# PMatthaei/ma-league

Measured on AMD Instinct MI355X. Metric: env-steps/sec (rollout+learn), 5v5 QMIX, 4096 envs, at 1/2/4/8 MI355X, higher is better.
Workload: dtype f32

## Files before the change

### include/maleague.h

```cpp
#ifndef MALEAGUE_H
#define MALEAGUE_H

#include <stdint.h>

#ifdef __cplusplus
extern "C" {
#endif

#define MLG_MAXU 64

typedef struct {
    int32_t U;
    int32_t n_agents;
    int32_t n_actions;
    int32_t grid;
    int32_t episode_limit;
    int32_t stochastic;
    int32_t policy_team;
    int32_t n_policy_teams;
    int32_t team[MLG_MAXU];
    int32_t role[MLG_MAXU];
    int32_t melee[MLG_MAXU];
    int32_t agent_unit[MLG_MAXU];
    int32_t scripted[2];
    uint64_t seed;
} MlgEnvSpec;

typedef struct {
    int32_t *x, *y, *hp;
    int32_t *t;
    uint32_t *episode;
    int32_t B;
} MlgEnvState;

typedef struct {
    float *state;
    float *obs;
    int64_t *actions;
    int32_t *avail;
    float *reward;
    uint8_t *terminated;
    float *actions_onehot;
    int64_t *filled;
    int32_t B, T1;
    int32_t ring_slot0, ring_size, full_write;
    const int32_t *rows;
    int32_t *slot_extent;
} MlgBatch;

typedef struct {
    int32_t *ep_len;
    float *ret;
    int32_t *won;
    int32_t *draw;
    uint64_t *agent_rows;
    float *ret_away;
} MlgRunInfo;

typedef struct {
    const float *fc1_w, *fc1_b;
    const float *w_ih, *b_ih;
    const float *w_hh, *b_hh;
    const float *fc2_w, *fc2_b;
} MlgAgentParams;

typedef struct {
    int32_t d_obs, n_actions, n_agents, hidden, d_in;
    int32_t obs_last_action, obs_agent_id;
} MlgAgentDims;

int64_t mlg_packed_agent_size(const MlgAgentDims *d);
int mlg_pack_agent(const MlgAgentDims *d, const MlgAgentParams *p, float *packed, void *stream);

int mlg_env_reset(const MlgEnvSpec *spec, MlgEnvState *st, void *stream);
int mlg_env_step(const MlgEnvSpec *spec, MlgEnvState *st, const int64_t *actions ,
                 float *reward , int32_t *done , int32_t *won ,
                 int32_t *draw , void *stream);
int mlg_env_observe(const MlgEnvSpec *spec, const MlgEnvState *st, float *obs ,
                    float *state , int32_t *avail , void *stream);

int mlg_rollout(const MlgEnvSpec *spec, MlgEnvState *st, const MlgAgentDims *dims, const float *packed,
                MlgBatch *batch, MlgRunInfo *info, float epsilon, int32_t test_mode, void *stream);

int mlg_rollout_selfplay(const MlgEnvSpec *spec, MlgEnvState *st, const MlgAgentDims *dims, const float *home_packed,
                         const float *away_packed, MlgBatch *home, MlgBatch *away, MlgRunInfo *info,
                         float eps_home, float eps_away, int32_t test_mode, void *stream);

int mlg_rollout_describe(const MlgEnvSpec *spec, const MlgAgentDims *dims, int32_t selfplay, char *name,
                         int32_t name_cap, int64_t *lds_bytes);

int mlg_zero_slots_bytes(const MlgBatch *batch, const int64_t *slot_bytes, int32_t slot0, int32_t count,
                         int32_t ring_size, void *stream);

int mlg_agent_forward(const MlgAgentDims *d, const float *packed, const float *inputs, const float *h_in,
                      float *q, float *h_out, int32_t R, void *stream);

int mlg_mac_forward(const MlgAgentDims *d, const float *packed, const MlgBatch *batch, int32_t t,
                    const float *h_in, float *q , float *h_out, void *stream);

int mlg_select_actions(const float *q, const int32_t *avail, int32_t R, int32_t A, int32_t n_agents,
                       const uint64_t *keys, const uint32_t *episodes, int32_t t, float epsilon,
                       int64_t *actions, int64_t *is_greedy, void *stream);

typedef struct {
    const float *hw1_0w, *hw1_0b, *hw1_2w, *hw1_2b;
    const float *hwf_0w, *hwf_0b, *hwf_2w, *hwf_2b;
    const float *hb1_w, *hb1_b;
    const float *v0_w, *v0_b, *v2_w, *v2_b;
    int32_t n_agents, state_dim, embed_dim, hypernet_embed, hypernet_layers;
} MlgQMixParams;
int mlg_qmix_forward(const MlgQMixParams *p, const float *agent_qs , const float *states ,
                     float *q_tot , int32_t R, void *stream);

int64_t mlg_agent_backward_workspace_floats(const MlgAgentDims *d, int32_t R);
int mlg_agent_backward(const MlgAgentDims *d, const MlgAgentParams *p, const float *packed, const float *inputs,
                       const float *h_in, const float *gq, const float *gh_out, float *d_inputs, float *d_h_in,
                       float *dparams, float *workspace, int32_t R, void *stream);
int64_t mlg_qmix_backward_workspace_floats(const MlgQMixParams *p, int32_t R);
int mlg_qmix_backward(const MlgQMixParams *p, const float *agent_qs, const float *states, const float *g_qtot,
                      float *d_agent_qs, float *dparams, float *workspace, int32_t R, void *stream);

typedef struct {
    int32_t B, T, N, A, d_obs, H, S, E, HE, hypernet_layers;
    int32_t mixer;
    int32_t double_q, obs_last_action, obs_agent_id;
    float gamma, lr, optim_alpha, optim_eps, grad_norm_clip;
    int32_t agent;
    int32_t distinct;
} MlgLearnerCfg;

typedef struct {
    MlgBatch batch;
    float *params;
    float *grads;
    float *square_avg;
    const float *target_params;
    float *workspace;
    float *stats;
    float *target_sync;
    double *trained_steps;
    const int32_t *host_rows;
} MlgLearnerBufs;

int64_t mlg_qlearner_param_counts(const MlgLearnerCfg *c, int64_t *n_agent, int64_t *n_mixer);
int64_t mlg_qlearner_workspace_floats(const MlgLearnerCfg *c);
int mlg_qlearner_inline_rows(void);
int mlg_qlearner_train(const MlgLearnerCfg *c, const MlgLearnerBufs *b, void *stream);
int mlg_qlearner_describe(const MlgLearnerCfg *c, char *name, int32_t name_cap);


typedef struct {
    MlgEnvSpec base;
    int32_t min_agents, max_agents;
} MlgEntityEnvSpec;

typedef struct {
    float *entities;
    uint8_t *obs_mask;
    uint8_t *entity_mask;
    int64_t *actions;
    int32_t *avail;
    float *reward;
    uint8_t *terminated;
    float *actions_onehot;
    int64_t *filled;
    int32_t B, T1, ring_slot0, ring_size, full_write;
    const int32_t *rows;
    int32_t *slot_extent;
} MlgEntityBatch;

typedef struct {
    int32_t n_agents, n_entities, entity_shape, n_actions, entity_last_action;
    int32_t attn_embed_dim, attn_n_heads, rnn_hidden_dim;
} MlgRefilDims;

int64_t mlg_refil_packed_agent_size(const MlgRefilDims *d);
int mlg_refil_pack_agent(const MlgRefilDims *d, const float *flat, float *packed, void *stream);

int mlg_refil_agent_forward(const MlgRefilDims *d, const float *packed, const float *entities, const uint8_t *obs_mask,
                            const uint8_t *entity_mask, const float *h_in, float *q, float *h_out, int32_t R,
                            void *stream);

int mlg_refil_rollout(const MlgEntityEnvSpec *spec, MlgEnvState *st, const MlgRefilDims *d, const float *packed,
                      MlgEntityBatch *batch, MlgRunInfo *info, float epsilon, int32_t test_mode, void *stream);

int mlg_refil_rollout_describe(const MlgEntityEnvSpec *spec, const MlgRefilDims *d, char *name, int32_t name_cap,
                               int64_t *lds_bytes);

int mlg_refil_attention(const float *w_in, const float *w_out, const float *b_out, const float *x,
                        const uint8_t *pre_mask, const uint8_t *post_mask, int32_t bs, int32_t ne, int32_t nq,
                        int32_t n_heads, float *y, void *stream);

int64_t mlg_refil_packed_mixer_size(const MlgRefilDims *d);
int mlg_refil_pack_mixer(const MlgRefilDims *d, const float *flat, float *packed, void *stream);
int mlg_refil_mixer_forward(const MlgRefilDims *d, const float *packed, const float *agent_qs, const float *entities,
                            const uint8_t *entity_mask, const uint8_t *w_mask, const uint8_t *i_mask,
                            int32_t softmax_mixing_weights, float *q_tot, int32_t R, void *stream);

int64_t mlg_refil_attention_backward_workspace_floats(int32_t bs, int32_t ne, int32_t nq, int32_t n_heads);
int mlg_refil_attention_backward(const float *w_in, const float *w_out, const float *b_out, const float *x,
                                 const uint8_t *pre_mask, const uint8_t *post_mask, const float *gy, int32_t bs,
                                 int32_t ne, int32_t nq, int32_t n_heads, float *dx, float *dparams, float *workspace,
                                 void *stream);
int64_t mlg_refil_mixer_backward_workspace_floats(const MlgRefilDims *d, int32_t R, int32_t imagine);
int mlg_refil_mixer_backward(const MlgRefilDims *d, const float *packed, const float *agent_qs, const float *entities,
                             const uint8_t *entity_mask, const uint8_t *w_mask, const uint8_t *i_mask,
                             int32_t softmax_mixing_weights, const float *g_qtot, float *d_agent_qs, float *dparams,
                             float *workspace, int32_t R, void *stream);
int64_t mlg_refil_agent_backward_workspace_floats(const MlgRefilDims *d, int32_t R);
int mlg_refil_agent_backward(const MlgRefilDims *d, const float *packed, const float *entities,
                             const uint8_t *obs_mask, const uint8_t *entity_mask, const float *h_in, const float *gq,
                             const float *gh_out, float *d_h_in, float *dparams, float *workspace, int32_t R,
                             void *stream);

typedef struct {
    int32_t B, T, n_agents, n_entities, entity_shape, n_actions, entity_last_action;
    int32_t attn_embed_dim, attn_n_heads, rnn_hidden_dim, hypernet_embed, mixing_embed_dim;
    int32_t double_q, softmax_mixing_weights;
    int32_t imagine;
    int32_t mixer;
    float gamma, lmbda, lr, optim_alpha, optim_eps, grad_norm_clip;
} MlgRefilLearnerCfg;

typedef struct {
    MlgEntityBatch batch;
    const uint8_t *groupA;
    float *params;
    float *grads;
    float *square_avg;
    const float *target_params;
    float *workspace;
    float *stats;
    double *trained_steps;
    float *target_sync;
    const int32_t *host_rows;
} MlgRefilLearnerBufs;

int64_t mlg_refil_param_counts(const MlgRefilLearnerCfg *c, int64_t *n_agent, int64_t *n_mixer);
int64_t mlg_refil_workspace_floats(const MlgRefilLearnerCfg *c);
int mlg_refil_train(const MlgRefilLearnerCfg *c, const MlgRefilLearnerBufs *b, void *stream);
int mlg_refil_draw_groups(int32_t B, int32_t NE, uint64_t seed, uint32_t draw, uint8_t *groupA, void *stream);

int mlg_debug_set_stamps(void *ptr);
int mlg_debug_set_learner_stamps(void *ptr);
int mlg_refil_debug_set_stamps(void *ptr);

int mlg_league_record_runs(const int32_t *won, const int32_t *draw, int32_t B, float *entry, int32_t count_games,
                           void *stream);

typedef struct {
    int32_t home, away;
    int32_t spec;
} MlgCrossplayPair;

typedef struct {
    const float *packed_pool;
    int32_t n_pool;
    int32_t n_pairs;
    const MlgCrossplayPair *pairs;
    const MlgCrossplayPair *host_pairs;
    const MlgEnvSpec *specs;
    const MlgEnvSpec *host_specs;
    int32_t n_specs;
    int32_t E;
    uint32_t episode0;
    float *workspace;
    int64_t workspace_floats;
    int32_t *ep_len;
    float *ret, *ret_away;
    int32_t *won;
    int32_t *draw;
    float *summary;
} MlgCrossplay;

int64_t mlg_crossplay_workspace_floats(const MlgAgentDims *dims, int32_t n_pairs, int32_t E);
int mlg_crossplay_rollout(const MlgAgentDims *dims, const MlgCrossplay *c, void *stream);

int mlg_pack_agent_pool(const MlgAgentDims *dims, const float *flat, int64_t row_stride, int32_t P,
                        float *packed_pool, void *stream);

int mlg_policy_probs(const float *logits, const int32_t *avail, int32_t R, int32_t A, float epsilon,
                     int32_t mask_before_softmax, int32_t test_mode, float *probs, void *stream);
int mlg_policy_probs_backward(const float *logits, const int32_t *avail, const float *g_probs, int32_t R, int32_t A,
                              float epsilon, int32_t mask_before_softmax, int32_t test_mode, float *d_logits,
                              void *stream);

int mlg_select_multinomial(const float *probs, const int32_t *avail, int32_t R, int32_t A, int32_t n_agents,
                           const uint64_t *keys, const uint32_t *episodes, int32_t t, int32_t greedy,
                           int64_t *actions, void *stream);

int mlg_rollout_policy(const MlgEnvSpec *spec, MlgEnvState *st, const MlgAgentDims *dims, const float *packed,
                       MlgBatch *batch, MlgRunInfo *info, float epsilon, int32_t test_mode,
                       int32_t mask_before_softmax, int32_t test_greedy, void *stream);

// ... 70 lines not shown
```

### ma-league_amd/csrc/distinct.hip

```cpp
#include <cstdlib>
#include <cstring>

#include "agent_device.h"
#include "rollout_env_device.h"
#include "rollout_host.h"

int check_agent_dims(const MlgAgentDims* d);

namespace {

constexpr int DX_MAX_WAVES = 8, DX_MAX_TPW = 4;

__device__ __forceinline__ floatx4 dx_row_chunk(const float* obs, const float* onehot, int k0, int d_obs, int d_in) {
    floatx4 v = {0.f, 0.f, 0.f, 0.f};
    if (!obs) return v;
#pragma unroll
    for (int r = 0; r < 4; ++r) {
        const int k = k0 + r;
        v[r] = k < d_obs ? obs[k] : ((onehot && k < d_in) ? onehot[k - d_obs] : 0.f);
    }
    return v;
}

template <int H>
// ... 100 lines not shown
    SpecShared& SS = *reinterpret_cast<SpecShared*>(smem + lay.env.spec);
    const RoEnv R = env_view(smem, lay.env);
    const int U = spec.U, N = spec.n_agents, A = spec.n_actions, S = 6 * U, DO = 8 * U;
    const int tid = threadIdx.x, nthr = blockDim.x;
    const int lane = tid & 63, wave = __builtin_amdgcn_readfirstlane(tid >> 6), W = nthr >> 6;
    const int e0 = blockIdx.x * RE;
    const int T1 = sd.bt[0].T1;
    const bool any_full_write = sd.bt[0].full_write != 0;
    load_spec_tables(spec, SS);
    const EnvTables T = make_tables(spec, SS);
    const float inv_p = 1.0f / (float)pow2_at_least(spec.grid);
    ro_reset<RoNoStamps>(T, SS, spec, st, R, sd, e0, inv_p);
    __syncthreads();

    floatx4 h[TPW][HC];
#pragma unroll
    for (int ti = 0; ti < TPW; ++ti)
#pragma unroll
        for (int c = 0; c < HC; ++c) h[ti][c] = floatx4{0.f, 0.f, 0.f, 0.f};
    RoNoStamps sp;
    sp.init();
    const int e = lane & 15, g = lane >> 4;
    const int n_at = L.Ap / 16;
    int last_t = 0;
    for (int t = 0; t < T1; ++t) {
#pragma unroll
        for (int ti = 0; ti < TPW; ++ti) {
            const int a = wave + ti * W;
            if (a >= N) continue;
            const bool valid = R.status[e] < 2;
            if (!__any(valid)) continue;
            int zero = 0;
            asm volatile("" : "+s"(zero));
            const WView Wv = global_view(sd.P[0] + (int64_t)a * L.total + zero, L);
            const MlgBatch bt = sd.bt[0];
            const int64_t bt_off = valid ? ((int64_t)R.slot[e] * T1 + t) * N + a : 0;
            RowIn in;
            in.x = valid ? bt.obs + bt_off * DO : nullptr;
            in.onehot = nullptr;
            in.prev_action = (valid && t > 0) ? R.prev[e * N + a] : -1;
            in.agent = 0;
            agent_cell_hidden<H>(Wv, L, in, h[ti], lane);
            const int32_t* av = valid ? bt.avail + bt_off * A : nullptr;
            ArgmaxState as{-INFINITY, 1 << 30};
            for (int at = 0; at < n_at; ++at) {
                const floatx4 q = agent_q_tile<H>(Wv, h[ti], at, lane);
                argmax_accumulate(as, q, av, at, A, lane);
            }
            const int act = argmax_reduce(as);
            if (valid && g == 0) ro_record_action(spec, R, sd, act, av, e, a, e0 + e, t, test_mode);
        }
        __syncthreads();
        ro_env_step(T, SS, spec, R, sd, info, e0, t, inv_p, sp);
        if (any_full_write && t + 1 < T1) zero_slots(sd, R, e0, t + 1, t + 2, A, S, DO);
        if (tid == 0) ro_list_running(R);
        __syncthreads();
        last_t = t;
        if (!R.misc[0]) break;
    }
    for (int x = tid; x < RE; x += nthr) R.stepped[x] = 0;
    __syncthreads();
    if (any_full_write && last_t + 2 < T1) zero_slots(sd, R, e0, last_t + 2, T1, A, S, DO);
    ro_finish(st, R, sd, info, e0, sd.bt[0].B, U);
}

int check_distinct_dims(const MlgAgentDims* dims, const char* who) {
    if (check_agent_dims(dims)) return 1;
    MLG_REQUIRE(dims->obs_agent_id == 0,
                "%s: obs_agent_id must be 0 (distinct agent networks take no agent id: network i is agent i)", who);
    return 0;
}

struct DxPlan {
    AgentLayout L;
    int tpw, waves;
    RolloutLds lay;
    char name[24];
};

int plan_distinct(const MlgEnvSpec* spec, const MlgAgentDims* dims, DxPlan* p) {
    MLG_REQUIRE(dims->n_agents == spec->n_agents && dims->n_actions == spec->n_actions && dims->d_obs == 8 * spec->U,
                "rollout_distinct: agent dims do not match env spec (N=%d/%d A=%d/%d d_obs=%d/%d)", dims->n_agents,
                spec->n_agents, dims->n_actions, spec->n_actions, dims->d_obs, 8 * spec->U);
    p->L = make_agent_layout(*dims);
    const int tiles = spec->n_agents;
    MLG_REQUIRE(tiles <= DX_MAX_WAVES * DX_MAX_TPW,
                "rollout_distinct: %d agent tiles (one per agent) > %d: at most %d tiles per wave on %d waves", tiles,
                DX_MAX_WAVES * DX_MAX_TPW, DX_MAX_TPW, DX_MAX_WAVES);
    p->waves = tiles < DX_MAX_WAVES ? tiles : DX_MAX_WAVES;
    p->tpw = (tiles + p->waves - 1) / p->waves;
    p->lay = make_rollout_lds(p->L, spec->U, spec->n_agents, false);
    MLG_REQUIRE((int64_t)p->lay.total * 4 <= LDS_LIMIT_BYTES,
                "rollout_distinct: the env state of %d units does not fit in LDS", spec->U);
    snprintf(p->name, sizeof p->name, "dx-global/tpw%d", p->tpw);
    return 0;
}

template <int H, int TPW>
int launch_distinct(const DxPlan& p, int grid, hipStream_t s, const MlgEnvSpec& spec, const MlgEnvState& st,
                    const Sides& sd, const MlgRunInfo& info, int test_mode) {
    const size_t bytes = (size_t)p.lay.total * 4;
    auto kern = rollout_distinct_kernel<H, TPW>;
    if (int rc = allow_lds(kern, bytes, "rollout_distinct")) return rc;
    hipLaunchKernelGGL(kern, dim3(grid), dim3(p.waves * 64), bytes, s, spec, st, p.L, sd, info, test_mode, p.lay);
    return 0;
}

}

extern "C" int mlg_mac_forward_distinct(const MlgAgentDims* d, const float* packed_pool, const MlgBatch* batch,
                                        int32_t t, const float* h_in, float* q, float* h_out, void* stream) {
    if (check_distinct_dims(d, "mac_forward_distinct")) return 1;
    MLG_REQUIRE(packed_pool && batch && batch->obs && batch->actions_onehot && q && h_out,
                "mac_forward_distinct: bad arguments");
    MLG_REQUIRE(mlg::aligned16(packed_pool), "mac_forward_distinct: packed_pool must be 16-byte aligned");
    MLG_REQUIRE(batch->B >= 0, "mac_forward_distinct: batch B=%d", batch->B);
    MLG_REQUIRE(t >= 0 && t < batch->T1, "mac_forward_distinct: t=%d out of [0, %d)", t, batch->T1);
    if (batch->B == 0) return 0;
    const AgentLayout L = make_agent_layout(*d);
    const int tpa = (batch->B + 15) / 16, tiles = tpa * d->n_agents;
    const int grid = (tiles + 3) / 4;
    hipStream_t s = (hipStream_t)stream;
#define MLG_DX_FWD(HH)                                                                                             \
    hipLaunchKernelGGL(mac_forward_distinct_kernel<HH>, dim3(grid), dim3(256), 0, s, L, packed_pool, *batch, (int)t, \
                       h_in, q, h_out, tpa, tiles)
    if (d->hidden == 64) MLG_DX_FWD(64);
    else if (d->hidden == 32) MLG_DX_FWD(32);
    else MLG_DX_FWD(128);
#undef MLG_DX_FWD
    return mlg::check_launch("mac_forward_distinct_kernel");
}

extern "C" int mlg_rollout_distinct_describe(const MlgEnvSpec* spec, const MlgAgentDims* dims, char* name,
                                             int32_t name_cap, int64_t* lds_bytes) {
    if (check_spec(spec) || check_distinct_dims(dims, "rollout_distinct_describe")) return 1;
    MLG_REQUIRE(name && name_cap > 0 && lds_bytes, "rollout_distinct_describe: null output");
    DxPlan plan;
    if (int rc = plan_distinct(spec, dims, &plan)) return rc;
    MLG_REQUIRE((size_t)name_cap > strlen(plan.name), "rollout_distinct_describe: name buffer of %d bytes too small",
                name_cap);
    strcpy(name, plan.name);
    *lds_bytes = (int64_t)plan.lay.total * 4;
    return 0;
}

extern "C" int mlg_rollout_distinct(const MlgEnvSpec* spec, MlgEnvState* st, const MlgAgentDims* dims,
                                    const float* packed_pool, MlgBatch* batch, MlgRunInfo* info, float epsilon,
                                    int32_t test_mode, void* stream) {
    if (check_spec(spec) || check_state(st) || check_distinct_dims(dims, "rollout_distinct")) return 1;
    MLG_REQUIRE(packed_pool && batch && info, "rollout_distinct: null pointer");
    MLG_REQUIRE(mlg::aligned16(packed_pool), "rollout_distinct: packed_pool must be 16-byte aligned");
    if (check_rollout_batch(batch, spec, st, "rollout_distinct")) return 1;
    MLG_REQUIRE(info->ep_len && info->ret && info->won && info->draw, "rollout_distinct: run info has null tensors");
    DxPlan plan;
    if (int rc = plan_distinct(spec, dims, &plan)) return rc;
    hipStream_t s = (hipStream_t)stream;
    Sides sd;
    sd.bt[0] = sd.bt[1] = *batch;
    sd.P[0] = sd.P[1] = packed_pool;
    sd.eps[0] = sd.eps[1] = test_mode ? 0.f : epsilon;
    sd.ns = 1;
    sd.nh = spec->n_agents;
    const int grid = (st->B + RE - 1) / RE;
    int rc = 0;
#define MLG_RO(HH, TT) rc = launch_distinct<HH, TT>(plan, grid, s, *spec, *st, sd, *info, test_mode ? 1 : 0)
#define MLG_RO_H(HH)                       \
    if (plan.tpw == 1) MLG_RO(HH, 1);      \
    else if (plan.tpw == 2) MLG_RO(HH, 2); \
    else if (plan.tpw == 3) MLG_RO(HH, 3); \
    else MLG_RO(HH, 4)
    if (plan.L.H == 64) {
        MLG_RO_H(64);
    } else if (plan.L.H == 32) {
        MLG_RO_H(32);
    } else {
        MLG_RO_H(128);
    }
#undef MLG_RO_H
#undef MLG_RO
    if (rc) return rc;
    return mlg::check_launch("rollout_distinct_kernel");
}
```

### ma-league_amd/csrc/learner.hip

```cpp
#include <algorithm>
#include <cstdio>
#include <cstring>

#include "agent_device.h"
#include "agent_ff_device.h"
#include "batch_mask_device.h"
#include "gru4_device.h"
#include "mlg_host.h"
#include "wgrad_device.h"

namespace {

using WJobs = mlg::BJobsT<16>;
using mlg::block_sum_1024;

struct AgentOffs {
    int64_t fc1w, fc1b, wih, whh, bih, bhh, fc2w, fc2b, total;
};
__host__ __device__ inline AgentOffs agent_offs(int H, int d_in, int A) {
    AgentOffs o;
    int64_t p = 0;
    o.fc1w = p; p += (int64_t)H * d_in;
    o.fc1b = p; p += H;
    o.wih = p; p += (int64_t)3 * H * H;
// ... 2256 lines not shown
                           ws + p.w.gr, ws + p.w.gz, ws + p.w.gn, ws + p.w.ghn, sk);
        hipLaunchKernelGGL((agent_q_kernel<H, true>), dim3(ntiles, c.T, 2 * c.N), dim3(64 * dsp.q_tiles), 0, s, c, p.L,
                           ws + p.w.p_on, ws + p.w.p_tg, ws + p.w.hs, ws + p.w.hs_tg, ws + p.w.mac, ws + p.w.tmac, sk);
    } else if (c.ff)
        hipLaunchKernelGGL((ff_hidden_kernel<H>), dim3(ntiles, c.T, 2), dim3(threads), 0, s, c, bt, p.L, ws + p.w.p_on,
                           ws + p.w.p_tg, ws + p.w.in, ws + p.w.hs, ws + p.w.hs_tg, sk);
    else
        hipLaunchKernelGGL((agent_in_kernel<H>), dim3(ntiles, c.T, 2), dim3(threads), 0, s, c, bt, p.L, ws + p.w.p_on,
                           ws + p.w.p_tg, ws + p.w.in, ws + p.w.x, ws + p.w.gi_on, ws + p.w.gi_tg, sk);
    if (c.ff || c.dx) {
    } else if (split_mix) {
        const int nrec = 2 * ((c.R + 3) / 4), per = dsp.per;
        hipLaunchKernelGGL((rec4_mixpre_kernel<H>), dim3(nrec + (p.w.n_mix_tiles + per - 1) / per), dim3(threads), 0, s,
                           c, p.L, ws + p.w.p_on, ws + p.w.p_tg, ws + p.w.gi_on, ws + p.w.gi_tg, ws + p.w.hs,
                           ws + p.w.hs_tg, ws + p.w.gr, ws + p.w.gz, ws + p.w.gn, ws + p.w.ghn, sk, bt, Mon,
                           Mtg, p.mp, hy);
    } else
        hipLaunchKernelGGL((agent_rec4_kernel<H>), dim3(2 * ((c.R + 3) / 4)), dim3(threads), 0, s, c, p.L,
                           ws + p.w.p_on, ws + p.w.p_tg, ws + p.w.gi_on, ws + p.w.gi_tg, ws + p.w.hs, ws + p.w.hs_tg,
                           ws + p.w.gr, ws + p.w.gz, ws + p.w.gn, ws + p.w.ghn, sk);
    if (!c.dx)
        hipLaunchKernelGGL((agent_q_kernel<H>), dim3(ntiles, c.T, 2), dim3(64 * dsp.q_tiles), 0, s, c, p.L, ws + p.w.p_on,
                           ws + p.w.p_tg, ws + p.w.hs, ws + p.w.hs_tg, ws + p.w.mac, ws + p.w.tmac, sk);
    MixOut mo{ws + p.w.srow, ws + p.w.l1act, ws + p.w.d1, ws + p.w.da2, ws + p.w.df2, ws + p.w.dv2,
              ws + p.w.dq, ws + p.w.d2, ws + p.w.part};
#define MLG_MIX_LAUNCH(K)                                                                                       \
    hipLaunchKernelGGL((K), dim3(p.w.n_mix_tiles), dim3(128), 0, s, c, bt, Mon, Mtg, p.mp, ws + p.w.mac, ws + p.w.tmac, \
                       ws + p.w.msum, mo, sk)
    switch (dsp.mix) {
        case MIX_IQL:
            hipLaunchKernelGGL(iql_td_kernel, dim3(p.w.n_mix_tiles), dim3(64), 0, s, c, bt, ws + p.w.mac, ws + p.w.tmac,
                               ws + p.w.msum, mo, sk);
            break;
        case MIX_QMIX_SPLIT:
            hipLaunchKernelGGL((mix_td2_kernel<64, 32>), dim3(p.w.n_mix_tiles), dim3(128), 0, s, c, bt, Mon, ws + p.w.mac,
                               ws + p.w.tmac, ws + p.w.msum, hy, mo, sk);
            break;
        case MIX_VDN_FAST:
        case MIX_QMIX_FAST1: MLG_MIX_LAUNCH((mix_td_kernel<64, 32, true>)); break;
        case MIX_QMIX1:
            if (c.E == 16) MLG_MIX_LAUNCH(mix_td1_kernel<16>);
            else if (c.E == 32) MLG_MIX_LAUNCH(mix_td1_kernel<32>);
            else MLG_MIX_LAUNCH(mix_td1_kernel<64>);
            break;
        case MIX_VDN:
        case MIX_QMIX_DFLT: MLG_MIX_LAUNCH((mix_td_kernel<64, 32>)); break;
        case MIX_QMIX_WIDTHS:
            switch (c.HE * 1000 + c.E) {
                case 32016: MLG_MIX_LAUNCH((mix_td_kernel<32, 16>)); break;
                case 32032: MLG_MIX_LAUNCH((mix_td_kernel<32, 32>)); break;
                case 32064: MLG_MIX_LAUNCH((mix_td_kernel<32, 64>)); break;
                case 64016: MLG_MIX_LAUNCH((mix_td_kernel<64, 16>)); break;
                case 64064: MLG_MIX_LAUNCH((mix_td_kernel<64, 64>)); break;
                case 128016: MLG_MIX_LAUNCH((mix_td_kernel<128, 16>)); break;
                case 128032: MLG_MIX_LAUNCH((mix_td_kernel<128, 32>)); break;
                case 128064: MLG_MIX_LAUNCH((mix_td_kernel<128, 64>)); break;
                default: return mlg::fail("learner: no mixer kernel for hypernet_embed=%d mixing_embed_dim=%d", c.HE, c.E);
            }
            break;
    }
#undef MLG_MIX_LAUNCH
    int64_t slab_floats, n_red;
    int n_tasks;
    mlg::BRepeat rp{};
    WJobs J = make_jobs(p, ws, bufs->grads, &slab_floats, &n_tasks, &n_red, &rp);
    if (c.dx) {
        hipLaunchKernelGGL((agent_bwd4_kernel<H, true>), dim3((Ra + 3) / 4, c.N), dim3(threads), 0, s, c, bt, p.L,
                           ws + p.w.p_on, ws + p.w.hs, ws + p.w.gr, ws + p.w.gz, ws + p.w.gn, ws + p.w.ghn, ws + p.w.dq,
                           ws + p.w.dgi, ws + p.w.dgh, sk);
        hipLaunchKernelGGL((agent_dx_kernel<H, true>), dim3(ntiles, c.T, c.N), dim3(threads), 0, s, c, ws + p.w.wihT,
                           ws + p.w.x, ws + p.w.dgi, ws + p.w.da, sk);
        hipLaunchKernelGGL(mlg::wgrad_block_rep_kernel<16>, dim3((unsigned)((n_tasks + 3) / 4)), dim3(256), 0, s, J, rp,
                           ws + p.w.slab);
        return run_finish(p, cfg, bufs, s, J, n_red, pj.flag, sk, ntiles, &rp);
    }
    if (c.ff) {
        hipLaunchKernelGGL((ff_bwd_kernel<H>), dim3(ntiles, c.T), dim3(threads), 0, s, c, p.L, ws + p.w.p_on, ws + p.w.hs,
                           ws + p.w.d2, ws + p.w.da, sk);
        hipLaunchKernelGGL(mlg::wgrad_block_kernel<16>, dim3((unsigned)((n_tasks + 3) / 4)), dim3(256), 0, s, J,
                           ws + p.w.slab);
        return run_finish(p, cfg, bufs, s, J, n_red, pj.flag, sk, ntiles);
    }
    int ta, tb;
    int64_t ra, rb;
    const WJobs JA = mlg::bjob_view(J, 3, J.n, &ta, &ra), JB = mlg::bjob_view(J, 0, 3, &tb, &rb);
    constexpr bool fused = Dispatch::fused_for(H);
    if constexpr (fused) {
        const int nbwd = (c.R + 3) / 4;
        hipLaunchKernelGGL((bwd4_wgrad_kernel<H>), dim3((unsigned)(nbwd + (ta + 3) / 4)), dim3(256), 0, s, c, bt, p.L,
                           ws + p.w.p_on, ws + p.w.hs, ws + p.w.gr, ws + p.w.gz, ws + p.w.gn, ws + p.w.ghn, ws + p.w.dq,
                           ws + p.w.dgi, ws + p.w.dgh, sk, JA, ws + p.w.slab, nbwd);
    } else {
        hipLaunchKernelGGL((agent_bwd4_kernel<H>), dim3((c.R + 3) / 4), dim3(threads), 0, s, c, bt, p.L, ws + p.w.p_on,
                           ws + p.w.hs, ws + p.w.gr, ws + p.w.gz, ws + p.w.gn, ws + p.w.ghn, ws + p.w.dq, ws + p.w.dgi,
                           ws + p.w.dgh, sk);
    }
    hipLaunchKernelGGL((agent_dx_kernel<H>), dim3(ntiles, c.T), dim3(threads), 0, s, c, ws + p.w.wihT, ws + p.w.x,
                       ws + p.w.dgi, ws + p.w.da, sk);
    if (fused)
        hipLaunchKernelGGL(mlg::wgrad_block_kernel<16>, dim3((unsigned)((tb + 3) / 4)), dim3(256), 0, s, JB,
                           ws + p.w.slab);
    else
        hipLaunchKernelGGL(mlg::wgrad_block_kernel<16>, dim3((unsigned)((n_tasks + 3) / 4)), dim3(256), 0, s, J,
                           ws + p.w.slab);
    return run_finish(p, cfg, bufs, s, J, n_red, pj.flag, sk, ntiles);
}

}

extern "C" int mlg_debug_set_learner_stamps(void* ptr) {
#ifdef MLG_STAMPS
    hipError_t e = hipMemcpyToSymbol(HIP_SYMBOL(g_mlg_lstamps), &ptr, sizeof(ptr));
    if (e != hipSuccess) return mlg::fail("set learner stamps: %s", hipGetErrorString(e));
    return 0;
#else
    (void)ptr;
    return mlg::fail("not a stamps build (-DMLG_STAMPS)");
#endif
}

extern "C" int64_t mlg_qlearner_param_counts(const MlgLearnerCfg* c, int64_t* n_agent, int64_t* n_mixer) {
    if (check_cfg(c)) return -1;
    Plan p = make_plan(c, c->T);
    if (n_agent) *n_agent = p.n_agent;
    if (n_mixer) *n_mixer = p.n_mixer;
    return p.n_agent + p.n_mixer;
}

extern "C" int mlg_qlearner_inline_rows(void) { return MLG_INLINE_ROWS; }

extern "C" int64_t mlg_qlearner_workspace_floats(const MlgLearnerCfg* c) {
    if (check_cfg(c)) return -1;
    Plan p = make_plan(c, c->T);
    int64_t slab, n_red;
    int tasks;
    mlg::BRepeat rp{};
    make_jobs(p, nullptr, nullptr, &slab, &tasks, &n_red, &rp);
    return p.w.total + slab;
}

extern "C" int mlg_qlearner_describe(const MlgLearnerCfg* c, char* name, int32_t name_cap) {
    if (check_cfg(c)) return 1;
    MLG_REQUIRE(name && name_cap > 0, "qlearner_describe: null output");
    Plan p = make_plan(c, c->T);
    Dispatch d;
    if (make_dispatch(p, &d)) return 1;
    char full[64];
    dispatch_name(p.c, d, full, sizeof full);
    MLG_REQUIRE((size_t)name_cap > strlen(full), "qlearner_describe: name buffer of %d bytes too small", name_cap);
    strcpy(name, full);
    return 0;
}

extern "C" int mlg_qlearner_train(const MlgLearnerCfg* c, const MlgLearnerBufs* b, void* stream) {
    if (check_cfg(c)) return 1;
    MLG_REQUIRE(b && b->params && b->grads && b->square_avg && b->target_params && b->workspace && b->stats,
                "qlearner_train: null buffer");
    const MlgBatch& bt = b->batch;
    MLG_REQUIRE(bt.state && bt.obs && bt.actions && bt.avail && bt.reward && bt.terminated && bt.actions_onehot && bt.filled,
                "qlearner_train: batch has null tensors");
    MLG_REQUIRE(bt.B == c->B && bt.T1 >= c->T, "qlearner_train: batch B=%d T1=%d vs cfg B=%d T=%d", bt.B, bt.T1, c->B, c->T);
    MLG_REQUIRE(!b->host_rows || c->B <= MLG_INLINE_ROWS, "qlearner_train: host_rows needs B <= %d (got %d)",
                MLG_INLINE_ROWS, c->B);
    Plan p = make_plan(c, bt.T1);
    hipStream_t s = (hipStream_t)stream;
    if (c->H == 64) return run_train<64>(p, c, b, s);
    if (c->H == 32) return run_train<32>(p, c, b, s);
    return run_train<128>(p, c, b, s);
}
```

### ma-league_amd/csrc/mlg_host.h

```cpp
#pragma once
#include <hip/hip_runtime.h>

#include <cstdarg>
#include <cstdio>
#include <mutex>
#include <string>

constexpr int MLG_INLINE_ROWS = 64;

namespace mlg {

inline std::string& last_error() {
    static thread_local std::string err;
    return err;
}

inline int fail(const char* fmt, ...) {
    char buf[1024];
    va_list ap;
    va_start(ap, fmt);
    vsnprintf(buf, sizeof(buf), fmt, ap);
    va_end(ap);
    last_error() = buf;
    return 1;
}

inline int check_launch(const char* what) {
    hipError_t e = hipGetLastError();
    if (e != hipSuccess) return fail("%s: %s", what, hipGetErrorString(e));
    return 0;
}

inline bool aligned16(const void* p) { return (reinterpret_cast<uintptr_t>(p) & 15u) == 0; }

struct SideStream {
    hipStream_t s = nullptr;
    hipEvent_t ev[4] = {nullptr, nullptr, nullptr, nullptr};
};
inline SideStream* side_stream(hipStream_t caller) {
    static SideStream side[64];
    static std::mutex mu;
    int dev = 0;
    hipDevice_t sdev = 0;
    if (hipGetDevice(&dev) != hipSuccess || dev < 0 || dev >= 64) return nullptr;
    if (hipStreamGetDevice(caller, &sdev) != hipSuccess || (int)sdev != dev) return nullptr;
    std::lock_guard<std::mutex> lk(mu);
    SideStream& ss = side[dev];
    if (!ss.s) {
        int least = 0, greatest = 0;
        if (hipDeviceGetStreamPriorityRange(&least, &greatest) != hipSuccess) return nullptr;
        SideStream fresh;
        for (auto& e : fresh.ev)
            if (hipEventCreateWithFlags(&e, hipEventDisableTiming) != hipSuccess) {
                for (auto& x : fresh.ev)
                    if (x) (void)hipEventDestroy(x);
                return nullptr;
            }
        if (hipStreamCreateWithPriority(&fresh.s, hipStreamNonBlocking, least) != hipSuccess) {
            for (auto& x : fresh.ev) (void)hipEventDestroy(x);
            return nullptr;
        }
        ss = fresh;
    }
    return &ss;
}
inline bool fork_join(SideStream* ss, int k, hipStream_t from, hipStream_t to) {
    return hipEventRecord(ss->ev[k], from) == hipSuccess && hipStreamWaitEvent(to, ss->ev[k], 0) == hipSuccess;
}

}

#define MLG_REQUIRE(cond, ...)                  \
    do {                                        \
        if (!(cond)) return mlg::fail(__VA_ARGS__); \
    } while (0)
```

### ma-league_amd/csrc/refil.hip

```cpp
#include <cstdlib>
#include <cstring>

#include "mlg_host.h"
#include "refil_device.h"
#include "refil_host.h"

using namespace refil;

#define RO_PHASE __device__ inline

#ifdef MLG_STAMPS
__device__ unsigned long long* g_refil_stamps = nullptr;
struct RStamps {
    unsigned long long acc[30], last, begin;
    __device__ void init() {
        for (int k = 0; k < 30; ++k) acc[k] = 0;
        last = begin = __builtin_amdgcn_s_memtime();
    }
    __device__ void mark(int k) {
        const unsigned long long now = __builtin_amdgcn_s_memtime();
        acc[k] += now - last;
        last = now;
    }
    unsigned long long s0;
// ... 724 lines not shown
    const int lane = threadIdx.x;
    const int i0 = blockIdx.x * 2;
    zero_tile(o, lane);
    if (lane < 32) {
        const int e = lane >> 4, q = lane & 15;
        const int64_t it = i0 + e;
        mrow[e][q] = (it < R && q < NEa) ? mask_row_bits(om + (it * NEa + q) * NEa, NEa) : 0xFFFFFFFFu;
        if (q == 0) emb[e] = it < R ? mask_row_bits(em + it * NEa, NEa) : 0xFFFFFFFFu;
    }
    wave_sync();
    for (int e = 0; e < 2; ++e) {
        const int64_t it = i0 + e;
        load_entity_rows(it < R ? ent + it * NEa * D0 : nullptr, NEa, D0, L.K1, ein, lane, 64);
        wave_sync();
        entity_block(P, L, ein, x1, qkv, mrow[e], NA, NEa, o + e * NAS * LDX, nullptr, lane);
    }
    const int col = lane & 15, g = lane >> 4;
    const int e = col >> 3, n = col & 7, it = i0 + e;
    const bool valid = it < R && n < NA;
    const uint32_t dead = dead_rows(emb[0], NA, NAS) | dead_rows(emb[1], NA, NAS) << 8;
    floatx4 h[4];
#pragma unroll
    for (int mt = 0; mt < 4; ++mt)
        h[mt] = valid ? ld4(h_in + ((int64_t)it * NA + n) * EMB + mt * 16 + 4 * g) : floatx4{0.f, 0.f, 0.f, 0.f};
    agent_tile_post(P, L, o, dead, h, lane);
    if (valid) {
#pragma unroll
        for (int mt = 0; mt < 4; ++mt) *reinterpret_cast<floatx4*>(h_out + ((int64_t)it * NA + n) * EMB + mt * 16 + 4 * g) = h[mt];
    }
    for (int at = 0; at < L.Ap / 16; ++at) {
        const floatx4 q = agent_q(P, L, h, at, dead, lane);
        if (valid) {
#pragma unroll
            for (int r = 0; r < 4; ++r) {
                const int ac = at * 16 + 4 * g + r;
                if (ac < A) q_out[((int64_t)it * NA + n) * A + ac] = q[r];
            }
        }
    }
}

#include "refil_ro4.inc"

}

extern "C" int mlg_refil_debug_set_stamps(void* ptr) {
#ifdef MLG_STAMPS
    unsigned long long* p = (unsigned long long*)ptr;
    if (hipMemcpyToSymbol(HIP_SYMBOL(g_refil_stamps), &p, sizeof(p)) != hipSuccess) return mlg::fail("set stamps");
    return 0;
#else
    (void)ptr;
    return mlg::fail("mlg_refil_debug_set_stamps: build with -DMLG_STAMPS (make stamps)");
#endif
}

extern "C" int64_t mlg_refil_packed_agent_size(const MlgRefilDims* d) {
    if (check_refil_dims(d)) return -1;
    return agent_layout(d).total;
}

extern "C" int mlg_refil_pack_agent(const MlgRefilDims* d, const float* flat, float* packed, void* stream) {
    if (check_refil_dims(d)) return 1;
    MLG_REQUIRE(flat && packed, "refil_pack_agent: null pointer");
    const RAgent L = agent_layout(d);
    if (launch_copy(agent_pack_jobs(L), flat, packed, (hipStream_t)stream)) return 1;
    hipLaunchKernelGGL(refil_pack_gsp_kernel, dim3((unsigned)((REFIL_GSP + REFIL_WSP + 255) / 256)), dim3(256), 0,
                       (hipStream_t)stream,
                       L, flat, packed);
    return mlg::check_launch("refil_pack_gsp_kernel");
}

extern "C" int mlg_refil_agent_forward(const MlgRefilDims* d, const float* packed, const float* entities,
                                       const uint8_t* obs_mask, const uint8_t* entity_mask, const float* h_in, float* q,
                                       float* h_out, int32_t R, void* stream) {
    if (check_refil_dims(d)) return 1;
    MLG_REQUIRE(packed && entities && obs_mask && entity_mask && h_in && q && h_out, "refil_agent_forward: null pointer");
    MLG_REQUIRE(R >= 0, "refil_agent_forward: R=%d", R);
    if (R == 0) return 0;
    const RAgent L = agent_layout(d);
    hipLaunchKernelGGL(refil_agent_step_kernel, dim3((unsigned)((R + 1) / 2)), dim3(64), 0, (hipStream_t)stream, L, packed,
                       R, d->n_agents, d->n_entities, L.D0, d->n_actions, entities, obs_mask, entity_mask, h_in, q, h_out);
    return mlg::check_launch("refil_agent_forward");
}

namespace {

struct RefilRolloutPlan {
    const char* name;
    bool four;
    bool st16;
    int kc;
    size_t lds_bytes;
};

int plan_refil_rollout(const MlgEntityEnvSpec* spec, const MlgRefilDims* d, RefilRolloutPlan* plan) {
    if (check_refil_dims(d)) return 1;
    MLG_REQUIRE(spec != nullptr, "refil_rollout: null argument");
    const MlgEnvSpec& sp = spec->base;
    const int S = sp.U / 2;
    MLG_REQUIRE(sp.U >= 2 && sp.U % 2 == 0 && sp.U <= NE && S <= NAS, "refil_rollout: U=%d unsupported (even, <= 16)",
                sp.U);
    MLG_REQUIRE(sp.n_agents == S && d->n_agents == S && d->n_entities == sp.U && d->entity_shape == 8 &&
                    d->n_actions == MLG_ACT_BASE + sp.U && d->entity_last_action,
                "refil_rollout: dims (n_agents=%d n_entities=%d entity_shape=%d n_actions=%d) do not match the env "
                "(S=%d, U=%d)", d->n_agents, d->n_entities, d->entity_shape, d->n_actions, S, sp.U);
    MLG_REQUIRE(spec->min_agents >= 1 && spec->min_agents <= spec->max_agents && spec->max_agents <= S,
                "refil_rollout: min_agents=%d max_agents=%d (slots %d)", spec->min_agents, spec->max_agents, S);
    MLG_REQUIRE(sp.policy_team == 0 && sp.scripted[0] == 0 && sp.scripted[1] == 1,
                "refil_rollout: the entity env has policy team 0 and scripted team 1");
    const RAgent L = agent_layout(d);
    const char* var = getenv("MLG_REFIL_ROLLOUT");
    const bool v1 = (var && strcmp(var, "v1") == 0) || L.K1 != 32;
    if (!v1) {
        const bool generic = getenv("MLG_REFIL_GENERIC") != nullptr;
        const bool st16 = sp.U == 16 && !generic;
        *plan = RefilRolloutPlan{st16 ? "ro4-static" : "ro4", true, st16, 2, sizeof(R4Shared)};
        return 0;
    }
    const int kc = L.K1 <= 16 ? 1 : (L.K1 <= 32 ? 2 : 3);
    static const char* const names[3] = {"ro2/kc1", "ro2/kc2", "ro2/kc3"};
    *plan = RefilRolloutPlan{names[kc - 1], false, false, kc, sizeof(RoShared)};
    return 0;
}

}

extern "C" int mlg_refil_rollout_describe(const MlgEntityEnvSpec* spec, const MlgRefilDims* d, char* name,
                                          int32_t name_cap, int64_t* lds_bytes) {
    MLG_REQUIRE(name && name_cap > 0 && lds_bytes, "refil_rollout_describe: null output");
    RefilRolloutPlan plan;
    if (int rc = plan_refil_rollout(spec, d, &plan)) return rc;
    MLG_REQUIRE((size_t)name_cap > strlen(plan.name), "refil_rollout_describe: name buffer of %d bytes too small",
                name_cap);
    strcpy(name, plan.name);
    *lds_bytes = (int64_t)plan.lds_bytes;
    return 0;
}

extern "C" int mlg_refil_rollout(const MlgEntityEnvSpec* spec, MlgEnvState* st, const MlgRefilDims* d,
                                 const float* packed, MlgEntityBatch* batch, MlgRunInfo* info, float epsilon,
                                 int32_t test_mode, void* stream) {
    MLG_REQUIRE(spec && st && packed && batch && info, "refil_rollout: null argument");
    RefilRolloutPlan plan;
    if (int rc = plan_refil_rollout(spec, d, &plan)) return rc;
    const MlgEnvSpec& sp = spec->base;
    const int S = sp.U / 2;
    const MlgEntityBatch& bt = *batch;
    MLG_REQUIRE(bt.entities && bt.obs_mask && bt.entity_mask && bt.actions && bt.avail && bt.reward && bt.terminated &&
                    bt.actions_onehot && bt.filled, "refil_rollout: batch has null tensors");
    MLG_REQUIRE(st->B == bt.B && bt.T1 >= sp.episode_limit + 1, "refil_rollout: B=%d/%d T1=%d (episode_limit %d)", st->B,
                bt.B, bt.T1, sp.episode_limit);
    MLG_REQUIRE(info->ep_len && info->ret && info->won && info->draw, "refil_rollout: run info has null buffers");
    if (bt.B == 0) return 0;
    int p = 1;
    while (p < sp.grid) p <<= 1;
    RoArgs a{sp.U, S, d->n_actions, d->entity_shape, S, spec->min_agents, spec->max_agents, bt.B, 1.0f / (float)p};
    const RAgent L = agent_layout(d);
    if (plan.four) {
        const size_t lds4 = plan.lds_bytes;
        const bool st16 = plan.st16;
        auto kern4 = st16 ? refil_rollout4_kernel<2, 16> : refil_rollout4_kernel<2, 0>;
        static bool attr4[2] = {false, false};
        if (!attr4[st16]) {
            hipError_t e = hipFuncSetAttribute(reinterpret_cast<const void*>(kern4),
                                               hipFuncAttributeMaxDynamicSharedMemorySize, (int)lds4);
            if (e != hipSuccess) return mlg::fail("refil_rollout: LDS %zu B: %s", lds4, hipGetErrorString(e));
            attr4[st16] = true;
        }
        const int per_block4 = R4_ENVS * R4_WAVES;
        hipLaunchKernelGGL(kern4, dim3((unsigned)((bt.B + per_block4 - 1) / per_block4)), dim3(64 * R4_WAVES), lds4,
                           (hipStream_t)stream, *spec, *st, L, packed, bt, *info, a, test_mode ? 0.f : epsilon,
                           test_mode);
        return mlg::check_launch("refil_rollout4");
    }
    auto kern = plan.kc == 1 ? refil_rollout_kernel<1>
                             : (plan.kc == 2 ? refil_rollout_kernel<2> : refil_rollout_kernel<3>);
    const size_t lds = plan.lds_bytes;
    static bool attr_set[3] = {false, false, false};
    const int ki = plan.kc - 1;
    if (!attr_set[ki]) {
        hipError_t e = hipFuncSetAttribute(reinterpret_cast<const void*>(kern), hipFuncAttributeMaxDynamicSharedMemorySize,
                                           (int)lds);
        if (e != hipSuccess) return mlg::fail("refil_rollout: LDS %zu B: %s", lds, hipGetErrorString(e));
        attr_set[ki] = true;
    }
    const int per_block = 2 * RO_WAVES;
    hipLaunchKernelGGL(kern, dim3((unsigned)((bt.B + per_block - 1) / per_block)), dim3(64 * RO_WAVES), lds,
                       (hipStream_t)stream, *spec, *st, L, packed, bt, *info, a, test_mode ? 0.f : epsilon, test_mode);
    return mlg::check_launch("refil_rollout");
}
```

### ma-league_amd/csrc/rollout.hip

```cpp
#include <cstring>

#include "agent_device.h"
#include "rollout_env_device.h"
#include "rollout_host.h"

#ifdef MLG_STAMPS
__device__ unsigned long long* g_mlg_stamps = nullptr;
struct Stamps {
    unsigned long long acc[30], last, begin, tstep;
    __device__ void init() {
        for (int k = 0; k < 30; ++k) acc[k] = 0;
        last = begin = tstep = __builtin_amdgcn_s_memtime();
    }
    __device__ void step(int t, int nrun) {
        const unsigned long long now = __builtin_amdgcn_s_memtime();
        if (g_mlg_stamps && threadIdx.x == 0 && t < 128)
            g_mlg_stamps[(int64_t)gridDim.x * 8 * 32 + (int64_t)blockIdx.x * 128 + t] = ((now - tstep) << 8) | (unsigned)nrun;
        tstep = now;
#ifdef MLG_STAMPS_LOWRUN
        on = nrun <= MLG_STAMPS_LOWRUN;
#endif
#ifdef MLG_STAMPS_MINRUN
        on = nrun >= MLG_STAMPS_MINRUN;
#endif
#ifdef MLG_STAMPS_TIMELINE
        on = nrun == 1 && !seen;
        seen = seen || on;
#endif
    }
    bool on = true;
    bool seen = false;
    __device__ void mark(int k) {
        const unsigned long long now = __builtin_amdgcn_s_memtime();
#ifdef MLG_STAMPS_TIMELINE
        if (on) acc[k] = now - tstep;
#else
        if (on) acc[k] += now - last;
#endif
        last = now;
    }
    __device__ void flush() {
        if ((threadIdx.x & 63) || !g_mlg_stamps) return;
        unsigned long long* o = g_mlg_stamps + ((int64_t)blockIdx.x * 8 + (threadIdx.x >> 6)) * 32;
        for (int k = 0; k < 30; ++k) o[k] = acc[k];
        o[30] = __builtin_amdgcn_s_memtime() - begin;
        o[31] = 1;
    }
};
#else
using Stamps = RoNoStamps;
#endif

namespace {

template <int H, int TPW, bool WLDS>
__global__ void __launch_bounds__(512) rollout_kernel(MlgEnvSpec spec, MlgEnvState st, AgentLayout L, Sides sd,
                                                     MlgRunInfo info, int test_mode, RolloutLds lay) {
    constexpr int HC = H / 16;
    extern __shared__ __attribute__((aligned(16))) int smem[];
    SpecShared& SS = *reinterpret_cast<SpecShared*>(smem + lay.env.spec);
    const RoEnv R = env_view(smem, lay.env);
    const int U = spec.U, N = spec.n_agents, A = spec.n_actions, S = 6 * U, DO = 8 * U, nh = sd.nh;
    const int tid = threadIdx.x, nthr = blockDim.x;
    const int lane = tid & 63, wave = tid >> 6, W = nthr >> 6;
    const int e0 = blockIdx.x * RE;
    const int T1 = sd.bt[0].T1;
    const bool any_full_write = sd.bt[0].full_write || (sd.ns > 1 && sd.bt[1].full_write);
    load_spec_tables(spec, SS);
    if (WLDS) load_weights_to_lds(sd.P[0], L, lay.lw, reinterpret_cast<float*>(smem + lay.wts));
    const EnvTables T = make_tables(spec, SS);
    const float inv_p = 1.0f / (float)pow2_at_least(spec.grid);
    ro_reset<Stamps>(T, SS, spec, st, R, sd, e0, inv_p);
    __syncthreads();

    floatx4 h[TPW][HC];
#pragma unroll
    for (int ti = 0; ti < TPW; ++ti)
#pragma unroll
        for (int c = 0; c < HC; ++c) h[ti][c] = floatx4{0.f, 0.f, 0.f, 0.f};
    Stamps sp;
    sp.init();
    const int tps = (RE * nh + 15) / 16, n_tiles = sd.ns * tps;
    const int col = lane & 15, g = lane >> 4;
    const int n_at = L.Ap / 16;
    int last_t = 0;
    for (int t = 0; t < T1; ++t) {
#pragma unroll
        for (int ti = 0; ti < TPW; ++ti) {
            const int tile = wave + ti * W;
            if (tile >= n_tiles) continue;
            const int side = tile >= tps;
            const int r = (tile - side * tps) * 16 + col;
            const bool in_range = r < RE * nh;
            const int e = in_range ? r / nh : 0, ln = r % nh, a = side * nh + ln;
            const bool valid = in_range && R.status[e] < 2;
            if (!__any(valid)) continue;
            int zero = 0;
            asm volatile("" : "+s"(zero));
            const WView Wv = WLDS ? lds_view(reinterpret_cast<const float*>(smem + lay.wts) + zero, lay.lw, L)
                                  : global_view((side ? sd.P[1] : sd.P[0]) + zero, L);
            const MlgBatch bt = side_batch(sd, side);
            const int64_t bt_off = valid ? ((int64_t)side_slot(R, side, e) * T1 + t) * nh + ln : 0;
            RowIn in;
            in.x = valid ? bt.obs + bt_off * DO : nullptr;
            in.onehot = nullptr;
            in.prev_action = (valid && t > 0) ? R.prev[e * N + a] : -1;
            in.agent = valid ? ln : 0;
            agent_cell_hidden<H>(Wv, L, in, h[ti], lane);
            const int32_t* av = valid ? bt.avail + bt_off * A : nullptr;
            ArgmaxState as{-INFINITY, 1 << 30};
            for (int at = 0; at < n_at; ++at) {
                const floatx4 q = agent_q_tile<H>(Wv, h[ti], at, lane);
                argmax_accumulate(as, q, av, at, A, lane);
            }
            const int act = argmax_reduce(as);
            if (valid && g == 0) ro_record_action(spec, R, sd, act, av, e, a, e0 + e, t, test_mode);
        }
        sp.mark(0);
        __syncthreads();
        sp.mark(1);
        ro_env_step(T, SS, spec, R, sd, info, e0, t, inv_p, sp);
        if (any_full_write && t + 1 < T1) zero_slots(sd, R, e0, t + 1, t + 2, A, S, DO);
        if (tid == 0) ro_list_running(R);
        __syncthreads();
        sp.mark(10);
        last_t = t;
        if (!R.misc[0]) break;
    }
    sp.flush();
    for (int e = tid; e < RE; e += nthr) R.stepped[e] = 0;
    __syncthreads();
    if (any_full_write && last_t + 2 < T1) zero_slots(sd, R, e0, last_t + 2, T1, A, S, DO);
    ro_finish(st, R, sd, info, e0, sd.bt[0].B, U);
}

__device__ inline int tail_init(const MlgBatch& bt, int slot) {
    int zend = bt.T1;
    if (bt.full_write && bt.slot_extent) {
        const int x = bt.slot_extent[slot];
        zend = x < 0 ? 0 : (x < bt.T1 ? x : bt.T1);
    }
    return bt.T1 | (zend << 16);
}
__device__ inline int tail_start(int zc, int row) { return (zc & ~0xFFFF) | row; }

__device__ inline void zero_slot_steps(const MlgBatch& bt, int slot, int z0, int z1, int N, int A, int S, int DO,
                                       int lane, int nl) {
    if (z0 >= z1) return;
    const int64_t r0 = (int64_t)slot * bt.T1 + z0;
    const int n = z1 - z0;
    auto z16 = [&](float* p, int per) {
        float* b = p + r0 * per;
        if (per % 4 == 0) {
            uint4* q = reinterpret_cast<uint4*>(b);
            for (int x = lane; x < n * per / 4; x += nl) gst(q + x, make_uint4(0u, 0u, 0u, 0u));
        } else {
            for (int x = lane; x < n * per; x += nl) gst(b + x, 0.f);
        }
    };
    z16(bt.obs, N * DO);
    z16(bt.state, S);
    int* av = bt.avail + r0 * N * A;
    float* oh = bt.actions_onehot + r0 * N * A;
    for (int x = lane; x < n * N * A; x += nl) {
        gst(av + x, 0);
        gst(oh + x, 0.f);
    }
    int64_t* ac = bt.actions + r0 * N;
    for (int x = lane; x < n * N; x += nl) gst(ac + x, (int64_t)0);
    for (int x = lane; x < n; x += nl) {
        gst(bt.reward + r0 + x, 0.f);
        gst(bt.terminated + r0 + x, (uint8_t)0);
        gst(bt.filled + r0 + x, (int64_t)0);
    }
}

struct UnitMasks {
    uint32_t team1, healer, tank, melee;
};

__device__ inline UnitMasks make_unit_masks(const SpecShared& SS, int U) {
    UnitMasks m{0u, 0u, 0u, 0u};
    for (int u = 0; u < U; ++u) {
        m.team1 |= (uint32_t)(SS.team[u] == 1) << u;
        m.healer |= (uint32_t)(SS.role[u] == 1) << u;
        m.tank |= (uint32_t)(SS.role[u] == 0) << u;
        m.melee |= (uint32_t)(SS.melee[u] == 1) << u;
    }
    return m;
}

__device__ __forceinline__ int pk_unit(int x, int y, int hp) { return x | (y << 12) | (hp << 24); }
__device__ __forceinline__ int pk_x(int q) { return q & 0xFFF; }
__device__ __forceinline__ int pk_y(int q) { return (q >> 12) & 0xFFF; }
__device__ __forceinline__ int pk_hp(int q) { return q >> 24; }
__device__ __forceinline__ int mask_role(const UnitMasks& M, int j) {
    return ((M.tank >> j) & 1) ? 0 : (((M.healer >> j) & 1) ? 1 : 2);
}
__device__ __forceinline__ int move_toward_d(int dx, int dy) {
    const int adx = dx < 0 ? -dx : dx, ady = dy < 0 ? -dy : dy;
    if (adx >= ady && dx != 0) return dx > 0 ? 3 : 4;
    if (dy != 0) return dy > 0 ? 1 : 2;
    return 0;
}

struct UnitLane {
    int x, y, hp;
    uint32_t tgt, sight;
    int ai;
};

__device__ __forceinline__ void v2_pair_pass(const UnitMasks& M, int U, int u, UnitLane& L, int* spk) {
    const uint32_t all = U >= 32 ? 0xFFFFFFFFu : ((1u << U) - 1u);
    const int hbase = (threadIdx.x & 63) & 32;
    const uint32_t alive_m = (uint32_t)(__ballot(u < U && L.hp > 0) >> hbase) & all;
    const int pk_own = pk_unit(L.x, L.y, L.hp);
    spk[u] = pk_own;
    const bool split = U <= 16, odd = split && (threadIdx.x & 16) != 0;
    int pkm = pk_own, uu = u;
    if (split) {
        const auto sw = __builtin_amdgcn_permlane16_swap((unsigned)pk_own, (unsigned)pk_own, false, false);
        pkm = odd ? (int)sw[0] : pk_own;
        uu = u & 15;
    }
    const int X = pk_x(pkm), Y = pk_y(pkm), HP = pk_hp(pkm);
    const int my_team = (M.team1 >> uu) & 1;
    const bool healer = (M.healer >> uu) & 1;
    const int r2 = ((M.melee >> uu) & 1) ? 2 : 9;
    const bool alive = HP > 0;
    const uint32_t mates = (my_team ? M.team1 : ~M.team1) & all;
    const uint32_t cand_a = alive ? (mates & alive_m & ~(1u << uu)) : 0u;
    const uint32_t cand_e = alive ? (~mates & alive_m & all) : 0u;
    const uint32_t seen = alive ? alive_m : 0u;
    constexpr uint32_t NONE = 0xFFFFFFFFu;
    uint32_t kbest = NONE, kally = NONE, kenemy = NONE, tgt = 0, sight = 0;
    auto visit = [&](int j, int q) {
        const int hj = pk_hp(q);
        const int dx = pk_x(q) - X, dy = pk_y(q) - Y;
        const uint32_t d2 = (uint32_t)(__mul24(dx, dx) + __mul24(dy, dy));
        const uint32_t bit = 1u << j;
        const bool vis = (seen & bit) && d2 <= MLG_SIGHT2;
        const bool inr = d2 <= (uint32_t)r2;
        const int mxj = (M.tank & bit) ? 64 : 32;
        const bool tg = inr && (healer ? ((cand_a & bit) && hj < mxj) : (cand_e & bit) != 0);
        sight |= vis ? bit : 0u;
        tgt |= tg ? bit : 0u;
        kbest = min(kbest, tg ? ((uint32_t)hj << 5 | j) : NONE);
        kally = min(kally, (cand_a & bit) ? (d2 << 5 | j) : NONE);
        kenemy = min(kenemy, (cand_e & bit) ? (d2 << 5 | j) : NONE);
    };
    if (split) {
        const int JH = (U + 1) >> 1, base = odd ? JH : 0;
        int q[8];
#pragma unroll
        for (int k = 0; k < 8; ++k) q[k] = k < JH ? spk[(base + k) & 31] : 0;
#pragma unroll
        for (int k = 0; k < 8; ++k)
            if (k < JH) visit((base + k) & 31, q[k]);
        auto other = [&](uint32_t v) {
            const auto s2 = __builtin_amdgcn_permlane16_swap(v, v, false, false);
            return (threadIdx.x & 16) ? s2[0] : s2[1];
        };
        kbest = min(kbest, other(kbest));
        kally = min(kally, other(kally));
        kenemy = min(kenemy, other(kenemy));
        tgt |= other(tgt);
        sight |= other(sight);
    } else {
        for (int j0 = 0; j0 < U; j0 += 4) {
            const int4 q4 = *reinterpret_cast<const int4*>(spk + j0);
            visit(j0, q4.x);
            if (j0 + 1 < U) visit(j0 + 1, q4.y);
            if (j0 + 2 < U) visit(j0 + 2, q4.z);
            if (j0 + 3 < U) visit(j0 + 3, q4.w);
        }
    }
    int ai = 0;
    if (alive) {
        uint32_t k = NONE;
        if (kbest != NONE) ai = MLG_ACT_BASE + (int)(kbest & 31);
        else if (healer && kally != NONE) k = (kally >> 5) > 2 ? kally : NONE;
        else k = kenemy;
        if (ai == 0 && k != NONE) {
            const int q = spk[k & 31];
            ai = move_toward_d(pk_x(q) - X, pk_y(q) - Y);
        }
    }
    L.tgt = tgt;
    L.sight = sight;
    L.ai = ai;
}

__device__ __forceinline__ void resolve_hits(const UnitMasks& M, int U, int hl, const int* spk, const int* sact, int& dmg,
                                             int& heal) {
    if (U <= 16) {
        const bool odd = (hl & 16) != 0;
        const int me = MLG_ACT_BASE + (hl & 15), JH = (U + 1) >> 1, base = odd ? JH : 0;
        int qs[8], as[8];
#pragma unroll
        for (int k = 0; k < 8; ++k) {
            qs[k] = k < JH ? spk[(base + k) & 31] : 0;
            as[k] = k < JH ? sact[(base + k) & 31] : 0;
        }
#pragma unroll
        for (int k = 0; k < 8; ++k) {
            if (k >= JH) break;
            const int i = base + k;
            const bool hit = i < U && pk_hp(qs[k]) > 0 && as[k] == me;
            const bool hl_i = (M.healer >> i) & 1;
            heal += (hit && hl_i) ? role_power(1) : 0;
            dmg += (hit && !hl_i) ? role_power(mask_role(M, i)) : 0;
        }
        const auto sd = __builtin_amdgcn_permlane16_swap((unsigned)dmg, (unsigned)dmg, false, false);
        const auto sh = __builtin_amdgcn_permlane16_swap((unsigned)heal, (unsigned)heal, false, false);
        dmg += (int)(odd ? sd[0] : sd[1]);
        heal += (int)(odd ? sh[0] : sh[1]);
        return;
    }
    const int me = MLG_ACT_BASE + hl;
    for (int i0 = 0; i0 < U; i0 += 4) {
        const int4 q4 = *reinterpret_cast<const int4*>(spk + i0);
        const int4 a4 = *reinterpret_cast<const int4*>(sact + i0);
// ... 770 lines not shown
    v2_observe(C.M, spec, *C.SS, C.pairtab, C.avtab, C.bt, slot, t, e, hbase, hl, L, C.lobs, C.ldo, C.lavm, C.inv_p, sp,
               C.obf, C.U, C.N, C.A, C.sd);
}

__device__ inline void env_lane_reset(const EnvCtx& C, const MlgEnvState& st, EnvLane& E, int e, int e0, int hl) {
    const MlgEnvSpec& spec = *C.spec;
    const int hbase = (threadIdx.x & 63) & 32;
    E.e = e;
    E.b = e0 + e;
    E.u = UnitLane{0, 0, 0, 0u, 0u, 0};
    E.st = 2;
    E.slot = 0;
    E.len = 0;
    E.zcur = C.bt.T1;
    E.h0 = 0;
    E.act = 0;
    E.ep = 0;
    E.ret = 0.f;
    E.stepped = false;
    if (E.b < C.B) {
        E.ep = st.episode[E.b];
        E.st = 0;
        E.slot = C.bt.ring_size > 0 ? (C.bt.ring_slot0 + E.b) % C.bt.ring_size : E.b;
        E.zcur = tail_init(C.bt, E.slot);
        if (hl < C.U) {
            const int tm = C.SS->team[hl];
            env_spawn_xyh(make_tables(spec, *C.SS), mlg_env_key(spec.seed, E.b), E.ep, hl, C.SS->team_first[tm],
                          C.SS->team_size[tm], E.u.x, E.u.y, E.u.hp);
        }
        if (hl == 0) {
            st.episode[E.b] = E.ep + 1;
            gst(C.bt.filled + (int64_t)E.slot * C.bt.T1, (int64_t)1);
        }
    }
    if (hl == 0) {
        C.R.status[e] = E.st;
        C.R.slot[e] = E.slot;
        C.R.episode[e] = E.ep;
        C.amask[e] = E.b < C.B ? (C.N >= 32 ? 0xFFFFFFFFu : (1u << C.N) - 1u) : 0u;
    }
    if (E.b < C.B) {
        Stamps none;
        v2_pair_pass(C.M, C.U, hl, E.u, C.pk + e * 32);
        env_observe(C, spec, E.slot, 0, e, hbase, hl, E.u, none);
    }
}

__device__ inline void env_lane_step1(const EnvCtx& C, EnvLane& E, int t, int hl) {
    E.stepped = false;
    if (E.st == 2) return;
    const MlgEnvSpec& spec = *C.spec;
    const int N = C.N, A = C.A, U = C.U, T1 = C.bt.T1;
    int* pact = C.R.pact + E.e * N;
    if (hl < N && !((C.amask[E.e] >> hl) & 1u)) {
        pact[hl] = 0;
        const int64_t off = ((int64_t)E.slot * T1 + t) * N + hl;
        gst(C.bt.actions + off, (int64_t)0);
        if (!C.bt.full_write) gst(C.bt.actions_onehot + off * A, 1.0f);
    }
    if (hl < N) C.R.prev[E.e * N + hl] = pact[hl];
    if (C.bt.full_write) {
        const int64_t oh = ((int64_t)E.slot * T1 + t) * N * A;
#pragma unroll 1
        for (int k = hl; k < N * A; k += 32) {
            const int pt = C.sd ? ((k / A) << 8) | (k % A) : C.avtab[k];
            gst(C.bt.actions_onehot + oh + k, (pt & 255) == pact[pt >> 8] ? 1.0f : 0.0f);
        }
    }
    if (E.st == 1) {
        E.st = 2;
        E.zcur = tail_start(E.zcur, t + 1);
        if (hl == 0) C.amask[E.e] = 0u;
        if (C.bt.full_write && hl == 0) {
            gst(C.bt.reward + (int64_t)E.slot * T1 + t, 0.f);
            gst(C.bt.terminated + (int64_t)E.slot * T1 + t, (uint8_t)0);
        }
        if (hl == 0) C.R.status[E.e] = E.st;
        return;
    }
    const bool uvalid = hl < U;
    int act = 0;
    if (uvalid) {
        const int ag = C.SS->agent[hl];
        if (ag) {
            const int a = pact[ag - 1];
            act = (a >= 0 && a < MLG_ACT_BASE + U && v2_avail(C.M, spec.grid, E.u.x, E.u.y, E.u.hp, E.u.tgt, a)) ? a : 0;
        } else {
            act = E.u.ai;
        }
    }
    int* sact = C.act + E.e * 32;
    const int* spk = C.pk + E.e * 32;
    sact[hl] = act;
    int dmg = 0, heal = 0;
    resolve_hits(C.M, U, hl, spk, sact, dmg, heal);
    E.h0 = E.u.hp;
    if (uvalid && E.h0 > 0) {
        const int v = E.h0 - dmg + heal, mx = role_maxhp(mask_role(C.M, hl));
        E.u.hp = v < 0 ? 0 : (v > mx ? mx : v);
        E.u.x += (act == 3) - (act == 4);
        E.u.y += (act == 1) - (act == 2);
    }
    E.act = act;
    E.stepped = true;
}

__device__ inline void env_lane_step2(const EnvCtx& C, EnvLane& E, int t, int hl, Stamps& sp) {
    if (!E.stepped) return;
    const MlgEnvSpec& spec = *C.spec;
    const int U = C.U, T1 = C.bt.T1;
    const int hbase = (threadIdx.x & 63) & 32;
    const bool uvalid = hl < U;
    const int h0 = E.h0, h1 = E.u.hp;
    const uint32_t alive_m = (uint32_t)(__ballot(uvalid && h1 > 0) >> hbase);
    const uint32_t kill_m = (uint32_t)(__ballot(uvalid && h0 > 0 && h1 == 0) >> hbase);
    int lost0, lost1;
    team_losses(C.M, uvalid && h0 > h1 ? h0 - h1 : 0, hbase, lost0, lost1);
    const int alive0 = __builtin_popcount(alive_m & ~C.M.team1), alive1 = __builtin_popcount(alive_m & C.M.team1);
    const int kills0 = __builtin_popcount(kill_m & C.M.team1), kills1 = __builtin_popcount(kill_m & ~C.M.team1);
    const int done = alive0 == 0 || alive1 == 0 || t + 1 >= spec.episode_limit;
    const int won0 = alive1 == 0 && alive0 > 0, won1 = alive0 == 0 && alive1 > 0;
    const int pt = spec.policy_team;
    const int wpt = pt ? won1 : won0, wop = pt ? won0 : won1;
    const int r_int = (pt ? lost0 : lost1) + 10 * (pt ? kills1 : kills0) + 200 * wpt;
    const float r = (float)r_int * 0.0625f;
    E.ret += r;
    if (hl == 0) {
        const int64_t sl = (int64_t)E.slot * T1 + t;
        gst(C.bt.reward + sl, r);
        gst(C.bt.terminated + sl, (uint8_t)done);
        gst(C.bt.filled + sl + 1, (int64_t)1);
        if (done) {
            gst(C.info.won + 2 * E.b, (int32_t)wpt);
            gst(C.info.won + 2 * E.b + 1, (int32_t)wop);
            gst(C.info.draw + E.b, (int32_t)(!won0 && !won1));
        }
    }
    if (done) {
        E.st = 1;
        E.len = t + 1;
    }
    if (hl == 0) C.R.status[E.e] = E.st;
    {
        const int N = C.N;
        const uint32_t am = (uint32_t)(__ballot(hl < N && ((alive_m >> C.SS->aunit[hl < N ? hl : 0]) & 1u)) >> hbase);
        if (hl == 0) C.amask[E.e] = am;
    }
    sp.mark(6);
    v2_pair_pass(C.M, U, hl, E.u, C.pk + E.e * 32);
    sp.mark(7);
    env_observe(C, spec, E.slot, t + 1, E.e, hbase, hl, E.u, sp);
}

__device__ inline void env_lane_tail(const EnvCtx& C, EnvLane& E, int steps, int hl) {
    const int z0 = E.zcur & 0xFFFF, zend = E.zcur >> 16;
    if (!C.bt.full_write || E.st != 2 || z0 >= zend || E.b >= C.B) return;
    const int z1 = z0 + steps < zend ? z0 + steps : zend;
    zero_slot_steps(C.bt, E.slot, z0, z1, C.N, C.A, 6 * C.U, 8 * C.U, hl, 32);
    E.zcur = (E.zcur & ~0xFFFF) | z1;
}

__device__ inline void env_lane_finish(const EnvCtx& C, const MlgEnvState& st, EnvLane& E, int hl) {
    if (E.b >= C.B) return;
    const int U = C.U;
    if (C.bt.full_write) env_lane_tail(C, E, C.bt.T1, hl);
    if (hl == 0) {
        if (C.bt.full_write && C.bt.slot_extent) C.bt.slot_extent[E.slot] = E.len + 1;
        C.info.ep_len[E.b] = E.len;
        C.info.ret[E.b] = E.ret;
        st.t[E.b] = E.len;
    }
    if (hl < U) {
        st.x[(int64_t)E.b * U + hl] = E.u.x;
        st.y[(int64_t)E.b * U + hl] = E.u.y;
        st.hp[(int64_t)E.b * U + hl] = E.u.hp;
    }
}

__device__ inline EnvCtx make_env_ctx(const MlgEnvSpec& spec, const RolloutLds2& lay, int* smem, const MlgBatch& bt,
                                      const MlgRunInfo& info, int U, int N, int A, bool sd) {
    EnvCtx C;
    C.U = U;
    C.N = N;
    C.A = A;
    C.sd = sd;
    float* fm = reinterpret_cast<float*>(smem);
    C.spec = &spec;
    C.SS = reinterpret_cast<const SpecShared*>(smem + lay.env.spec);
    C.M = make_unit_masks(*C.SS, U);
    C.R = env_view(smem, lay.env);
    C.bt = bt;
    C.info = info;
    C.pairtab = smem + lay.pairtab;
    C.avtab = smem + lay.avtab;
    C.pk = smem + lay.pk;
    C.act = smem + lay.act;
    C.amask = reinterpret_cast<uint32_t*>(smem + lay.am);
    C.lobs = fm + lay.obs;
    C.lavm = reinterpret_cast<uint64_t*>(smem + lay.avail);
    C.ldo = lay.ldo;
    C.obf = lay.xpl != 0;
    C.B = bt.B;
    C.inv_p = 1.0f / (float)pow2_at_least(spec.grid);
    return C;
}

__device__ __forceinline__ EnvCtx env_ctx_step(const EnvCtx& C) {
    EnvCtx c = C;
    asm volatile("" : "+v"(c.M.team1), "+v"(c.M.healer), "+v"(c.M.tank), "+v"(c.M.melee));
    asm volatile("" : "+v"(c.bt.obs), "+v"(c.bt.state), "+v"(c.bt.avail), "+v"(c.bt.actions));
    asm volatile("" : "+v"(c.bt.actions_onehot), "+v"(c.bt.reward), "+v"(c.bt.terminated), "+v"(c.bt.filled));
    return c;
}

template <int H, bool G8, int SN, int SU>
struct StaticShape {
    static constexpr bool on = SN > 0;
    static constexpr MlgAgentDims dims{8 * SU, 5 + SU, SN, H, 8 * SU + 5 + SU + SN, 1, 1};
    static constexpr AgentLayout L = on ? make_agent_layout(dims) : AgentLayout{};
    static constexpr RolloutLds2 lay = on ? make_rollout_lds2(L, SU, SN, 16, 2, G8 ? 1 : 0) : RolloutLds2{};
};

__device__ __forceinline__ MlgBatch split_batch_sgprs(MlgBatch b) {
    asm volatile("" : "+s"(b.obs), "+s"(b.state), "+s"(b.avail), "+s"(b.actions));
    asm volatile("" : "+s"(b.actions_onehot), "+s"(b.reward), "+s"(b.terminated), "+s"(b.filled));
    return b;
}

template <int H, bool G8, int SN = 0, int SU = 0>
__device__ __forceinline__ void rollout_v2_body(const MlgEnvSpec& spec, const MlgEnvState& st, const AgentLayout& L,
                                                const float* __restrict__ P, const MlgBatch& bt_arg, const MlgRunInfo& info,
                                                float eps, int test_mode, const RolloutLds2& lay, int DU, int DN,
                                                int DA, bool SD) {
    const MlgBatch bt = split_batch_sgprs(bt_arg);
    constexpr int HC = H / 16, NW = 8, REW = 16, G = NW / HC;
    extern __shared__ __attribute__((aligned(16))) int smem[];
    float* fm = reinterpret_cast<float*>(smem);
    const int N = spec.n_agents, lane = threadIdx.x & 63, wave = __builtin_amdgcn_readfirstlane(threadIdx.x >> 6), hl = lane & 31;
    const int e0 = blockIdx.x * REW, T1 = bt.T1;
    v2_prologue(spec, L, P, lay, smem, REW * N);
    const EnvCtx C = make_env_ctx(spec, lay, smem, bt, info, DU, DN, DA, SD);
    EnvLane E;
    env_lane_reset(C, st, E, wave * 2 + (lane >> 5), e0, hl);
    const int j = wave % HC, gi = wave / HC;
    GruChunk<G8 ? 16 : H> W;
    GruG8 W8;
    if constexpr (G8)
        load_gru_g8(W8, P, L, lay, wave, lane);
    else
        load_gru_chunk<H>(W, P, L, fm, lay, j, lane);
    __syncthreads();
    Stamps sp;
    sp.init();
    uint64_t rows_issued = 0;
    uint32_t m_prev = 0u;
    int x_prev = 0;
    for (int t = 0; t < T1; ++t) {
        const uint32_t run = (uint32_t)__ballot(lane < REW && C.R.status[lane & (REW - 1)] < 2);
        sp.step(t, __popc(run));
        if (run == 0) break;
        const float* hc = fm + lay.hb + (t & 1) * (lay.nhb - 1) * lay.hsz;
        float* hn = fm + lay.hb + ((t & 1) ^ 1) * (lay.nhb - 1) * lay.hsz;
        StepRows SR;
        int tiles;
        int* wmap = smem + lay.rmap + wave * lay.rms;
        if constexpr (G8) {
            tiles = make_rmap(C.amask[lane & 15], wmap, lane, m_prev, x_prev);
            sp.mark(14);
            if constexpr (SN > 0) {
                const int nu = tiles > gi ? (tiles - gi + G - 1) / G : 0;
                fc1_g8_static<H, (8 * SU + 31) / 32, (SN + G - 1) / G>(L, lay, fm, wmap, C.R.prev, nu, j, gi, G, t, lane);
            } else
                ph_fc1_g8<H>(L, lay, fm, wmap, C.R.prev, tiles, j, gi, G, t, lane);
        } else {
            SR = make_rows(C.amask, 0, 16, lane);
            tiles = SR.tiles;
            ph_fc1<H>(L, lay, fm, C.R.prev, SR, j, gi, G, t, lane);
        }
        rows_issued += tiles * 16;
        sp.mark(0);
        lds_barrier();
        if constexpr (G8) sp.mark(5);
        int pre = -1;
        if constexpr (G8)
            if (wave < tiles) pre = eps_coin(spec, C.R, wmap, wave, e0, t, eps, test_mode, lane);
        if constexpr (G8)
            ph_gru_g8<H>(W8, lay, fm, wmap, hn, tiles, N, wave, lane);
        else
            ph_gru<H>(W, lay, fm, hc, hn, SR, N, j, gi, G, lane);
        sp.mark(1);
        lds_barrier();
        if constexpr (G8) sp.mark(13);
        if constexpr (G8)
            ph_fc2_g8<H>(spec, L, lay, fm, wmap, C.R, bt, hn, tiles, wave, NW, e0, t, eps, test_mode, lane, pre);
        else
            ph_fc2<H>(spec, L, lay, fm, C.R, bt, hn, SR, wave, NW, e0, t, eps, test_mode, lane);
        if constexpr (G8) {
            const bool idle = tiles < NW;
            const int step = idle ? NW - tiles : NW;
            for (int ti = idle ? wave - tiles : wave; ti >= 0 && ti < tiles; ti += step)
                hpl_split_tile<H>(lay, fm, wmap, hn, ti, N, lane);
        }
        sp.mark(2);
        lds_barrier();
        sp.mark(3);
        const EnvCtx Ce = env_ctx_step(C);
        env_lane_step1(Ce, E, t, hl);
        sp.mark(4);
        env_lane_step2(Ce, E, t, hl, sp);
#if defined(MLG_V7_TAIL_MIXED)
        if (!E.stepped && (t & 1)) env_lane_tail(Ce, E, 8, hl);
#else
        if (__ballot(E.stepped) == 0 && (t & 1)) env_lane_tail(Ce, E, 8, hl);
#endif
        sp.mark(8);
        lds_barrier();
        sp.mark(10);
    }
    sp.flush();
    if (threadIdx.x == 0 && info.agent_rows) atomicAdd(info.agent_rows, (unsigned long long)rows_issued);
    env_lane_finish(C, st, E, hl);
}

template <int H, bool G8 = false, int SN = 0, int SU = 0>
__global__ void __launch_bounds__(512, 2) rollout_v2_kernel(MlgEnvSpec spec, MlgEnvState st, AgentLayout L,
                                                           const float* __restrict__ P, MlgBatch bt, MlgRunInfo info,
                                                           float eps, int test_mode, RolloutLds2 lay) {
    using S = StaticShape<H, G8, SN, SU>;
    if constexpr (S::on)
        rollout_v2_body<H, G8, SN, SU>(spec, st, S::L, P, bt, info, eps, test_mode, S::lay, SU, SN, 5 + SU, true);
    else
        rollout_v2_body<H, G8>(spec, st, L, P, bt, info, eps, test_mode, lay, spec.U, spec.n_agents, spec.n_actions,
                               G8);
}

#include "rollout_sp.inc"
#include "rollout_sp8.inc"

__global__ void env_reset_kernel(MlgEnvSpec spec, MlgEnvState st) {
    __shared__ SpecShared SS;
    load_spec_tables(spec, SS);
    const EnvTables T = make_tables(spec, SS);
    const int b = blockIdx.x * blockDim.x + threadIdx.x;
    if (b >= st.B) return;
    const uint32_t ep = st.episode[b];
    st.episode[b] = ep + 1;
    st.t[b] = 0;
    const int U = spec.U;
    for (int u = 0; u < U; ++u) {
        const int tm = SS.team[u];
        env_spawn_unit(T, mlg_env_key(spec.seed, b), ep, u, SS.team_first[tm], SS.team_size[tm], st.x + (int64_t)b * U,
                       st.y + (int64_t)b * U, st.hp + (int64_t)b * U);
    }
}

__global__ void env_step_kernel(MlgEnvSpec spec, MlgEnvState st, const int64_t* __restrict__ actions, float* reward,
                                int32_t* done_out, int32_t* won_out, int32_t* draw_out) {
    __shared__ SpecShared SS;
    __shared__ int s_act[64][MLG_MAXU], s_nhp[64][MLG_MAXU];
    load_spec_tables(spec, SS);
    const EnvTables T = make_tables(spec, SS);
    const int b = blockIdx.x * blockDim.x + threadIdx.x;
    if (b >= st.B) return;
    const int U = spec.U, N = spec.n_agents;
    int* x = st.x + (int64_t)b * U;
    int* y = st.y + (int64_t)b * U;
    int* hp = st.hp + (int64_t)b * U;
    int* act = s_act[threadIdx.x];
    int* nhp = s_nhp[threadIdx.x];
    for (int u = 0; u < U; ++u) {
        const int ag = SS.agent[u];
        act[u] = env_exec_action(T, x, y, hp, u, ag ? actions[(int64_t)b * N + ag - 1] : 0);
    }
    for (int j = 0; j < U; ++j) nhp[j] = env_resolve_hp(T, act, hp, j);
    for (int j = 0; j < U; ++j)
        if (hp[j] > 0) env_apply_move(act[j], &x[j], &y[j]);
    int alive[2] = {0, 0}, lost[2] = {0, 0}, kills[2] = {0, 0};
    for (int j = 0; j < U; ++j) {
        const int tm = SS.team[j];
        if (hp[j] > 0) {
            lost[tm] += hp[j] - nhp[j] > 0 ? hp[j] - nhp[j] : 0;
            if (nhp[j] == 0) kills[1 - tm] += 1;
        }
        if (nhp[j] > 0) alive[tm] += 1;
        hp[j] = nhp[j];
    }
    const int t = st.t[b];
    const int done = alive[0] == 0 || alive[1] == 0 || t + 1 >= spec.episode_limit;
    st.t[b] = t + 1;
    int won[2];
    won[0] = alive[1] == 0 && alive[0] > 0;
    won[1] = alive[0] == 0 && alive[1] > 0;
    int k = 0;
    for (int tm = 0; tm < 2; ++tm) {
        if (spec.scripted[tm]) continue;
        const int r_int = lost[1 - tm] + 10 * kills[tm] + 200 * won[tm];
        reward[(int64_t)b * spec.n_policy_teams + k] = (float)r_int * 0.0625f;
        ++k;
    }
    done_out[b] = done;
    won_out[2 * b] = won[spec.policy_team];
    won_out[2 * b + 1] = won[1 - spec.policy_team];
    draw_out[b] = done && !won[0] && !won[1];
}

__global__ void env_observe_kernel(MlgEnvSpec spec, MlgEnvState st, float* obs, float* state, int32_t* avail) {
    __shared__ SpecShared SS;
    load_spec_tables(spec, SS);
    const EnvTables T = make_tables(spec, SS);
    const int b = blockIdx.x * blockDim.x + threadIdx.x;
    if (b >= st.B) return;
    const int U = spec.U, N = spec.n_agents, A = spec.n_actions;
    const int* x = st.x + (int64_t)b * U;
    const int* y = st.y + (int64_t)b * U;
    const int* hp = st.hp + (int64_t)b * U;
    const float inv_p = 1.0f / (float)pow2_at_least(spec.grid);
    for (int a = 0; a < N; ++a)
        for (int j = 0; j < U; ++j) env_obs_feat(T, x, y, hp, spec.agent_unit[a], j, inv_p, obs + (((int64_t)b * N + a) * U + j) * 8);
    for (int j = 0; j < U; ++j) env_state_feat(T, x, y, hp, j, inv_p, state + ((int64_t)b * U + j) * 6);
    for (int a = 0; a < N; ++a)
        for (int k = 0; k < A; ++k) avail[((int64_t)b * N + a) * A + k] = env_avail_one(T, x, y, hp, spec.agent_unit[a], k);
}

template <int SN, int SU>
bool static_shape_matches(const AgentLayout& L, const RolloutLds2& lay) {
    using S = StaticShape<64, true, SN, SU>;
    return memcmp(&L, &S::L, sizeof(AgentLayout)) == 0 && memcmp(&lay, &S::lay, sizeof(RolloutLds2)) == 0;
}

enum class Arm { V1, V2, V7, SP2, SP7, SP8 };

struct RolloutPlan {
    Arm arm;
    int sn;
    int tpw, waves;
    bool wlds;
    RolloutLds lay1;
    RolloutLds2 lay2;
    RolloutLdsSP laysp;
    size_t lds_bytes;
    char name[24];
};

int plan_rollout_v1(const AgentLayout& L, const MlgEnvSpec& spec, bool selfplay, RolloutPlan* p) {
    const int ns = selfplay ? 2 : 1, nh = spec.n_agents / ns;
    const int tiles = ns * ((RE * nh + 15) / 16);
    p->arm = Arm::V1;
    p->sn = 0;
    p->waves = tiles < 8 ? tiles : 8;
    p->tpw = (tiles + p->waves - 1) / p->waves;
    MLG_REQUIRE(p->tpw <= 4, "rollout: %d agent tiles per wave > 4 (too many agents per env)", p->tpw);
    MLG_REQUIRE(L.H == 32 || L.H == 64 || L.H == 128, "rollout: rnn_hidden_dim=%d unsupported (32, 64, 128)", L.H);
    p->lay1 = make_rollout_lds(L, spec.U, spec.n_agents, true);
    p->wlds = !selfplay && p->lay1.total * 4 <= LDS_LIMIT_BYTES && !getenv("MLG_ROLLOUT_GLOBAL_WEIGHTS");
    if (!p->wlds) p->lay1 = make_rollout_lds(L, spec.U, spec.n_agents, false);
    p->lds_bytes = (size_t)p->lay1.total * 4;
    snprintf(p->name, sizeof p->name, "v1-%s/tpw%d", p->wlds ? "lds" : "global", p->tpw);
    return 0;
}

int plan_rollout_single(const AgentLayout& L, const MlgEnvSpec& spec, RolloutPlan* p) {
    const char* k = getenv("MLG_ROLLOUT_KERNEL");
    const int want = (k && k[0] == 'v') ? k[1] - '0' : (L.H == 64 ? 7 : 2);
    if (want == 1 || (L.H != 64 && L.H != 32) || spec.U > 32) return plan_rollout_v1(L, spec, false, p);
    p->lay2 = make_rollout_lds2(L, spec.U, spec.n_agents, 16);
    if (p->lay2.total * 4 > LDS_LIMIT_BYTES) return plan_rollout_v1(L, spec, false, p);
    p->arm = Arm::V2;
    p->sn = 0;
    if (want == 7 && L.H == 64) {
        const RolloutLds2 l7 = make_rollout_lds2(L, spec.U, spec.n_agents, 16, 2, 1);
        if (l7.total * 4 <= LDS_LIMIT_BYTES) {
            p->arm = Arm::V7;
            p->lay2 = l7;
            if (!getenv("MLG_ROLLOUT_GENERIC")) {
                if (static_shape_matches<5, 10>(L, l7)) p->sn = 5;
                else if (static_shape_matches<3, 6>(L, l7)) p->sn = 3;
            }
        }
    }
    p->lds_bytes = (size_t)p->lay2.total * 4;
    snprintf(p->name, sizeof p->name, "%s", p->arm == Arm::V2 ? "v2" : p->sn ? "v7-static" : "v7");
    return 0;
}

int plan_rollout_selfplay(const AgentLayout& L, const MlgEnvSpec& spec, RolloutPlan* p) {
    const char* k = getenv("MLG_ROLLOUT_KERNEL");
    const bool force_v1 = k && k[0] == 'v' && k[1] == '1', force_sp2 = k && !strcmp(k, "sp2");
    const bool force_sp7 = k && !strcmp(k, "sp7");
    const bool generic = getenv("MLG_ROLLOUT_GENERIC") != nullptr;
    if (!force_v1 && !force_sp2 && !force_sp7 && L.H == 64 && !generic) {
        p->sn = static_shape_matches_sp8<10, 10>(L, spec.n_agents) ? 10
                : static_shape_matches_sp8<6, 6>(L, spec.n_agents) ? 6 : 0;
        if (p->sn) {
            p->arm = Arm::SP8;
            p->lds_bytes = (size_t)(p->sn == 10 ? StaticShapeSP8<10, 10>::lay.total : StaticShapeSP8<6, 6>::lay.total) * 4;
            snprintf(p->name, sizeof p->name, "sp8");
            return 0;
        }
    }
    const RolloutLdsSP l7 = make_rollout_lds_sp(L, spec.U, spec.n_agents, true);
    if (!force_v1 && !force_sp2 && L.H == 64 && L.Dob <= 32 * SP7_MAXKK && l7.total * 4 <= LDS_LIMIT_BYTES) {
        p->arm = Arm::SP7;
        p->laysp = l7;
        p->sn = 0;
        if (!generic) {
            if (static_shape_matches_sp<10, 10>(L, l7)) p->sn = 10;
            else if (static_shape_matches_sp<6, 6>(L, l7)) p->sn = 6;
        }
        p->lds_bytes = (size_t)l7.total * 4;
        snprintf(p->name, sizeof p->name, "%s", p->sn ? "sp7-static" : "sp7");
        return 0;
    }
    const RolloutLdsSP lsp = make_rollout_lds_sp(L, spec.U, spec.n_agents);
    if (!force_v1 && (L.H == 64 || L.H == 32) && spec.U <= 32 && lsp.total * 4 <= LDS_LIMIT_BYTES) {
        p->arm = Arm::SP2;
        p->laysp = lsp;
        p->sn = 0;
        p->lds_bytes = (size_t)lsp.total * 4;
        snprintf(p->name, sizeof p->name, "sp2");
        return 0;
    }
    return plan_rollout_v1(L, spec, true, p);
}

int plan_rollout(const AgentLayout& L, const MlgEnvSpec& spec, bool selfplay, RolloutPlan* p) {
    return selfplay ? plan_rollout_selfplay(L, spec, p) : plan_rollout_single(L, spec, p);
}

template <int H, int TPW, bool WLDS>
int launch_rollout_t(hipStream_t s, const MlgEnvSpec& spec, const MlgEnvState& st, const AgentLayout& L,
                     const Sides& sd, const MlgRunInfo& info, int tm, const RolloutPlan& p) {
    auto kern = rollout_kernel<H, TPW, WLDS>;
    if (int rc = allow_lds(kern, p.lds_bytes, "rollout")) return rc;
    hipLaunchKernelGGL(kern, dim3((st.B + RE - 1) / RE), dim3(p.waves * 64), p.lds_bytes, s, spec, st, L, sd, info, tm,
                       p.lay1);
    return 0;
}

template <int H>
int launch_rollout_h(hipStream_t s, const MlgEnvSpec& spec, const MlgEnvState& st, const AgentLayout& L,
                     const Sides& sd, const MlgRunInfo& info, int tm, const RolloutPlan& p) {
#define MLG_RO(TT)                                                                 \
    return p.wlds ? launch_rollout_t<H, TT, true>(s, spec, st, L, sd, info, tm, p) \
                  : launch_rollout_t<H, TT, false>(s, spec, st, L, sd, info, tm, p)
    if (p.tpw == 1) MLG_RO(1);
    if (p.tpw == 2) MLG_RO(2);
    if (p.tpw == 3) MLG_RO(3);
    MLG_RO(4);
#undef MLG_RO
}

int launch_rollout_v1(hipStream_t s, const MlgEnvSpec& spec, const MlgEnvState& st, const AgentLayout& L,
                      const Sides& sd, const MlgRunInfo& info, int tm, const RolloutPlan& p) {
    int rc = L.H == 64   ? launch_rollout_h<64>(s, spec, st, L, sd, info, tm, p)
             : L.H == 32 ? launch_rollout_h<32>(s, spec, st, L, sd, info, tm, p)
                         : launch_rollout_h<128>(s, spec, st, L, sd, info, tm, p);
    if (rc) return rc;
    return mlg::check_launch("rollout_kernel");
}

int launch_rollout_v2(hipStream_t s, const MlgEnvSpec& spec, const MlgEnvState& st, const AgentLayout& L,
                      const float* P, const MlgBatch& bt, const MlgRunInfo& info, float eps, int tm,
                      const RolloutPlan& p) {
    auto kern = L.H == 64 ? rollout_v2_kernel<64> : rollout_v2_kernel<32>;
    if (p.arm == Arm::V7)
        kern = p.sn == 5   ? rollout_v2_kernel<64, true, 5, 10>
               : p.sn == 3 ? rollout_v2_kernel<64, true, 3, 6>
                           : rollout_v2_kernel<64, true>;
    const int threads = 512, rew = 16;
    if (int rc = allow_lds(kern, p.lds_bytes, "rollout v2")) return rc;
    hipLaunchKernelGGL(kern, dim3((bt.B + rew - 1) / rew), dim3(threads), p.lds_bytes, s, spec, st, L, P, bt, info, eps,
                       tm, p.lay2);
    return mlg::check_launch("rollout_v2_kernel");
}


}

int check_agent_dims(const MlgAgentDims* d);

struct ZeroJobs {
    unsigned char* base[16];
    int64_t begin[16], end[16];
    int64_t words0[17];
    int n;
};

__global__ void zero_ranges_kernel(ZeroJobs J) {
    const int64_t total = J.words0[J.n];
    for (int64_t i = (int64_t)blockIdx.x * blockDim.x + threadIdx.x; i < total; i += (int64_t)gridDim.x * blockDim.x) {
        int j = 0;
        while (j + 1 < J.n && J.words0[j + 1] <= i) ++j;
        const int64_t a0 = (J.begin[j] + 15) & ~int64_t(15);
        *reinterpret_cast<uint4*>(J.base[j] + a0 + (i - J.words0[j]) * 16) = make_uint4(0, 0, 0, 0);
    }
    if (blockIdx.x == 0 && threadIdx.x < J.n) {
        const int j = threadIdx.x;
        const int64_t a0 = (J.begin[j] + 15) & ~int64_t(15), a1 = J.end[j] & ~int64_t(15);
        if (a0 >= a1) {
            for (int64_t b = J.begin[j]; b < J.end[j]; ++b) J.base[j][b] = 0;
        } else {
            for (int64_t b = J.begin[j]; b < a0; ++b) J.base[j][b] = 0;
            for (int64_t b = a1; b < J.end[j]; ++b) J.base[j][b] = 0;
        }
    }
}

extern "C" int mlg_zero_slots_bytes(const MlgBatch* bt, const int64_t* slot_bytes , int32_t slot0, int32_t count,
                                    int32_t ring_size, void* stream) {
    MLG_REQUIRE(bt && slot_bytes, "zero_slots: null argument");
    MLG_REQUIRE(ring_size >= 1 && count >= 0 && count <= ring_size && slot0 >= 0 && slot0 < ring_size,
                "zero_slots: bad range (slot0=%d count=%d ring=%d)", slot0, count, ring_size);
    void* ptrs[8] = {bt->state, bt->obs, bt->actions, bt->avail, bt->reward, bt->terminated, bt->actions_onehot,
                     bt->filled};
    ZeroJobs J;
    J.n = 0;
    J.words0[0] = 0;
    const int first = (slot0 + count <= ring_size) ? count : ring_size - slot0;
    const int second = count - first;
    for (int k = 0; k < 8; ++k) {
        MLG_REQUIRE(ptrs[k] != nullptr && slot_bytes[k] > 0, "zero_slots: key %d missing", k);
        for (int part = 0; part < 2; ++part) {
            const int s0 = part == 0 ? slot0 : 0, n = part == 0 ? first : second;
            if (n <= 0) continue;
            J.base[J.n] = reinterpret_cast<unsigned char*>(ptrs[k]);
            J.begin[J.n] = (int64_t)s0 * slot_bytes[k];
            J.end[J.n] = (int64_t)(s0 + n) * slot_bytes[k];
            const int64_t a0 = (J.begin[J.n] + 15) & ~int64_t(15), a1 = J.end[J.n] & ~int64_t(15);
            J.words0[J.n + 1] = J.words0[J.n] + (a1 > a0 ? (a1 - a0) / 16 : 0);
            ++J.n;
        }
    }
    if (J.n == 0) return 0;
    hipLaunchKernelGGL(zero_ranges_kernel, dim3(2048), dim3(256), 0, (hipStream_t)stream, J);
    return mlg::check_launch("zero_ranges_kernel");
}

extern "C" int mlg_debug_set_stamps(void* ptr) {
#ifdef MLG_STAMPS
    hipError_t e = hipMemcpyToSymbol(HIP_SYMBOL(g_mlg_stamps), &ptr, sizeof(ptr));
    if (e != hipSuccess) return mlg::fail("set stamps: %s", hipGetErrorString(e));
    return 0;
#else
    (void)ptr;
    return mlg::fail("not a stamps build (-DMLG_STAMPS)");
#endif
}

extern "C" int mlg_env_reset(const MlgEnvSpec* spec, MlgEnvState* st, void* stream) {
    if (check_spec(spec) || check_state(st)) return 1;
    hipLaunchKernelGGL(env_reset_kernel, dim3((st->B + 63) / 64), dim3(64), 0, (hipStream_t)stream, *spec, *st);
    return mlg::check_launch("env_reset_kernel");
}

extern "C" int mlg_env_step(const MlgEnvSpec* spec, MlgEnvState* st, const int64_t* actions, float* reward,
                            int32_t* done, int32_t* won, int32_t* draw, void* stream) {
    if (check_spec(spec) || check_state(st)) return 1;
    MLG_REQUIRE(actions && reward && done && won && draw, "env_step: null output pointer");
    hipLaunchKernelGGL(env_step_kernel, dim3((st->B + 63) / 64), dim3(64), 0, (hipStream_t)stream, *spec, *st, actions,
                       reward, done, won, draw);
    return mlg::check_launch("env_step_kernel");
}

extern "C" int mlg_env_observe(const MlgEnvSpec* spec, const MlgEnvState* st, float* obs, float* state, int32_t* avail,
                               void* stream) {
    if (check_spec(spec) || check_state(st)) return 1;
    MLG_REQUIRE(obs && state && avail, "env_observe: null output pointer");
    hipLaunchKernelGGL(env_observe_kernel, dim3((st->B + 63) / 64), dim3(64), 0, (hipStream_t)stream, *spec, *st, obs,
                       state, avail);
    return mlg::check_launch("env_observe_kernel");
}

namespace {

int check_rollout_dims(const MlgEnvSpec* spec, const MlgAgentDims* dims) {
    MLG_REQUIRE(dims->n_agents == spec->n_agents && dims->n_actions == spec->n_actions && dims->d_obs == 8 * spec->U,
                "rollout: agent dims do not match env spec (N=%d/%d A=%d/%d d_obs=%d/%d)", dims->n_agents,
                spec->n_agents, dims->n_actions, spec->n_actions, dims->d_obs, 8 * spec->U);
    return 0;
}

int check_selfplay_dims(const MlgEnvSpec* spec, const MlgAgentDims* dims) {
    MLG_REQUIRE(spec->n_policy_teams == 2 && spec->n_agents % 2 == 0,
                "rollout_selfplay: %d agents in %d policy teams do not fit the symmetric two-team scenario "
                "(stepper_utils.py:9)", spec->n_agents, spec->n_policy_teams);
    const int nh = spec->n_agents / 2;
    MLG_REQUIRE(dims->n_agents == nh && dims->n_actions == spec->n_actions && dims->d_obs == 8 * spec->U,
                "rollout_selfplay: agent dims do not match one side of the env (N=%d/%d A=%d/%d d_obs=%d/%d)",
                dims->n_agents, nh, dims->n_actions, spec->n_actions, dims->d_obs, 8 * spec->U);
    for (int a = 0; a < nh; ++a)
        MLG_REQUIRE(spec->team[spec->agent_unit[a]] == spec->policy_team &&
                        spec->team[spec->agent_unit[nh + a]] == 1 - spec->policy_team,
                    "rollout_selfplay: agents 0..%d must be the home team, %d..%d the away team", nh - 1, nh,
                    2 * nh - 1);
    return 0;
}

}

extern "C" int mlg_rollout_describe(const MlgEnvSpec* spec, const MlgAgentDims* dims, int32_t selfplay, char* name,
                                    int32_t name_cap, int64_t* lds_bytes) {
    if (check_spec(spec) || check_agent_dims(dims)) return 1;
    MLG_REQUIRE(name && name_cap > 0 && lds_bytes, "rollout_describe: null output");
    if (selfplay ? check_selfplay_dims(spec, dims) : check_rollout_dims(spec, dims)) return 1;
    RolloutPlan plan;
    if (int rc = plan_rollout(make_agent_layout(*dims), *spec, selfplay != 0, &plan)) return rc;
    MLG_REQUIRE((size_t)name_cap > strlen(plan.name), "rollout_describe: name buffer of %d bytes too small", name_cap);
    strcpy(name, plan.name);
    *lds_bytes = (int64_t)plan.lds_bytes;
    return 0;
}

extern "C" int mlg_rollout(const MlgEnvSpec* spec, MlgEnvState* st, const MlgAgentDims* dims, const float* packed,
                           MlgBatch* batch, MlgRunInfo* info, float epsilon, int32_t test_mode, void* stream) {
    if (check_spec(spec) || check_state(st) || check_agent_dims(dims)) return 1;
    MLG_REQUIRE(packed && batch && info, "rollout: null pointer");
    if (check_rollout_batch(batch, spec, st, "rollout")) return 1;
    MLG_REQUIRE(info->ep_len && info->ret && info->won && info->draw, "rollout: run info has null tensors");
    if (check_rollout_dims(spec, dims)) return 1;
    const AgentLayout L = make_agent_layout(*dims);
    hipStream_t s = (hipStream_t)stream;
    const float eps = test_mode ? 0.f : epsilon;
    RolloutPlan plan;
    if (int rc = plan_rollout(L, *spec, false, &plan)) return rc;
    if (plan.arm != Arm::V1) return launch_rollout_v2(s, *spec, *st, L, packed, *batch, *info, eps, test_mode, plan);
    Sides sd;
    sd.bt[0] = sd.bt[1] = *batch;
    sd.P[0] = sd.P[1] = packed;
    sd.eps[0] = sd.eps[1] = eps;
    sd.ns = 1;
    sd.nh = spec->n_agents;
    return launch_rollout_v1(s, *spec, *st, L, sd, *info, test_mode, plan);
}

extern "C" int mlg_rollout_selfplay(const MlgEnvSpec* spec, MlgEnvState* st, const MlgAgentDims* dims,
                                    const float* home_packed, const float* away_packed, MlgBatch* home, MlgBatch* away,
                                    MlgRunInfo* info, float eps_home, float eps_away, int32_t test_mode, void* stream) {
    if (check_spec(spec) || check_state(st) || check_agent_dims(dims)) return 1;
    MLG_REQUIRE(home_packed && away_packed && info, "rollout_selfplay: null pointer");
    if (check_rollout_batch(home, spec, st, "rollout_selfplay (home)") ||
        check_rollout_batch(away, spec, st, "rollout_selfplay (away)"))
        return 1;
    MLG_REQUIRE(info->ep_len && info->ret && info->won && info->draw, "rollout_selfplay: run info has null tensors");
    if (check_selfplay_dims(spec, dims)) return 1;
    const AgentLayout L = make_agent_layout(*dims);
    hipStream_t s = (hipStream_t)stream;
    Sides sd;
    sd.bt[0] = *home;
    sd.bt[1] = *away;
    sd.P[0] = home_packed;
    sd.P[1] = away_packed;
    sd.eps[0] = test_mode ? 0.f : eps_home;
    sd.eps[1] = test_mode ? 0.f : eps_away;
    sd.ns = 2;
    sd.nh = spec->n_agents / 2;
    RolloutPlan plan;
    if (int rc = plan_rollout(L, *spec, true, &plan)) return rc;
    const size_t bytes = plan.lds_bytes;
    if (plan.arm == Arm::SP8) {
        auto kern = plan.sn == 10 ? rollout_sp8_kernel<10, 10> : rollout_sp8_kernel<6, 6>;
        if (int rc = allow_lds(kern, bytes, "rollout_selfplay")) return rc;
        hipLaunchKernelGGL(kern, dim3((st->B + RS8 - 1) / RS8), dim3(512), bytes, s, *spec, *st, home_packed,
                           away_packed, *home, *away, *info, sd.eps[0], sd.eps[1], test_mode);
        return mlg::check_launch("rollout_sp8_kernel");
    }
    if (plan.arm == Arm::SP7) {
        auto kern = plan.sn == 10 ? rollout_sp7_kernel<10, 10>
                    : plan.sn == 6 ? rollout_sp7_kernel<6, 6>
                                   : rollout_sp7_kernel<0, 0>;
        if (int rc = allow_lds(kern, bytes, "rollout_selfplay")) return rc;
        hipLaunchKernelGGL(kern, dim3((st->B + RS - 1) / RS), dim3(512), bytes, s, *spec, *st, L, home_packed,
                           away_packed, *home, *away, *info, sd.eps[0], sd.eps[1], test_mode, plan.laysp);
        return mlg::check_launch("rollout_sp7_kernel");
    }
    if (plan.arm == Arm::SP2) {
        auto kern = L.H == 64 ? rollout_sp_kernel<64> : rollout_sp_kernel<32>;
        if (int rc = allow_lds(kern, bytes, "rollout_selfplay")) return rc;
        hipLaunchKernelGGL(kern, dim3((st->B + RS - 1) / RS), dim3(512), bytes, s, *spec, *st, L, home_packed,
                           away_packed, *home, *away, *info, sd.eps[0], sd.eps[1], test_mode, plan.laysp);
        return mlg::check_launch("rollout_sp_kernel");
    }
    return launch_rollout_v1(s, *spec, *st, L, sd, *info, test_mode, plan);
}
```

### ma-league_amd/csrc/rollout_ff.hip

```cpp
#include <cstdlib>
#include <cstring>

#include "agent_ff_device.h"
#include "rollout_env_device.h"
#include "rollout_host.h"

int check_agent_dims(const MlgAgentDims* d);

namespace {

struct FFRolloutLds {
    int32_t wts, total;
    RoEnvLds env;
    LdsWeights lw;
};

__host__ __device__ inline FFRolloutLds make_ff_rollout_lds(const AgentLayout& L, int U, int n_agents,
                                                            bool weights_in_lds) {
    FFRolloutLds r;
    r.lw = make_ff_lds_weights(L);
    int64_t o = 0;
    r.wts = ro_take(o, weights_in_lds ? r.lw.total : 0);
    r.env = make_env_lds(o, U, n_agents);
    r.total = o;
    return r;
}

template <int H, int TPW, bool WLDS>
__global__ void __launch_bounds__(512) rollout_ff_kernel(MlgEnvSpec spec, MlgEnvState st, AgentLayout L, Sides sd,
                                                        MlgRunInfo info, int test_mode, FFRolloutLds lay) {
    constexpr int HC = H / 16;
    extern __shared__ __attribute__((aligned(16))) int smem[];
    SpecShared& SS = *reinterpret_cast<SpecShared*>(smem + lay.env.spec);
    const RoEnv R = env_view(smem, lay.env);
    const int U = spec.U, N = spec.n_agents, A = spec.n_actions, S = 6 * U, DO = 8 * U, nh = sd.nh;
    const int tid = threadIdx.x, nthr = blockDim.x;
    const int lane = tid & 63, wave = tid >> 6, W = nthr >> 6;
    const int e0 = blockIdx.x * RE;
    const int T1 = sd.bt[0].T1;
    const bool any_full_write = sd.bt[0].full_write != 0;
    load_spec_tables(spec, SS);
    if (WLDS) load_ff_weights_to_lds(sd.P[0], L, lay.lw, reinterpret_cast<float*>(smem + lay.wts));
    const EnvTables T = make_tables(spec, SS);
    const float inv_p = 1.0f / (float)pow2_at_least(spec.grid);
    ro_reset<RoNoStamps>(T, SS, spec, st, R, sd, e0, inv_p);
    __syncthreads();

    RoNoStamps sp;
    sp.init();
    const int n_tiles = (RE * nh + 15) / 16;
    const int col = lane & 15, g = lane >> 4;
    const int n_at = L.Ap / 16;
    int last_t = 0;
    for (int t = 0; t < T1; ++t) {
#pragma unroll
        for (int ti = 0; ti < TPW; ++ti) {
            const int tile = wave + ti * W;
            if (tile >= n_tiles) continue;
            const int r = tile * 16 + col;
            const bool in_range = r < RE * nh;
            const int e = in_range ? r / nh : 0, a = r % nh;
            const bool valid = in_range && R.status[e] < 2;
            if (!__any(valid)) continue;
            int zero = 0;
            asm volatile("" : "+s"(zero));
            const WView Wv = WLDS ? lds_view(reinterpret_cast<const float*>(smem + lay.wts) + zero, lay.lw, L)
                                  : global_view(sd.P[0] + zero, L);
            const MlgBatch bt = sd.bt[0];
            const int64_t bt_off = valid ? ((int64_t)R.slot[e] * T1 + t) * nh + a : 0;
            RowIn in;
            in.x = valid ? bt.obs + bt_off * DO : nullptr;
            in.onehot = nullptr;
            in.prev_action = (valid && t > 0) ? R.prev[e * N + a] : -1;
            in.agent = valid ? a : 0;
            floatx4 x[HC];
            ff_hidden<H, false>(Wv, L, in, x, lane);
            const int32_t* av = valid ? bt.avail + bt_off * A : nullptr;
            ArgmaxState as{-INFINITY, 1 << 30};
            for (int at = 0; at < n_at; ++at) {
                const floatx4 q = agent_q_tile<H>(Wv, x, at, lane);
                argmax_accumulate(as, q, av, at, A, lane);
            }
            const int act = argmax_reduce(as);
            if (valid && g == 0) ro_record_action(spec, R, sd, act, av, e, a, e0 + e, t, test_mode);
        }
        __syncthreads();
        ro_env_step(T, SS, spec, R, sd, info, e0, t, inv_p, sp);
        if (any_full_write && t + 1 < T1) zero_slots(sd, R, e0, t + 1, t + 2, A, S, DO);
        if (tid == 0) ro_list_running(R);
        __syncthreads();
        last_t = t;
        if (!R.misc[0]) break;
    }
    for (int e = tid; e < RE; e += nthr) R.stepped[e] = 0;
    __syncthreads();
    if (any_full_write && last_t + 2 < T1) zero_slots(sd, R, e0, last_t + 2, T1, A, S, DO);
    ro_finish(st, R, sd, info, e0, sd.bt[0].B, U);
}

template <int H, int TPW, bool WLDS>
int launch_ff_t(int grid, int threads, hipStream_t s, const MlgEnvSpec& spec, const MlgEnvState& st,
                const AgentLayout& L, const Sides& sd, const MlgRunInfo& info, int test_mode, const FFRolloutLds& lay) {
    const size_t bytes = (size_t)lay.total * 4;
    auto kern = rollout_ff_kernel<H, TPW, WLDS>;
    if (int rc = allow_lds(kern, bytes, "rollout_ff")) return rc;
    hipLaunchKernelGGL(kern, dim3(grid), dim3(threads), bytes, s, spec, st, L, sd, info, test_mode, lay);
    return 0;
}

struct FFPlan {
    AgentLayout L;
    int tpw, waves;
    bool wlds;
    FFRolloutLds lay;
    char name[24];
};

int plan_ff(const MlgEnvSpec* spec, const MlgAgentDims* dims, FFPlan* p) {
    MLG_REQUIRE(dims->n_agents == spec->n_agents && dims->n_actions == spec->n_actions && dims->d_obs == 8 * spec->U,
                "rollout_ff: agent dims do not match env spec (N=%d/%d A=%d/%d d_obs=%d/%d)", dims->n_agents,
                spec->n_agents, dims->n_actions, spec->n_actions, dims->d_obs, 8 * spec->U);
    p->L = make_ff_layout(*dims);
    const int tiles = (RE * spec->n_agents + 15) / 16;
    p->waves = tiles < 8 ? tiles : 8;
    p->tpw = (tiles + p->waves - 1) / p->waves;
    MLG_REQUIRE(p->tpw <= 4, "rollout_ff: %d agent tiles per wave > 4 (too many agents per env)", p->tpw);
    p->lay = make_ff_rollout_lds(p->L, spec->U, spec->n_agents, true);
    p->wlds = (int64_t)p->lay.total * 4 <= LDS_LIMIT_BYTES;
    if (!p->wlds) {
        p->lay = make_ff_rollout_lds(p->L, spec->U, spec->n_agents, false);
        MLG_REQUIRE((int64_t)p->lay.total * 4 <= LDS_LIMIT_BYTES,
                    "rollout_ff: the env state of %d units does not fit in LDS", spec->U);
    }
    snprintf(p->name, sizeof p->name, "ff-%s/tpw%d", p->wlds ? "lds" : "global", p->tpw);
    return 0;
}

template <int H, int TPW>
int launch_ff(const FFPlan& p, int grid, hipStream_t s, const MlgEnvSpec& spec, const MlgEnvState& st, const Sides& sd,
              const MlgRunInfo& info, int test_mode) {
    if (p.wlds) return launch_ff_t<H, TPW, true>(grid, p.waves * 64, s, spec, st, p.L, sd, info, test_mode, p.lay);
    return launch_ff_t<H, TPW, false>(grid, p.waves * 64, s, spec, st, p.L, sd, info, test_mode, p.lay);
}

}

extern "C" int mlg_rollout_ff_describe(const MlgEnvSpec* spec, const MlgAgentDims* dims, char* name, int32_t name_cap,
                                       int64_t* lds_bytes) {
    if (check_spec(spec) || check_agent_dims(dims)) return 1;
    MLG_REQUIRE(name && name_cap > 0 && lds_bytes, "rollout_ff_describe: null output");
    FFPlan plan;
    if (int rc = plan_ff(spec, dims, &plan)) return rc;
    MLG_REQUIRE((size_t)name_cap > strlen(plan.name), "rollout_ff_describe: name buffer of %d bytes too small",
                name_cap);
    strcpy(name, plan.name);
    *lds_bytes = (int64_t)plan.lay.total * 4;
    return 0;
}

extern "C" int mlg_rollout_ff(const MlgEnvSpec* spec, MlgEnvState* st, const MlgAgentDims* dims, const float* packed,
                              MlgBatch* batch, MlgRunInfo* info, float epsilon, int32_t test_mode, void* stream) {
    if (check_spec(spec) || check_state(st) || check_agent_dims(dims)) return 1;
    MLG_REQUIRE(packed && batch && info, "rollout_ff: null pointer");
    MLG_REQUIRE(mlg::aligned16(packed), "rollout_ff: packed must be 16-byte aligned");
    if (check_rollout_batch(batch, spec, st, "rollout_ff")) return 1;
    MLG_REQUIRE(info->ep_len && info->ret && info->won && info->draw, "rollout_ff: run info has null tensors");
    FFPlan plan;
    if (int rc = plan_ff(spec, dims, &plan)) return rc;
    hipStream_t s = (hipStream_t)stream;
    Sides sd;
    sd.bt[0] = sd.bt[1] = *batch;
    sd.P[0] = sd.P[1] = packed;
    sd.eps[0] = sd.eps[1] = test_mode ? 0.f : epsilon;
    sd.ns = 1;
    sd.nh = spec->n_agents;
    const int grid = (st->B + RE - 1) / RE;
    int rc = 0;
#define MLG_RO(HH, TT) rc = launch_ff<HH, TT>(plan, grid, s, *spec, *st, sd, *info, test_mode ? 1 : 0)
#define MLG_RO_H(HH)                       \
    if (plan.tpw == 1) MLG_RO(HH, 1);      \
    else if (plan.tpw == 2) MLG_RO(HH, 2); \
    else if (plan.tpw == 3) MLG_RO(HH, 3); \
    else MLG_RO(HH, 4)
    if (plan.L.H == 64) {
        MLG_RO_H(64);
    } else if (plan.L.H == 32) {
        MLG_RO_H(32);
    } else {
        MLG_RO_H(128);
    }
#undef MLG_RO_H
#undef MLG_RO
    if (rc) return rc;
    return mlg::check_launch("rollout_ff_kernel");
}
```

### ma-league_amd/csrc/rollout_policy.hip

```cpp
#include <cstdlib>
#include <cstring>

#include "agent_device.h"
#include "coma_device.h"
#include "rollout_env_device.h"
#include "rollout_host.h"

int check_agent_dims(const MlgAgentDims* d);

namespace {

constexpr int RO_MAXAT = 5;
__device__ __forceinline__ int ro_policy_select(floatx4 (&qt)[RO_MAXAT], int n_at, const int32_t* av, int A, int lane,
                                                float eps, bool mask, bool test_mode, bool greedy, float u) {
    const int g = lane >> 4;
    auto xor_f = [](float v, int m) { return __shfl_xor(v, m); };
    unsigned ok = 0u;
    float mx = -INFINITY;
#pragma unroll
    for (int at = 0; at < RO_MAXAT; ++at)
#pragma unroll
        for (int r = 0; r < 4; ++r) {
            const int a = at * 16 + 4 * g + r;
            const bool in = at < n_at && a < A;
// ... 82 lines not shown
    extern __shared__ __attribute__((aligned(16))) int smem[];
    SpecShared& SS = *reinterpret_cast<SpecShared*>(smem + lay.env.spec);
    const RoEnv R = env_view(smem, lay.env);
    const int U = spec.U, N = spec.n_agents, A = spec.n_actions, S = 6 * U, DO = 8 * U, nh = sd.nh;
    const int tid = threadIdx.x, nthr = blockDim.x;
    const int lane = tid & 63, wave = tid >> 6, W = nthr >> 6;
    const int e0 = blockIdx.x * RE;
    const int T1 = sd.bt[0].T1;
    const bool any_full_write = sd.bt[0].full_write || (sd.ns > 1 && sd.bt[1].full_write);
    load_spec_tables(spec, SS);
    if (WLDS) load_weights_to_lds(sd.P[0], L, lay.lw, reinterpret_cast<float*>(smem + lay.wts));
    const EnvTables T = make_tables(spec, SS);
    const float inv_p = 1.0f / (float)pow2_at_least(spec.grid);
    ro_reset<RoNoStamps>(T, SS, spec, st, R, sd, e0, inv_p);
    __syncthreads();

    floatx4 h[TPW][HC];
#pragma unroll
    for (int ti = 0; ti < TPW; ++ti)
#pragma unroll
        for (int c = 0; c < HC; ++c) h[ti][c] = floatx4{0.f, 0.f, 0.f, 0.f};
    RoNoStamps sp;
    sp.init();
    const int tps = (RE * nh + 15) / 16, n_tiles = sd.ns * tps;
    const int col = lane & 15, g = lane >> 4;
    const int n_at = L.Ap / 16;
    int last_t = 0;
    for (int t = 0; t < T1; ++t) {
#pragma unroll
        for (int ti = 0; ti < TPW; ++ti) {
            const int tile = wave + ti * W;
            if (tile >= n_tiles) continue;
            const int side = tile >= tps;
            const int r = (tile - side * tps) * 16 + col;
            const bool in_range = r < RE * nh;
            const int e = in_range ? r / nh : 0, ln = r % nh, a = side * nh + ln;
            const bool valid = in_range && R.status[e] < 2;
            if (!__any(valid)) continue;
            int zero = 0;
            asm volatile("" : "+s"(zero));
            const WView Wv = WLDS ? lds_view(reinterpret_cast<const float*>(smem + lay.wts) + zero, lay.lw, L)
                                  : global_view((side ? sd.P[1] : sd.P[0]) + zero, L);
            const MlgBatch bt = side_batch(sd, side);
            const int64_t bt_off = valid ? ((int64_t)side_slot(R, side, e) * T1 + t) * nh + ln : 0;
            RowIn in;
            in.x = valid ? bt.obs + bt_off * DO : nullptr;
            in.onehot = nullptr;
            in.prev_action = (valid && t > 0) ? R.prev[e * N + a] : -1;
            in.agent = valid ? ln : 0;
            agent_cell_hidden<H>(Wv, L, in, h[ti], lane);
            const int32_t* av = valid ? bt.avail + bt_off * A : nullptr;
            floatx4 qt[RO_MAXAT];
#pragma unroll
            for (int at = 0; at < RO_MAXAT; ++at)
                qt[at] = at < n_at ? agent_q_tile<H>(Wv, h[ti], at, lane) : floatx4{0.f, 0.f, 0.f, 0.f};
            const bool tm = (flags & 1) != 0, greedy = tm && (flags & 4) != 0;
            float u = 0.f;
            if (valid && !greedy)
                u = mlg_u01(mlg_rng(mlg_env_key(spec.seed, e0 + e),
                                    mlg_ctr(R.episode[e], (uint32_t)t, MLG_PURPOSE_POLICY, (uint32_t)a)));
            const int act = ro_policy_select(qt, n_at, av, A, lane, sd.eps[0], (flags & 2) != 0, tm, greedy, u);
            if (valid && g == 0) ro_record_action(spec, R, sd, act, av, e, a, e0 + e, t, 1);
        }
        sp.mark(0);
        __syncthreads();
        sp.mark(1);
        ro_env_step(T, SS, spec, R, sd, info, e0, t, inv_p, sp);
        if (any_full_write && t + 1 < T1) zero_slots(sd, R, e0, t + 1, t + 2, A, S, DO);
        if (tid == 0) ro_list_running(R);
        __syncthreads();
        sp.mark(10);
        last_t = t;
        if (!R.misc[0]) break;
    }
    sp.flush();
    for (int e = tid; e < RE; e += nthr) R.stepped[e] = 0;
    __syncthreads();
    if (any_full_write && last_t + 2 < T1) zero_slots(sd, R, e0, last_t + 2, T1, A, S, DO);
    ro_finish(st, R, sd, info, e0, sd.bt[0].B, U);
}


template <int H, int TPW, bool WLDS>
int launch_policy_t(int grid, int threads, hipStream_t s, const MlgEnvSpec& spec, const MlgEnvState& st,
                    const AgentLayout& L, const Sides& sd, const MlgRunInfo& info, int flags, const RolloutLds& lay) {
    const size_t bytes = (size_t)lay.total * 4;
    auto kern = rollout_policy_kernel<H, TPW, WLDS>;
    if (int rc = allow_lds(kern, bytes, "rollout_policy")) return rc;
    hipLaunchKernelGGL(kern, dim3(grid), dim3(threads), bytes, s, spec, st, L, sd, info, flags, lay);
    return 0;
}

struct PolicyPlan {
    AgentLayout L;
    int tpw, waves;
    bool wlds;
    RolloutLds lay;
    char name[24];
};

int plan_policy(const MlgEnvSpec* spec, const MlgAgentDims* dims, PolicyPlan* p) {
    MLG_REQUIRE(dims->n_agents == spec->n_agents && dims->n_actions == spec->n_actions && dims->d_obs == 8 * spec->U,
                "rollout_policy: agent dims do not match env spec (N=%d/%d A=%d/%d d_obs=%d/%d)", dims->n_agents,
                spec->n_agents, dims->n_actions, spec->n_actions, dims->d_obs, 8 * spec->U);
    p->L = make_agent_layout(*dims);
    MLG_REQUIRE(p->L.Ap <= 16 * RO_MAXAT, "rollout_policy: n_actions=%d does not fit %d action tiles", dims->n_actions,
                RO_MAXAT);
    const int tiles = (RE * spec->n_agents + 15) / 16;
    p->waves = tiles < 8 ? tiles : 8;
    p->tpw = (tiles + p->waves - 1) / p->waves;
    MLG_REQUIRE(p->tpw <= 4, "rollout_policy: %d agent tiles per wave > 4 (too many agents per env)", p->tpw);
    MLG_REQUIRE(p->L.H == 32 || p->L.H == 64 || p->L.H == 128,
                "rollout_policy: rnn_hidden_dim=%d unsupported (32, 64, 128)", p->L.H);
    p->lay = make_rollout_lds(p->L, spec->U, spec->n_agents, true);
    p->wlds = p->lay.total * 4 <= LDS_LIMIT_BYTES;
    if (!p->wlds) {
        p->lay = make_rollout_lds(p->L, spec->U, spec->n_agents, false);
        MLG_REQUIRE(p->lay.total * 4 <= LDS_LIMIT_BYTES, "rollout_policy: the env state of %d units does not fit in LDS",
                    spec->U);
    }
    snprintf(p->name, sizeof p->name, "policy-%s/tpw%d", p->wlds ? "lds" : "global", p->tpw);
    return 0;
}

template <int H, int TPW>
int launch_policy(const PolicyPlan& p, int grid, hipStream_t s, const MlgEnvSpec& spec, const MlgEnvState& st,
                  const Sides& sd, const MlgRunInfo& info, int flags) {
    if (p.wlds) return launch_policy_t<H, TPW, true>(grid, p.waves * 64, s, spec, st, p.L, sd, info, flags, p.lay);
    return launch_policy_t<H, TPW, false>(grid, p.waves * 64, s, spec, st, p.L, sd, info, flags, p.lay);
}

}

extern "C" int mlg_rollout_policy_describe(const MlgEnvSpec* spec, const MlgAgentDims* dims, char* name,
                                           int32_t name_cap, int64_t* lds_bytes) {
    if (check_spec(spec) || check_agent_dims(dims)) return 1;
    MLG_REQUIRE(name && name_cap > 0 && lds_bytes, "rollout_policy_describe: null output");
    PolicyPlan plan;
    if (int rc = plan_policy(spec, dims, &plan)) return rc;
    MLG_REQUIRE((size_t)name_cap > strlen(plan.name), "rollout_policy_describe: name buffer of %d bytes too small",
                name_cap);
    strcpy(name, plan.name);
    *lds_bytes = (int64_t)plan.lay.total * 4;
    return 0;
}

extern "C" int mlg_rollout_policy(const MlgEnvSpec* spec, MlgEnvState* st, const MlgAgentDims* dims,
                                  const float* packed, MlgBatch* batch, MlgRunInfo* info, float epsilon,
                                  int32_t test_mode, int32_t mask_before_softmax, int32_t test_greedy, void* stream) {
    if (check_spec(spec) || check_state(st) || check_agent_dims(dims)) return 1;
    MLG_REQUIRE(packed && batch && info, "rollout_policy: null pointer");
    if (check_rollout_batch(batch, spec, st, "rollout_policy")) return 1;
    MLG_REQUIRE(info->ep_len && info->ret && info->won && info->draw, "rollout_policy: run info has null tensors");
    PolicyPlan plan;
    if (int rc = plan_policy(spec, dims, &plan)) return rc;
    hipStream_t s = (hipStream_t)stream;
    Sides sd;
    sd.bt[0] = sd.bt[1] = *batch;
    sd.P[0] = sd.P[1] = packed;
    sd.eps[0] = sd.eps[1] = test_mode ? 0.f : epsilon;
    sd.ns = 1;
    sd.nh = spec->n_agents;
    const int flags = (test_mode ? 1 : 0) | (mask_before_softmax ? 2 : 0) | (test_greedy ? 4 : 0);
    const int grid = (st->B + RE - 1) / RE;
    int rc = 0;
#define MLG_RO(HH, TT) rc = launch_policy<HH, TT>(plan, grid, s, *spec, *st, sd, *info, flags)
#define MLG_RO_H(HH)               \
    if (plan.tpw == 1) MLG_RO(HH, 1);      \
    else if (plan.tpw == 2) MLG_RO(HH, 2); \
    else if (plan.tpw == 3) MLG_RO(HH, 3); \
    else MLG_RO(HH, 4)
    if (plan.L.H == 64) {
        MLG_RO_H(64);
    } else if (plan.L.H == 32) {
        MLG_RO_H(32);
    } else {
        MLG_RO_H(128);
    }
#undef MLG_RO_H
#undef MLG_RO
    if (rc) return rc;
    return mlg::check_launch("rollout_policy_kernel");
}
```

### ma-league_amd/maleague/_native.py

```python
from __future__ import annotations

import ctypes
import os

import torch

MAXU = 64
_LIB_PATH = os.environ.get("MLG_LIB") or os.path.join(os.path.dirname(os.path.abspath(__file__)), "_lib",
                                                      "libmaleague.so")


class NativeError(RuntimeError):
    """Raised when a libmaleague call fails (the C side's mlg_last_error())."""


class MlgEnvSpec(ctypes.Structure):
    _fields_ = [("U", ctypes.c_int32), ("n_agents", ctypes.c_int32), ("n_actions", ctypes.c_int32),
                ("grid", ctypes.c_int32), ("episode_limit", ctypes.c_int32), ("stochastic", ctypes.c_int32),
                ("policy_team", ctypes.c_int32), ("n_policy_teams", ctypes.c_int32),
                ("team", ctypes.c_int32 * MAXU), ("role", ctypes.c_int32 * MAXU), ("melee", ctypes.c_int32 * MAXU),
                ("agent_unit", ctypes.c_int32 * MAXU), ("scripted", ctypes.c_int32 * 2), ("seed", ctypes.c_uint64)]


class MlgEnvState(ctypes.Structure):
    _fields_ = [("x", ctypes.c_void_p), ("y", ctypes.c_void_p), ("hp", ctypes.c_void_p), ("t", ctypes.c_void_p),
                ("episode", ctypes.c_void_p), ("B", ctypes.c_int32)]


class MlgBatch(ctypes.Structure):
    _fields_ = [("state", ctypes.c_void_p), ("obs", ctypes.c_void_p), ("actions", ctypes.c_void_p),
                ("avail", ctypes.c_void_p), ("reward", ctypes.c_void_p), ("terminated", ctypes.c_void_p),
                ("actions_onehot", ctypes.c_void_p), ("filled", ctypes.c_void_p), ("B", ctypes.c_int32),
                ("T1", ctypes.c_int32), ("ring_slot0", ctypes.c_int32), ("ring_size", ctypes.c_int32),
                ("full_write", ctypes.c_int32), ("rows", ctypes.c_void_p), ("slot_extent", ctypes.c_void_p)]


class MlgRunInfo(ctypes.Structure):
    _fields_ = [("ep_len", ctypes.c_void_p), ("ret", ctypes.c_void_p), ("won", ctypes.c_void_p),
                ("draw", ctypes.c_void_p), ("agent_rows", ctypes.c_void_p), ("ret_away", ctypes.c_void_p)]


class MlgAgentParams(ctypes.Structure):
    _fields_ = [(n, ctypes.c_void_p) for n in ["fc1_w", "fc1_b", "w_ih", "b_ih", "w_hh", "b_hh", "fc2_w", "fc2_b"]]


class MlgAgentDims(ctypes.Structure):
    _fields_ = [(n, ctypes.c_int32) for n in ["d_obs", "n_actions", "n_agents", "hidden", "d_in", "obs_last_action",
                                              "obs_agent_id"]]


class MlgFFParams(ctypes.Structure):
    _fields_ = [(n, ctypes.c_void_p) for n in ["fc1_w", "fc1_b", "fc2_w", "fc2_b"]]


class MlgQMixParams(ctypes.Structure):
    _fields_ = [(n, ctypes.c_void_p) for n in ["hw1_0w", "hw1_0b", "hw1_2w", "hw1_2b", "hwf_0w", "hwf_0b", "hwf_2w",
                                              "hwf_2b", "hb1_w", "hb1_b", "v0_w", "v0_b", "v2_w", "v2_b"]] + \
               [(n, ctypes.c_int32) for n in ["n_agents", "state_dim", "embed_dim", "hypernet_embed",
                                              "hypernet_layers"]]


class MlgLearnerCfg(ctypes.Structure):
    _fields_ = [(n, ctypes.c_int32) for n in ["B", "T", "N", "A", "d_obs", "H", "S", "E", "HE", "hypernet_layers",
                                              "mixer", "double_q", "obs_last_action", "obs_agent_id"]] + \
               [(n, ctypes.c_float) for n in ["gamma", "lr", "optim_alpha", "optim_eps", "grad_norm_clip"]] + \
               [("agent", ctypes.c_int32),
                ("distinct", ctypes.c_int32)]


class MlgLearnerBufs(ctypes.Structure):
    _fields_ = [("batch", MlgBatch)] + [(n, ctypes.c_void_p) for n in ["params", "grads", "square_avg",
                                                                      "target_params", "workspace", "stats",
                                                                      "target_sync", "trained_steps", "host_rows"]]


class MlgEntityEnvSpec(ctypes.Structure):
    _fields_ = [("base", MlgEnvSpec), ("min_agents", ctypes.c_int32), ("max_agents", ctypes.c_int32)]


class MlgEntityBatch(ctypes.Structure):
    _fields_ = [(n, ctypes.c_void_p) for n in ["entities", "obs_mask", "entity_mask", "actions", "avail", "reward",
                                              "terminated", "actions_onehot", "filled"]] + \
               [(n, ctypes.c_int32) for n in ["B", "T1", "ring_slot0", "ring_size", "full_write"]] + \
               [("rows", ctypes.c_void_p), ("slot_extent", ctypes.c_void_p)]


class MlgRefilDims(ctypes.Structure):
    _fields_ = [(n, ctypes.c_int32) for n in ["n_agents", "n_entities", "entity_shape", "n_actions",
                                              "entity_last_action", "attn_embed_dim", "attn_n_heads",
                                              "rnn_hidden_dim"]]



class MlgRefilLearnerCfg(ctypes.Structure):
    _fields_ = [(n, ctypes.c_int32) for n in ["B", "T", "n_agents", "n_entities", "entity_shape", "n_actions",
                                              "entity_last_action", "attn_embed_dim", "attn_n_heads", "rnn_hidden_dim",
                                              "hypernet_embed", "mixing_embed_dim", "double_q",
                                              "softmax_mixing_weights", "imagine", "mixer"]] + \
               [(n, ctypes.c_float) for n in ["gamma", "lmbda", "lr", "optim_alpha", "optim_eps", "grad_norm_clip"]]


class MlgRefilLearnerBufs(ctypes.Structure):
    _fields_ = [("batch", MlgEntityBatch)] + [(n, ctypes.c_void_p) for n in ["groupA", "params", "grads", "square_avg",
                                                                           "target_params", "workspace", "stats",
                                                                           "trained_steps", "target_sync",
                                                                           "host_rows"]]


class MlgCrossplayPair(ctypes.Structure):
    _fields_ = [("home", ctypes.c_int32), ("away", ctypes.c_int32), ("spec", ctypes.c_int32)]


class MlgCrossplay(ctypes.Structure):
    _fields_ = [("packed_pool", ctypes.c_void_p), ("n_pool", ctypes.c_int32), ("n_pairs", ctypes.c_int32),
                ("pairs", ctypes.c_void_p), ("host_pairs", ctypes.c_void_p), ("specs", ctypes.c_void_p),
                ("host_specs", ctypes.c_void_p), ("n_specs", ctypes.c_int32), ("E", ctypes.c_int32),
                ("episode0", ctypes.c_uint32), ("workspace", ctypes.c_void_p), ("workspace_floats", ctypes.c_int64),
                ("ep_len", ctypes.c_void_p), ("ret", ctypes.c_void_p), ("ret_away", ctypes.c_void_p),
                ("won", ctypes.c_void_p), ("draw", ctypes.c_void_p), ("summary", ctypes.c_void_p)]


class MlgComaCfg(ctypes.Structure):
    _fields_ = [(n, ctypes.c_int32) for n in ["B", "T", "N", "A", "d_obs", "S", "hidden"]] + \
               [(n, ctypes.c_float) for n in ["lr", "optim_eps", "grad_norm_clip"]] + \
               [(n, ctypes.c_double) for n in ["gamma", "td_lambda", "optim_alpha"]]


class MlgComaBufs(ctypes.Structure):
    _fields_ = [("batch", MlgBatch)] + [(n, ctypes.c_void_p) for n in ["params", "grads", "square_avg",
                                                                      "target_params", "workspace", "q_vals",
                                                                      "targets", "stats", "counters"]]


_P = ctypes.c_void_p
_I = ctypes.c_int32
SIGNATURES = {
    "mlg_packed_agent_size": (ctypes.c_int64, [_P]),
    "mlg_pack_agent": (ctypes.c_int, [_P, _P, _P, _P]),
    "mlg_env_reset": (ctypes.c_int, [_P, _P, _P]),
    "mlg_env_step": (ctypes.c_int, [_P, _P, _P, _P, _P, _P, _P, _P]),
    "mlg_env_observe": (ctypes.c_int, [_P, _P, _P, _P, _P, _P]),
    "mlg_rollout": (ctypes.c_int, [_P, _P, _P, _P, _P, _P, ctypes.c_float, _I, _P]),
    "mlg_rollout_selfplay": (ctypes.c_int, [_P, _P, _P, _P, _P, _P, _P, _P, ctypes.c_float, ctypes.c_float, _I, _P]),
    "mlg_rollout_describe": (ctypes.c_int, [_P, _P, _I, _P, _I, _P]),
    "mlg_agent_forward": (ctypes.c_int, [_P, _P, _P, _P, _P, _P, _I, _P]),
    "mlg_mac_forward": (ctypes.c_int, [_P, _P, _P, _I, _P, _P, _P, _P]),
    "mlg_select_actions": (ctypes.c_int, [_P, _P, _I, _I, _I, _P, _P, _I, ctypes.c_float, _P, _P, _P]),
    "mlg_qmix_forward": (ctypes.c_int, [_P, _P, _P, _P, _I, _P]),
    "mlg_agent_backward_workspace_floats": (ctypes.c_int64, [_P, _I]),
    "mlg_agent_backward": (ctypes.c_int, [_P] * 11 + [_I, _P]),
    "mlg_qmix_backward_workspace_floats": (ctypes.c_int64, [_P, _I]),
    "mlg_qmix_backward": (ctypes.c_int, [_P] * 7 + [_I, _P]),
    "mlg_qlearner_param_counts": (ctypes.c_int64, [_P, _P, _P]),
    "mlg_qlearner_workspace_floats": (ctypes.c_int64, [_P]),
    "mlg_qlearner_inline_rows": (ctypes.c_int, []),
    "mlg_qlearner_train": (ctypes.c_int, [_P, _P, _P]),
    "mlg_qlearner_describe": (ctypes.c_int, [_P, _P, _I]),
    "mlg_zero_slots_bytes": (ctypes.c_int, [_P, _P, _I, _I, _I, _P]),
    "mlg_refil_packed_agent_size": (ctypes.c_int64, [_P]),
    "mlg_refil_pack_agent": (ctypes.c_int, [_P, _P, _P, _P]),
    "mlg_refil_agent_forward": (ctypes.c_int, [_P, _P, _P, _P, _P, _P, _P, _P, _I, _P]),
    "mlg_refil_rollout": (ctypes.c_int, [_P, _P, _P, _P, _P, _P, ctypes.c_float, _I, _P]),
    "mlg_refil_rollout_describe": (ctypes.c_int, [_P, _P, _P, _I, _P]),
    "mlg_refil_attention": (ctypes.c_int, [_P] * 6 + [_I] * 4 + [_P] * 2),
    "mlg_refil_packed_mixer_size": (ctypes.c_int64, [_P]),
    "mlg_refil_pack_mixer": (ctypes.c_int, [_P, _P, _P, _P]),
    "mlg_refil_mixer_forward": (ctypes.c_int, [_P] * 7 + [_I, _P, _I, _P]),
    "mlg_refil_attention_backward_workspace_floats": (ctypes.c_int64, [_I] * 4),
    "mlg_refil_attention_backward": (ctypes.c_int, [_P] * 7 + [_I] * 4 + [_P] * 4),
    "mlg_refil_mixer_backward_workspace_floats": (ctypes.c_int64, [_P, _I, _I]),
    "mlg_refil_mixer_backward": (ctypes.c_int, [_P] * 7 + [_I] + [_P] * 4 + [_I, _P]),
    "mlg_refil_agent_backward_workspace_floats":(ctypes.c_int64, [_P, _I]),
    "mlg_refil_agent_backward": (ctypes.c_int, [_P] * 11 + [_I, _P]),
    "mlg_refil_param_counts": (ctypes.c_int64, [_P, _P, _P]),
    "mlg_refil_workspace_floats": (ctypes.c_int64, [_P]),
    "mlg_refil_train": (ctypes.c_int, [_P, _P, _P]),
    "mlg_debug_set_stamps": (ctypes.c_int, [_P]),
    "mlg_debug_set_learner_stamps": (ctypes.c_int, [_P]),
    "mlg_refil_debug_set_stamps": (ctypes.c_int, [_P]),
    "mlg_league_record_runs": (ctypes.c_int, [_P, _P, _I, _P, _I, _P]),
    "mlg_refil_draw_groups": (ctypes.c_int, [_I, _I, ctypes.c_uint64, ctypes.c_uint32, _P, _P]),
    "mlg_crossplay_workspace_floats": (ctypes.c_int64, [_P, _I, _I]),
    "mlg_crossplay_rollout": (ctypes.c_int, [_P, _P, _P]),
    "mlg_pack_agent_pool": (ctypes.c_int, [_P, _P, ctypes.c_int64, _I, _P, _P]),
    "mlg_policy_probs": (ctypes.c_int, [_P, _P, _I, _I, ctypes.c_float, _I, _I, _P, _P]),
    "mlg_policy_probs_backward": (ctypes.c_int, [_P, _P, _P, _I, _I, ctypes.c_float, _I, _I, _P, _P]),
    "mlg_select_multinomial": (ctypes.c_int, [_P, _P, _I, _I, _I, _P, _P, _I, _I, _P, _P]),
    "mlg_rollout_policy": (ctypes.c_int, [_P, _P, _P, _P, _P, _P, ctypes.c_float, _I, _I, _I, _P]),
    "mlg_rollout_policy_describe": (ctypes.c_int, [_P, _P, _P, _I, _P]),
    "mlg_coma_policy_loss": (ctypes.c_int, [_P, _P, _P, _P, _P, _I, _I, _I, _P, _P, _P]),
    "mlg_coma_param_count": (ctypes.c_int64, [_P]),
    "mlg_coma_workspace_floats": (ctypes.c_int64, [_P]),
    "mlg_coma_critic_train": (ctypes.c_int, [_P, _P, _P]),
    "mlg_coma_target_update": (ctypes.c_int, [_P, _P, ctypes.c_int64, _P, _I, _P]),
    "mlg_ff_packed_size": (ctypes.c_int64, [_P]),
    "mlg_ff_pack": (ctypes.c_int, [_P, _P, _P, _P]),
    "mlg_ff_forward": (ctypes.c_int, [_P, _P, _P, _P, _I, _P]),
    "mlg_ff_mac_forward": (ctypes.c_int, [_P, _P, _P, _I, _P, _P]),
    "mlg_ff_backward_workspace_floats": (ctypes.c_int64, [_P, _I]),
    "mlg_ff_backward": (ctypes.c_int, [_P] * 8 + [_I, _P]),
    "mlg_rollout_ff": (ctypes.c_int, [_P, _P, _P, _P, _P, _P, ctypes.c_float, _I, _P]),
    "mlg_rollout_ff_describe": (ctypes.c_int, [_P, _P, _P, _I, _P]),
    "mlg_mac_forward_distinct": (ctypes.c_int, [_P, _P, _P, _I, _P, _P, _P, _P]),
    "mlg_rollout_distinct": (ctypes.c_int, [_P, _P, _P, _P, _P, _P, ctypes.c_float, _I, _P]),
    "mlg_rollout_distinct_describe": (ctypes.c_int, [_P, _P, _P, _I, _P]),
    "mlg_last_error": (ctypes.c_char_p, []),
    "mlg_version": (ctypes.c_char_p, []),
}

_lib = None


def lib_path() -> str:
    return _LIB_PATH


def load(require_gpu: bool = False):
    global _lib
    if _lib is None:
        if not os.path.exists(_LIB_PATH):
            raise NativeError(f"libmaleague.so not found at {_LIB_PATH}; build it with `make -C ma-league_amd` "
                              "(or __graft_entry__.build()). There is no CPU fallback.")
        lib = ctypes.CDLL(_LIB_PATH)
        for name, (res, args) in SIGNATURES.items():
            fn = getattr(lib, name)
            fn.restype = res
# ... 91 lines not shown
```

### ma-league_amd/maleague/components/replay_buffer.py

```python
from __future__ import annotations

import weakref
from types import SimpleNamespace

import numpy as np
import torch

from .episode_batch import EpisodeBatch


class ReplayBuffer(EpisodeBatch):
    def __init__(self, scheme, groups, buffer_size: int, max_seq_length: int, preprocess=None, device="cpu"):
        super().__init__(scheme, groups, buffer_size, max_seq_length, preprocess=preprocess, device=device)
        self.buffer_size = buffer_size
        self.buffer_index = 0
        self.episodes_in_buffer = 0
        self._outstanding = []
        self.slot_extent = (torch.full((buffer_size,), max_seq_length, dtype=torch.int32, device=device)
                            if torch.device(device).type == "cuda" else None)

    def update(self, data, bs=slice(None), ts=slice(None), mark_filled=True):
        super().update(data, bs, ts, mark_filled)
        self.invalidate_extents(bs)

    def extent_ptr(self):
        ext = getattr(self, "slot_extent", None)
        return None if ext is None else ext.data_ptr()

    def invalidate_extents(self, slots=None):
        if getattr(self, "slot_extent", None) is not None:
            if slots is None:
                self.slot_extent.fill_(self.max_seq_length)
            else:
                self.slot_extent[slots] = self.max_seq_length

    def has_outstanding(self) -> bool:
        self._outstanding = [r for r in getattr(self, "_outstanding", []) if r() is not None and r().attached]
        return bool(self._outstanding)

    def _register(self, ring_batch: "RingEpisodeBatch"):
        if not hasattr(self, "_outstanding"):
            self._outstanding = []
        self._outstanding.append(weakref.ref(ring_batch))

    def _detach_outstanding(self):
        for r in getattr(self, "_outstanding", []):
            rb = r()
            if rb is not None and rb.attached:
                rb.detach()
        self._outstanding = []

    def insert_episode_batch(self, ep_batch: EpisodeBatch):
        if isinstance(ep_batch, RingEpisodeBatch) and ep_batch.attached and ep_batch.ring is self:
            if ep_batch.slot0 != self.buffer_index:
                raise RuntimeError("ring episodes must be inserted in the order they were written")
            self._advance(ep_batch.batch_size)
            ep_batch.committed = True
            return
        self._detach_outstanding()
        room = self.buffer_size - self.buffer_index
        if ep_batch.batch_size > room:
            self.insert_episode_batch(ep_batch[0:room, :])
            self.insert_episode_batch(ep_batch[room:, :])
            return
        dst = slice(self.buffer_index, self.buffer_index + ep_batch.batch_size)
        self._copy_in(ep_batch, dst)
        self.invalidate_extents(dst)
        self.buffer_index += ep_batch.batch_size
        self.episodes_in_buffer = max(self.episodes_in_buffer, self.buffer_index)
        self.buffer_index %= self.buffer_size
        assert self.buffer_index < self.buffer_size

    def _advance(self, n: int):
        room = self.buffer_size - self.buffer_index
        if n > room:
            self._advance(room)
            self._advance(n - room)
            return
        self.buffer_index += n
        self.episodes_in_buffer = max(self.episodes_in_buffer, self.buffer_index)
        self.buffer_index %= self.buffer_size

    def _copy_in(self, ep_batch: EpisodeBatch, dst: slice):
        t = slice(0, ep_batch.max_seq_length)
        src = ep_batch.data.transition_data
        derived = {v[0] for v in self.preprocess.values()}
        for key, value in src.items():
            if key not in self.data.transition_data:
                raise KeyError(f"{key} not found in transition or episode data")
            if key in self.preprocess and self.preprocess[key][0] in src:
                self.data.transition_data[key][dst, t] = value.to(self.data.transition_data[key].dtype)
                continue
            if key in derived or key not in self.preprocess:
                self.data.transition_data[key][dst, t] = value.to(self.data.transition_data[key].dtype)
            else:
                self.update({key: value}, dst, t, mark_filled=False)
        if ep_batch.data.episode_data:
            self.update(ep_batch.data.episode_data, dst)

    def can_sample(self, batch_size: int) -> bool:
        return self.episodes_in_buffer >= batch_size

    def sample(self, batch_size: int, view: bool = False) -> EpisodeBatch:
        assert self.can_sample(batch_size)
        if self.episodes_in_buffer == batch_size:
            ep_ids = np.arange(batch_size)
            if not view:
                return self[:batch_size]
        else:
            ep_ids = np.random.choice(self.episodes_in_buffer, batch_size, replace=False)
        if view and torch.device(self.device).type == "cuda":
            return SampledEpisodeBatch(self, ep_ids)
        return self[ep_ids]

    def __repr__(self):
        return (f"ReplayBuffer. {self.episodes_in_buffer}/{self.buffer_size} episodes. "
                f"Keys:{self.scheme.keys()} Groups:{self.groups.keys()}")


class RingEpisodeBatch(EpisodeBatch):

    def __init__(self, ring: ReplayBuffer, slot0: int, batch_size: int):
        self.ring, self.slot0, self.committed = ring, slot0, False
        self.scheme, self.groups, self.preprocess = ring.scheme, ring.groups, ring.preprocess
        self.batch_size, self.max_seq_length, self.device = batch_size, ring.max_seq_length, ring.device
        self._data = None
        ring._register(self)

    @property
    def attached(self) -> bool:
        return self.ring is not None and not self.committed

    def detach(self):
        d = self.data
        self._data = SimpleNamespace(transition_data={k: v.clone() for k, v in d.transition_data.items()},
                                     episode_data={k: v.clone() for k, v in d.episode_data.items()})
        self.ring = None

    @property
    def data(self):
        if self._data is None:
            size, B = self.ring.buffer_size, self.batch_size
            if self.slot0 + B <= size:
                sel = lambda v: v[self.slot0:self.slot0 + B]
            else:
                idx = (torch.arange(B, device=self.device) + self.slot0) % size
                sel = lambda v: v.index_select(0, idx)
            self._data = SimpleNamespace(
                transition_data={k: sel(v) for k, v in self.ring.data.transition_data.items()},
                episode_data={k: sel(v) for k, v in self.ring.data.episode_data.items()})
        return self._data

    @data.setter
    def data(self, value):
        self._data = value


class SampledEpisodeBatch(EpisodeBatch):

    def __init__(self, ring: ReplayBuffer, ep_ids):
        self.ring = ring
        self.scheme, self.groups, self.preprocess = ring.scheme, ring.groups, ring.preprocess
        self.batch_size, self.max_seq_length, self.device = len(ep_ids), ring.max_seq_length, ring.device
        self.ep_ids = np.asarray(ep_ids, dtype=np.int64)
        self.host_rows = np.ascontiguousarray(self.ep_ids, dtype=np.int32)
        self._rows = None
        self._data = None

    @property
    def rows(self) -> torch.Tensor:
        if self._rows is None:
            host = torch.from_numpy(self.host_rows)
            if torch.device(self.device).type == "cuda":
                host = host.pin_memory()
            self._rows = host.to(self.device, non_blocking=True)
        return self._rows

    @property
    def data(self):
        if self._data is None:
            idx = self.rows.long()
            self._data = SimpleNamespace(
                transition_data={k: v.index_select(0, idx) for k, v in self.ring.data.transition_data.items()},
                episode_data={k: v.index_select(0, idx) for k, v in self.ring.data.episode_data.items()})
        return self._data

    @data.setter
    def data(self, value):
        self._data = value
```

### ma-league_amd/maleague/learners/q_learner.py

```python
from __future__ import annotations

import copy
import os

import torch

from .. import _native
from ..components.batch_view import mlg_batch
from ..controllers.distinct_controller import DistinctMAC
from ..modules.agents import DQNAgentNetwork
from ..modules.mixers import QMixer, VDNMixer
from ..utils.checkpoint import save_module, save_optimizer

AGENT_ORDER = ["fc1.weight", "fc1.bias", "gru.weight_ih", "gru.weight_hh", "gru.bias_ih", "gru.bias_hh",
               "fc2.weight", "fc2.bias"]
QMIX_ORDER = ["hyper_w_1.0.weight", "hyper_w_1.0.bias", "hyper_w_1.2.weight", "hyper_w_1.2.bias",
              "hyper_w_final.0.weight", "hyper_w_final.0.bias", "hyper_w_final.2.weight", "hyper_w_final.2.bias",
              "hyper_b_1.weight", "hyper_b_1.bias", "V.0.weight", "V.0.bias", "V.2.weight", "V.2.bias"]
QMIX1_ORDER = ["hyper_w_1.weight", "hyper_w_1.bias", "hyper_w_final.weight", "hyper_w_final.bias",
               "hyper_b_1.weight", "hyper_b_1.bias", "V.0.weight", "V.0.bias", "V.2.weight", "V.2.bias"]


class FlatParams:

# ... 2 lines not shown
        n = sum(p.numel() for p in params)
        self.flat = torch.empty(n, dtype=torch.float32, device=device)
        self.views = []
        off = 0
        for p in params:
            k = p.numel()
            self.flat[off:off + k].copy_(p.detach().reshape(-1))
            p.data = self.flat[off:off + k].view_as(p)
            self.views.append((p, off, k))
            off += k

    def attach_grads(self, gflat):
        for p, off, k in self.views:
            p.grad = gflat[off:off + k].view_as(p)


class Learner:
    def __init__(self, mac, scheme, logger, args, name=None):
        self.mac = mac
        self.scheme = scheme
        self.logger = logger
        self.args = args
        self.name = f'{"" if name is None else name}_{self.__class__.__name__.lower()}_'
        self.log_stats_t = -self.args.learner_log_interval - 1
        self.optimiser = None

    def parameters(self):
        raise NotImplementedError()

    def train(self, batch, t_env: int, episode_num: int):
        raise NotImplementedError()

    def update_targets(self):
        pass


class QLearner(Learner):
    def __init__(self, mac, scheme, logger, args, name=None):
        super().__init__(mac, scheme, logger, args, name)
        self.last_target_update_episode = 0
        self.mixer = None
        if args.mixer is not None:
            if args.mixer == "vdn":
                self.mixer = VDNMixer()
            elif args.mixer == "qmix":
                self.mixer = QMixer(args)
            else:
                raise ValueError(f"Mixer {args.mixer} not recognised.")
            self.target_mixer = copy.deepcopy(self.mixer)
        self.target_mac = copy.deepcopy(mac)
        self.device = torch.device(getattr(args, "device", "cuda"))
        self._ws = None
        self._stats = None
        self._last_stats = None
        self._stats_fresh = False
        self.train_calls = 0
        self._distinct = isinstance(mac, DistinctMAC)
        self._tcount = None
        self._tviews = None
        if self._distinct:
            mac.enable_autograd()
            if isinstance(self.mixer, QMixer):
                self.mixer.enable_autograd()

    def parameters(self):
        return list(self.mac.parameters()) + (list(self.mixer.parameters()) if self.mixer is not None else [])

    def _target_parameters(self):
        return list(self.target_mac.parameters()) + (list(self.target_mixer.parameters())
                                                     if self.mixer is not None else [])

    def _check_order(self):
        for agent in (self.mac.agents if self._distinct else [self.mac.agent]):
            names = [n for n, _ in agent.named_parameters()]
            order = list(getattr(agent, "PARAM_ORDER", AGENT_ORDER))
            if names != order:
                raise RuntimeError(f"agent parameter order {names} != kernel layout {order}")
        if isinstance(self.mixer, QMixer):
            names = [n for n, _ in self.mixer.named_parameters()]
            order = QMIX1_ORDER if self.mixer.hypernet_layers == 1 else QMIX_ORDER
            if names != order:
                raise RuntimeError(f"mixer parameter order {names} != kernel layout {order}")

    def build_optimizer(self):
        self._check_order()
        nets = [self.mac.agents, self.target_mac.agents] if self._distinct else [self.mac.agent, self.target_mac.agent]
        for m in nets + ([self.mixer, self.target_mixer] if self.mixer else []):
            m.to(self.device)
        params = self.parameters()
        self._flat = FlatParams(params, self.device)
        self._tflat = FlatParams(self._target_parameters(), self.device)
        self._grads = torch.zeros_like(self._flat.flat)
        self._sq = torch.zeros_like(self._flat.flat)
        self._flat.attach_grads(self._grads)
        a = self.args
        self.optimiser = torch.optim.RMSprop(params=params, lr=a.lr, alpha=a.optim_alpha, eps=a.optim_eps)
        self._step = torch.zeros((), dtype=torch.float32)
        for p, off, k in self._flat.views:
            self.optimiser.state[p] = {"step": self._step, "square_avg": self._sq[off:off + k].view_as(p)}
        self._stats = torch.zeros(8, dtype=torch.float32, device=self.device)
        self._online().mark_dirty()
        self._target().mark_dirty()

    def _online(self):
        return self.mac if self._distinct else self.mac.agent

    def _target(self):
        return self.target_mac if self._distinct else self.target_mac.agent

    def _trained_counters(self):
        agents = self.mac.agents
        if self._tcount is None or not all(a.trained_counter_is(v) for a, v in zip(agents, self._tviews)):
            self._tcount = torch.stack([a.trained_counter(self.device) for a in agents])
            self._tviews = [a.seat_trained_counter(self._tcount[i]) for i, a in enumerate(agents)]
        return self._tcount

    def _cfg(self, B, T):
        a = self.args
        d = self._online().dims()
        mixer = 2 if isinstance(self.mixer, QMixer) else (1 if isinstance(self.mixer, VDNMixer) else 0)
        return _native.MlgLearnerCfg(B=B, T=T, N=a.n_agents, A=a.n_actions, d_obs=d.d_obs, H=a.rnn_hidden_dim,
                             S=int(a.state_shape), E=int(getattr(a, "mixing_embed_dim", 32)),
                             HE=int(getattr(a, "hypernet_embed", 64)), hypernet_layers=int(getattr(a, "hypernet_layers", 1)),
                             mixer=mixer, double_q=int(bool(a.double_q)), obs_last_action=int(bool(a.obs_last_action)),
                             obs_agent_id=int(bool(a.obs_agent_id)), gamma=float(a.gamma), lr=float(a.lr),
                             optim_alpha=float(a.optim_alpha), optim_eps=float(a.optim_eps),
                             grad_norm_clip=float(a.grad_norm_clip),
                             agent=int(not self._distinct and isinstance(self.mac.agent, DQNAgentNetwork)),
                             distinct=int(self._distinct))

    def train(self, batch, t_env, episode_num: int):
        if self.optimiser is None:
            raise RuntimeError("call build_optimizer() before train()")
        if self._distinct:
            which = os.environ.get("MLG_DISTINCT_LEARNER", "fused")
            if which == "unrolled":
                return self._train_distinct(batch, t_env, episode_num)
            if which != "fused":
                raise ValueError(f"MLG_DISTINCT_LEARNER={which!r} not recognised (fused, unrolled)")
        lib = _native.load(require_gpu=True)
        cfg = self._cfg(batch.batch_size, batch.max_seq_length)
        need = lib.mlg_qlearner_workspace_floats(_native.byref(cfg))
        if need < 0:
            raise _native.NativeError(lib.mlg_last_error().decode())
        if self._ws is None or self._ws.numel() < need:
            self._ws = torch.zeros(int(need * 1.25) + 1024, dtype=torch.float32, device=self.device)
        host_rows = getattr(batch, "host_rows", None)
        if host_rows is not None and (batch.batch_size > lib.mlg_qlearner_inline_rows()
                                      or getattr(batch, "_data", None) is not None):
            host_rows = None
        mb, keep = mlg_batch(batch, device_rows=host_rows is None)
        sync = (episode_num - self.last_target_update_episode) / self.args.target_update_interval >= 1.0
        counter = self._trained_counters() if self._distinct else self.mac.agent.trained_counter(self.device)
        bufs = _native.MlgLearnerBufs(mb, self._flat.flat.data_ptr(), self._grads.data_ptr(), self._sq.data_ptr(),
                                      self._tflat.flat.data_ptr(), self._ws.data_ptr(), self._stats.data_ptr(),
                                      self._tflat.flat.data_ptr() if sync else None, counter.data_ptr(),
                                      None if host_rows is None else host_rows.ctypes.data)
        _native.call("mlg_qlearner_train", _native.byref(cfg), _native.byref(bufs), _native.stream_ptr(self.device))
        del keep
        self._step += 1
        self._online().mark_dirty()
        self.train_calls += 1
        if sync:
            self._target().mark_dirty()
            self.logger.info(f"Updated {self.name}target network.")
            self.last_target_update_episode = episode_num
        self._stats_fresh = True
        if callable(t_env):
            up = getattr(t_env, "upper", None)
            if up is not None and up() - self.log_stats_t < self.args.learner_log_interval:
                return
            t_env = t_env()
        if t_env - self.log_stats_t >= self.args.learner_log_interval:
            for k, v in self.last_stats.items():
                self.logger.log_stat(self.name + k, v, t_env)
            self.log_stats_t = t_env

    def _train_distinct(self, batch, t_env, episode_num):
        a = self.args
        rewards = batch["reward"][:, :-1]
        actions = batch["actions"][:, :-1]
        terminated = batch["terminated"][:, :-1].float()
        mask = batch["filled"][:, :-1].float()
        mask[:, 1:] = mask[:, 1:] * (1 - terminated[:, :-1])
        avail = batch["avail_actions"]
        T = batch.max_seq_length
        te = batch["filled"][:, :, 0].sum(dim=1).max().clamp(min=2)
        mask = mask * (torch.arange(T - 1, device=mask.device) < te - 1).view(1, T - 1, 1).float()
        self.mac.init_hidden(batch.batch_size)
        mac_out = torch.stack([self.mac.forward(batch, t=t) for t in range(T)], dim=1)
        chosen = torch.gather(mac_out[:, :-1], dim=3, index=actions).squeeze(3)
        stored = (batch["filled"][:, :, 0] != 0).unsqueeze(2)
        alive = ((avail[..., 1:] != 0).any(dim=3) & stored).flatten(0, 1).any(dim=0)
        chosen = torch.where(alive.view(1, 1, -1), chosen, chosen.detach())
        with torch.no_grad():
            self.target_mac.init_hidden(batch.batch_size)
            tmac = torch.stack([self.target_mac.forward(batch, t=t) for t in range(T)][1:], dim=1)
            tmac[avail[:, 1:] == 0] = -9999999
            if a.double_q:
                md = mac_out.detach().clone()
                md[avail == 0] = -9999999
                cur_max = md[:, 1:].max(dim=3, keepdim=True)[1]
                target_max = torch.gather(tmac, 3, cur_max).squeeze(3)
            else:
                target_max = tmac.max(dim=3)[0]
        if self.mixer is not None:
            chosen = self.mixer(chosen, batch["state"][:, :-1])
            with torch.no_grad():
                target_max = self.target_mixer(target_max, batch["state"][:, 1:])
        targets = rewards + a.gamma * (1 - terminated) * target_max
        td = chosen - targets.detach()
        mask = mask.expand_as(td)
        mtd = td * mask
        n = mask.sum()
        loss = (mtd ** 2).sum() / n
        self._grads.zero_()
        self._flat.attach_grads(self._grads)
        loss.backward()
        params = self.parameters()
        grad_norm = torch.nn.utils.clip_grad_norm_(params, a.grad_norm_clip)
        steps_done = float(self._step)
        self.optimiser.step()
        self._step.fill_(steps_done + 1)
        self.mac.mark_dirty()
        self.train_calls += 1
        if (episode_num - self.last_target_update_episode) / a.target_update_interval >= 1.0:
            self.update_targets()
            self.last_target_update_episode = episode_num
        with torch.no_grad():
            steps = torch.count_nonzero(mask)
            for ag in self.mac.agents:
                ag.add_trained_steps(steps)
            self._stats[:7] = torch.stack([loss.detach(), grad_norm.detach().reshape(()), mtd.abs().sum() / n,
                                           (chosen * mask).sum() / (n * a.n_agents),
                                           (targets * mask).sum() / (n * a.n_agents), n, steps.float()])
        self._stats_fresh = True
        if callable(t_env):
            up = getattr(t_env, "upper", None)
            if up is not None and up() - self.log_stats_t < a.learner_log_interval:
                return
            t_env = t_env()
        if t_env - self.log_stats_t >= a.learner_log_interval:
            for k, v in self.last_stats.items():
                self.logger.log_stat(self.name + k, v, t_env)
            self.log_stats_t = t_env

    @property
    def last_stats(self):
        if self._stats is None or not self._stats_fresh:
            return self._last_stats
        st = self._stats.cpu()
        self._last_stats = {"loss": float(st[0]), "grad_norm": float(st[1]), "td_error_abs": float(st[2]),
                            "q_taken_mean": float(st[3]), "target_mean": float(st[4])}
        self._stats_fresh = False
        return self._last_stats

    def update_targets(self):
        self._tflat.flat.copy_(self._flat.flat)
        (self.target_mac if self._distinct else self.target_mac.agent).mark_dirty()
        self.logger.info(f"Updated {self.name}target network.")

    def cuda(self):
        pass

    def save_models(self, path, name):
        self.mac.save_models(path, name=self.name)
        if self.mixer is not None:
            save_module(self.mixer, f"{path}/{self.name}mixer.th")
        save_optimizer(self.optimiser, f"{path}/{self.name}opt.th")

    def load_models(self, path):
        self.mac.load_models(path, self.name)
        self.target_mac.load_models(path, self.name)
        if self.mixer is not None:
            sd = torch.load(f"{path}/{self.name}mixer.th", map_location=lambda s, loc: s, weights_only=True)
            self.mixer.load_state_dict(sd)
        opt = torch.load(f"{path}/{self.name}opt.th", map_location=lambda s, loc: s, weights_only=True)
        self.optimiser.load_state_dict(opt)
        if self._distinct:
            self._tflat.flat.copy_(self._flat.flat)
        for p, off, k in self._flat.views:
            st = self.optimiser.state.get(p, {})
            if "square_avg" in st:
                self._sq[off:off + k].copy_(st["square_avg"].reshape(-1))
            if "step" in st:
                self._step.fill_(float(st["step"]))
            self.optimiser.state[p] = {"step": self._step, "square_avg": self._sq[off:off + k].view_as(p)}
        self._online().mark_dirty()
        self._target().mark_dirty()
```

### ma-league_amd/maleague/steppers/parallel_stepper.py

```python
from __future__ import annotations

from collections import deque
from collections.abc import Sequence
from functools import partial

import numpy as np
import torch

from .. import _native
from ..components.batch_view import mlg_batch
from ..components.episode_batch import EpisodeBatch
from ..components.replay_buffer import RingEpisodeBatch
from ..controllers.distinct_controller import DistinctMAC
from ..custom_logging import Collectibles, Originator
from ..envs.teams_env import TeamsEnvSpec, VecEnvState
from ..exceptions import MultiAgentControllerNotInitialized
from ..modules.agents import DQNAgentNetwork


def _same_device(a, b) -> bool:
    a, b = torch.device(a), torch.device(b)
    if a.type != b.type:
        return False
    if a.type == "cuda":
        cur = torch.cuda.current_device()
        return (cur if a.index is None else a.index) == (cur if b.index is None else b.index)
    return True


class EnvInfos(Sequence):

    def __init__(self, won, draw, ep_len):
        self._won, self._draw, self._len, self._order = won, draw, ep_len, None

    def _o(self):
        if self._order is None:
            self._order = np.lexsort((np.arange(len(self._len)), self._len))
        return self._order

    @property
    def won(self):
        return self._won[self._o()]

    @property
    def draw(self):
        return self._draw[self._o()]

    def __len__(self):
        return len(self._draw)

    def __getitem__(self, i):
        if isinstance(i, slice):
            return [self[k] for k in range(*i.indices(len(self)))]
        k = self._o()[i]
        return {"battle_won": [bool(self._won[k, 0]), bool(self._won[k, 1])], "draw": bool(self._draw[k])}


class LazyEnvInfos(Sequence):

    def __init__(self, stepper, run_id):
        self._stepper, self._run_id, self._infos = stepper, run_id, None

    def _get(self):
        if self._infos is None:
            self._infos = self._stepper._env_infos_of(self._run_id)
        return self._infos

    def __len__(self):
        return self._stepper.batch_size

    def __getitem__(self, i):
        return self._get()[i]


class EnvStepper:
    def __init__(self, args, logger, log_start_t=0):
        self.args = args
        self.logger = logger
        self.batch_size = None
        self.t_env = 0
        self.is_initalized = False
        self.log_start_t = log_start_t or 0

    @property
    def log_t(self):
        return self.log_start_t + self.t_env


class ParallelStepper(EnvStepper):
    def __init__(self, args, logger, log_start_t=0):
        super().__init__(args, logger, log_start_t)
        self.batch_size = args.batch_size_run
        self.device = torch.device(args.device)
        env_args = dict(args.env_args)
        env_args.setdefault("seed", getattr(args, "seed", 0))
        self.spec = self._build_spec(env_args, getattr(args, "config_dir", None))
        self.policy_team_id = self.spec.policy_team
        self.env_info = self.spec.env_info()
        self.episode_limit = self.env_info["episode_limit"]
        self._cspec = self.spec.to_c()
        self.envs = VecEnvState(self.spec, self.batch_size, self.device)
        B = self.batch_size
        self._info = torch.zeros(6 * B, dtype=torch.int32, device=self.device)
        self.agent_rows = torch.zeros(1, dtype=torch.int64, device=self.device)
        pin = self.device.type == "cuda"
        self._info_hosts = [torch.zeros(6 * B, dtype=torch.int32, pin_memory=pin) for _ in range(self._HOST_RING)]
        self._pendings = deque()
        self._last_end_ev = None
        self._host_slot = None
        self._post = []
        self._runs = {}
        self._run_id = 0
        self._t = 0
        self.env_steps_this_run = 0
        self.new_batch_fn = None
        self.home_mac = None
        self.home_batch = None
        self.away_mac = None
        self.timing = None
        self.timing_every = 1
        self.t_history = None
        self._launches = 0
        self._ring = None

    _batch_keys = ("state", "obs", "actions", "avail_actions", "reward", "terminated", "actions_onehot", "filled")
    _HOST_RING = 4
    _ZERO_COPY = True

    def _build_spec(self, env_args, config_dir):
        return TeamsEnvSpec.from_env_args(env_args, config_dir)

    def set_match_build_plan(self, plan):
        env_args = dict(self.args.env_args)
        env_args["match_build_plan"] = plan
        env_args.setdefault("seed", getattr(self.args, "seed", 0))
        spec = self._build_spec(env_args, getattr(self.args, "config_dir", None))
        old = self.spec
        if (spec.U, spec.n_agents, spec.n_actions, spec.policy_team, spec.n_policy_teams) != \
                (old.U, old.n_agents, old.n_actions, old.policy_team, old.n_policy_teams):
            raise ValueError(f"match_build_plan changes the env shape (U {old.U} -> {spec.U}, agents {old.n_agents} -> "
                             f"{spec.n_agents}, policy teams {old.n_policy_teams} -> {spec.n_policy_teams}): a "
                             "roster swap keeps the team sizes")
        self.args.env_args = env_args
        self.spec = spec
        self.envs.spec = spec
        self._cspec = spec.to_c()

    def _to_mlg(self, batch):
        return mlg_batch(batch)

    def _rollout(self, mb, run_info, epsilon, test_mode):
        if isinstance(self.home_mac, DistinctMAC):
            mac = self.home_mac
            _native.call("mlg_rollout_distinct", _native.byref(self._cspec), _native.byref(self.envs.to_c()),
                         _native.byref(mac.dims()), _native.ptr(mac.packed()), _native.byref(mb),
                         _native.byref(run_info), float(epsilon), int(bool(test_mode)), _native.stream_ptr(self.device))
            return
        agent = self.home_mac.agent
        if isinstance(agent, DQNAgentNetwork):
            self._refuse_dqn_policy()
        st = self.envs.to_c()
        if isinstance(agent, DQNAgentNetwork):
            _native.call("mlg_rollout_ff", _native.byref(self._cspec), _native.byref(st), _native.byref(agent.dims()),
                         _native.ptr(agent.packed()), _native.byref(mb), _native.byref(run_info), float(epsilon),
                         int(bool(test_mode)), _native.stream_ptr(self.device))
            return
        if getattr(self.home_mac, "agent_output_type", "q") == "pi_logits":
            sel = self.home_mac.action_selector
            _native.call("mlg_rollout_policy", _native.byref(self._cspec), _native.byref(st),
                         _native.byref(agent.dims()), _native.ptr(agent.packed()), _native.byref(mb),
                         _native.byref(run_info), float(epsilon), int(bool(test_mode)),
                         int(bool(getattr(self.home_mac.args, "mask_before_softmax", True))),
                         int(bool(getattr(sel, "test_greedy", True))), _native.stream_ptr(self.device))
            return
        _native.call("mlg_rollout", _native.byref(self._cspec), _native.byref(st), _native.byref(agent.dims()),
                     _native.ptr(agent.packed()), _native.byref(mb), _native.byref(run_info), float(epsilon),
                     int(bool(test_mode)), _native.stream_ptr(self.device))

    _SELFPLAY = False

    def _refuse_dqn_policy(self):
        if getattr(self.home_mac, "agent_output_type", "q") == "pi_logits":
            raise NotImplementedError("agent='dqn' with agent_output_type='pi_logits' is not supported: the policy "
                                      "rollout (mlg_rollout_policy) runs the recurrent agent (agent='rnn') only")

    def describe_rollout(self):
        if self.home_mac is None:
            raise MultiAgentControllerNotInitialized()
        if isinstance(self.home_mac, DistinctMAC):
            return _native.rollout_distinct_describe(self._cspec, self.home_mac.dims())
        if isinstance(self.home_mac.agent, DQNAgentNetwork):
            self._refuse_dqn_policy()
            return _native.rollout_ff_describe(self._cspec, self.home_mac.agent.dims())
        if getattr(self.home_mac, "agent_output_type", "q") == "pi_logits":
            return _native.rollout_policy_describe(self._cspec, self.home_mac.agent.dims())
        return _native.rollout_describe(self._cspec, self.home_mac.agent.dims(), self._SELFPLAY)

    def initialize(self, scheme, groups, preprocess, home_mac, away_mac=None):
        if away_mac is not None:
            raise NotImplementedError("ParallelStepper drives one policy; self-play (home + away MAC) is "
                                      "SelfPlayParallelStepper (steppers.SELF_REGISTRY['parallel'])")
        self.new_batch_fn = partial(EpisodeBatch, scheme, groups, self.batch_size, self.episode_limit + 1,
                                    preprocess=preprocess, device=self.device)
        self.home_mac = home_mac
        self.is_initalized = True

    def get_env_info(self):
        return self.env_info

    @property
    def t_env(self) -> int:
        self._resolve()
        return self._t_env

    @t_env.setter
    def t_env(self, value: int):
        if getattr(self, "_pendings", None):
            self._resolve()
        self._t_env = int(value)

    @property
    def t(self) -> int:
        self._resolve()
        return self._t

    @t.setter
    def t(self, value: int):
        self._t = int(value)

    @property
    def last_run(self):
        self._resolve()
        self._finish_post()
        return self._runs[self._run_id][0] if self._run_id in self._runs else None

    def t_env_bounds(self):
        lo = self._t_env
        pend = sum(1 for p in self._pendings if not p[2])
        return lo, lo + pend * self.batch_size * self.episode_limit

    def _epsilon(self, mac, test_mode):
        sel = mac.action_selector
        lo, hi = self.t_env_bounds()
        e = sel.schedule.eval(lo)
        if hi != lo and sel.schedule.eval(hi) != e:
            e = sel.schedule.eval(self.t_env)
        sel.epsilon = e
        if test_mode:
            sel.epsilon = 0.0
            return 0.0
        return float(e)

    def _zero_copy(self) -> bool:
        return self._ZERO_COPY and self.device.type == "cuda"

    def _reserve_host(self):
        while len(self._pendings) >= self._HOST_RING:
            self._resolve_one()
        return self._info_hosts[(self._run_id + 1) % self._HOST_RING]

    def _queue_summary(self, test_mode):
        ev = None
        if self._zero_copy():
            host = self._host_slot
            ev = self._last_end_ev
        else:
            host = self._reserve_host()
            host.copy_(self._info, non_blocking=True)
        self._last_end_ev = None
        if ev is None:
            ev = torch.cuda.Event()
            ev.record()
        self._run_id += 1
        self._pendings.append((self._run_id, ev, test_mode, host))

    def _resolve(self):
        while getattr(self, "_pendings", None):
            self._resolve_one()

    def _resolve_one(self):
        run_id, ev, test_mode, buf = self._pendings.popleft()
        ev.synchronize()
        B = self.batch_size
        host = buf.numpy().copy()
        ep_len = host[0:B]
        self._t = int(ep_len.max())
        if self.t_history is not None:
            self.t_history.append((run_id, self._t))
        if not test_mode:
            self.env_steps_this_run = int(ep_len.sum())
            self._t_env += self.env_steps_this_run
        self._post.append((run_id, host, self._t, self._t_env, test_mode))

    def _finish_post(self):
        B = self.batch_size
        mode_now = self.logger.test_mode
        for run_id, host, t_max, t_env, test_mode in self._post:
            self.logger.test_mode = test_mode
            ep_len = host[0:B]
            won = host[B:3 * B].reshape(B, 2) != 0
            draw = host[3 * B:4 * B] != 0
            ret = host[4 * B:5 * B].view(np.float32)
            ret_away = host[5 * B:6 * B].view(np.float32)
            infos = EnvInfos(won, draw, ep_len)
            last = {"ep_len": torch.from_numpy(ep_len), "returns": torch.from_numpy(ret)}
            if self.away_mac is not None:
                last["away_returns"] = torch.from_numpy(ret_away)
            self._runs[run_id] = (last, infos)
            self._runs.pop(run_id - 2, None)
            self.logger.collect(Collectibles.RETURN, ret, origin=Originator.HOME, parallel=True)
            if self.away_mac is not None:
                self.logger.collect(Collectibles.RETURN, ret_away, origin=Originator.AWAY, parallel=True)
            self.logger.collect(Collectibles.WON, won[:, 0], origin=Originator.HOME, parallel=True)
            self.logger.collect(Collectibles.WON, won[:, 1], origin=Originator.AWAY, parallel=True)
            self.logger.collect(Collectibles.DRAW, draw, parallel=True)
            self.logger.collect(Collectibles.STEPS, t_max, parallel=True)
            self.logger.log(t_env)
        self.logger.test_mode = mode_now
        self._post = []

    def _env_infos_of(self, run_id):
        self._resolve()
        self._finish_post()
        if run_id not in self._runs:
            raise RuntimeError("env_infos of an old run are no longer available")
        return self._runs[run_id][1]

    def flush(self):
        self._resolve()
        self._finish_post()

    def attach_replay(self, buffer) -> bool:
        ok = (_same_device(buffer.device, self.device) and buffer.max_seq_length == self.episode_limit + 1
              and buffer.buffer_size >= self.batch_size
              and all(k in buffer.data.transition_data for k in self._batch_keys))
        self._ring = buffer if ok else None
        return ok

    def save_replay(self):
        pass

    def close_env(self):
        pass

    def reset(self):
        pass

    def _launch(self, batch: EpisodeBatch, epsilon: float, test_mode: bool):
        mb, keep = self._to_mlg(batch)
        self._launch_mb(mb, epsilon, test_mode)
        del keep

    def last_run_info(self) -> torch.Tensor:
        return self._host_slot if self._zero_copy() and self._host_slot is not None else self._info

    def _run_info(self):
        B = self.batch_size
        if self._zero_copy():
            self._host_slot = self._reserve_host()
            info = self._host_slot
        else:
            info = self._info
        return _native.MlgRunInfo(info[0:B].data_ptr(), info[4 * B:5 * B].data_ptr(), info[B:3 * B].data_ptr(),
                                  info[3 * B:4 * B].data_ptr(), self.agent_rows.data_ptr(),
                                  info[5 * B:6 * B].data_ptr())

    def _timed_launch(self) -> bool:
        self._launches += 1
        return self.timing is not None and self.timing_every > 0 and self._launches % self.timing_every == 0

    def _launch_mb(self, mb, epsilon: float, test_mode: bool):
        run_info = self._run_info()
        (self.home_mac if isinstance(self.home_mac, DistinctMAC) else self.home_mac.agent).packed()
        ev = None
        if self._timed_launch():
            ev = (torch.cuda.Event(enable_timing=True), torch.cuda.Event(enable_timing=True))
            ev[0].record()
        self._rollout(mb, run_info, epsilon, test_mode)
        if ev is not None:
            ev[1].record()
            self.timing.append(ev)
            self._last_end_ev = ev[1]

    def run(self, test_mode=False):
        if self.home_mac is None:
            raise MultiAgentControllerNotInitialized()
        self.reset()
        self.logger.test_mode = test_mode
        self.home_mac.init_hidden(batch_size=self.batch_size)
        eps = self._epsilon(self.home_mac, test_mode)
        ring = self._ring if not test_mode else None
        if ring is not None and ring.has_outstanding():
            ring = None
        if ring is not None:
            slot0 = ring.buffer_index
            mb, keep = self._to_mlg(ring)
            mb.B, mb.ring_slot0, mb.ring_size, mb.full_write = self.batch_size, slot0, ring.buffer_size, 1
            mb.slot_extent = ring.extent_ptr()
            self._launch_mb(mb, eps, test_mode)
            del keep
            self.home_batch = RingEpisodeBatch(ring, slot0, self.batch_size)
        else:
            self.home_batch = self.new_batch_fn()
            self._launch(self.home_batch, eps, test_mode)
        self._queue_summary(test_mode)
        self._finish_post()
        return self.home_batch, LazyEnvInfos(self, self._run_id)


class EpisodeStepper(ParallelStepper):

    def __init__(self, args, logger, log_start_t=0):
        assert args.batch_size_run == 1
        super().__init__(args, logger, log_start_t)

    @property
    def epsilon(self):
        return getattr(self.home_mac.action_selector, "epsilon", None)

    def run(self, test_mode=False):
        batch, infos = super().run(test_mode)
        self.logger.log_stat("home_epsilon", self.epsilon, self.log_t)
        return batch, infos[-1]
```

Measured before the change: 204.0 million.

## Overlap learner with rollout via per-slot ready flags and side-stream gating

The rollout kernel now publishes a per-replay-slot ready tag with release semantics once each env's episode finishes. The learner forks onto a side stream and runs a spin-wait kernel that polls only the sampled rows belonging to the current run, so training can start before the whole rollout kernel completes. This is meant to hide learner time behind the rollout tail. In exchange it adds extra zeroing work, s_waitcnt and release fences inside the rollout loop, a spinning wavefront that occupies a CU, and a timeout path that flags errors.

```diff
diff --git a/include/maleague.h b/include/maleague.h
--- a/include/maleague.h
+++ b/include/maleague.h
@@ -55,6 +55,8 @@
     int32_t *draw;
     uint64_t *agent_rows;
     float *ret_away;
+    int32_t *slot_ready;
+    int32_t run_tag;
 } MlgRunInfo;
 
 typedef struct {
@@ -140,6 +142,11 @@
     float *target_sync;
     double *trained_steps;
     const int32_t *host_rows;
+    const int32_t *slot_ready;
+    int32_t run_tag;
+    int32_t n_wait_rows;
+    const int32_t *wait_rows;
+    int32_t *gate_error;
 } MlgLearnerBufs;
 
 int64_t mlg_qlearner_param_counts(const MlgLearnerCfg *c, int64_t *n_agent, int64_t *n_mixer);
diff --git a/ma-league_amd/csrc/distinct.hip b/ma-league_amd/csrc/distinct.hip
--- a/ma-league_amd/csrc/distinct.hip
+++ b/ma-league_amd/csrc/distinct.hip
@@ -276,6 +276,7 @@
     MLG_REQUIRE(mlg::aligned16(packed_pool), "rollout_distinct: packed_pool must be 16-byte aligned");
     if (check_rollout_batch(batch, spec, st, "rollout_distinct")) return 1;
     MLG_REQUIRE(info->ep_len && info->ret && info->won && info->draw, "rollout_distinct: run info has null tensors");
+    MLG_REQUIRE(!info->slot_ready, "rollout_distinct: slot_ready is not supported (mlg_rollout's v7 / v2 kernels only)");
     DxPlan plan;
     if (int rc = plan_distinct(spec, dims, &plan)) return rc;
     hipStream_t s = (hipStream_t)stream;
diff --git a/ma-league_amd/csrc/learner.hip b/ma-league_amd/csrc/learner.hip
--- a/ma-league_amd/csrc/learner.hip
+++ b/ma-league_amd/csrc/learner.hip
@@ -2432,6 +2432,39 @@
     return 0;
 }
 
+struct WaitRows {
+    int32_t n;
+    int32_t rows[MLG_INLINE_ROWS];
+};
+
+constexpr long long GATE_TIMEOUT_TICKS = 200000000LL;
+__global__ void __launch_bounds__(64) wait_slots_kernel(const int32_t* __restrict__ slot_ready, int32_t tag, WaitRows w,
+                                                        int32_t* err) {
+    const int l = threadIdx.x;
+    const bool mine = l < w.n;
+    const int32_t* p = slot_ready + (mine ? w.rows[l] : 0);
+    const long long t0 = wall_clock64();
+    bool ok = !mine;
+    while (true) {
+        if (!ok) ok = __hip_atomic_load(p, __ATOMIC_RELAXED, __HIP_MEMORY_SCOPE_AGENT) == tag;
+        if (__all(ok)) break;
+        if (wall_clock64() - t0 > GATE_TIMEOUT_TICKS) {
+            if (l == 0) __hip_atomic_store(err, 1, __ATOMIC_RELAXED, __HIP_MEMORY_SCOPE_AGENT);
+            break;
+        }
+        __builtin_amdgcn_s_sleep(32);
+    }
+    __builtin_amdgcn_fence(__ATOMIC_ACQUIRE, "agent");
+}
+
+namespace {
+int train_on(const MlgLearnerCfg* c, const MlgLearnerBufs* b, Plan& p, hipStream_t s) {
+    if (c->H == 64) return run_train<64>(p, c, b, s);
+    if (c->H == 32) return run_train<32>(p, c, b, s);
+    return run_train<128>(p, c, b, s);
+}
+}
+
 extern "C" int mlg_qlearner_train(const MlgLearnerCfg* c, const MlgLearnerBufs* b, void* stream) {
     if (check_cfg(c)) return 1;
     MLG_REQUIRE(b && b->params && b->grads && b->square_avg && b->target_params && b->workspace && b->stats,
@@ -2442,9 +2475,29 @@
     MLG_REQUIRE(bt.B == c->B && bt.T1 >= c->T, "qlearner_train: batch B=%d T1=%d vs cfg B=%d T=%d", bt.B, bt.T1, c->B, c->T);
     MLG_REQUIRE(!b->host_rows || c->B <= MLG_INLINE_ROWS, "qlearner_train: host_rows needs B <= %d (got %d)",
                 MLG_INLINE_ROWS, c->B);
+    MLG_REQUIRE(b->n_wait_rows >= 0 && b->n_wait_rows <= MLG_INLINE_ROWS, "qlearner_train: n_wait_rows=%d not in 0..%d",
+                b->n_wait_rows, MLG_INLINE_ROWS);
+    MLG_REQUIRE(b->n_wait_rows == 0 || (b->wait_rows && b->slot_ready && b->gate_error),
+                "qlearner_train: wait_rows needs slot_ready, wait_rows and gate_error");
     Plan p = make_plan(c, bt.T1);
     hipStream_t s = (hipStream_t)stream;
-    if (c->H == 64) return run_train<64>(p, c, b, s);
-    if (c->H == 32) return run_train<32>(p, c, b, s);
-    return run_train<128>(p, c, b, s);
-}
+    if (b->n_wait_rows > 0) {
+        mlg::SideStream* side = mlg::side_stream(s);
+        if (side && side->armed && side->armed_tag == b->run_tag) {
+            side->armed = false;
+            MLG_REQUIRE(hipStreamWaitEvent(side->s, side->ev[4], 0) == hipSuccess, "qlearner_train: side stream fork");
+            WaitRows w;
+            w.n = b->n_wait_rows;
+            for (int i = 0; i < MLG_INLINE_ROWS; ++i) w.rows[i] = i < w.n ? b->wait_rows[i] : 0;
+            hipLaunchKernelGGL(wait_slots_kernel, dim3(1), dim3(64), 0, side->s, b->slot_ready, b->run_tag, w,
+                               b->gate_error);
+            int rc = mlg::check_launch("wait_slots_kernel");
+            if (!rc) rc = train_on(c, b, p, side->s);
+            const bool joined = mlg::fork_join(side, 5, side->s, s);
+            if (rc) return rc;
+            MLG_REQUIRE(joined, "qlearner_train: side stream join");
+            return 0;
+        }
+    }
+    return train_on(c, b, p, s);
+}
diff --git a/ma-league_amd/csrc/mlg_host.h b/ma-league_amd/csrc/mlg_host.h
--- a/ma-league_amd/csrc/mlg_host.h
+++ b/ma-league_amd/csrc/mlg_host.h
@@ -35,7 +35,9 @@
 
 struct SideStream {
     hipStream_t s = nullptr;
-    hipEvent_t ev[4] = {nullptr, nullptr, nullptr, nullptr};
+    hipEvent_t ev[6] = {nullptr, nullptr, nullptr, nullptr, nullptr, nullptr};
+    bool armed = false;
+    int32_t armed_tag = 0;
 };
 inline SideStream* side_stream(hipStream_t caller) {
     static SideStream side[64];
diff --git a/ma-league_amd/csrc/refil.hip b/ma-league_amd/csrc/refil.hip
--- a/ma-league_amd/csrc/refil.hip
+++ b/ma-league_amd/csrc/refil.hip
@@ -900,6 +900,7 @@
     MLG_REQUIRE(st->B == bt.B && bt.T1 >= sp.episode_limit + 1, "refil_rollout: B=%d/%d T1=%d (episode_limit %d)", st->B,
                 bt.B, bt.T1, sp.episode_limit);
     MLG_REQUIRE(info->ep_len && info->ret && info->won && info->draw, "refil_rollout: run info has null buffers");
+    MLG_REQUIRE(!info->slot_ready, "refil_rollout: slot_ready is not supported (mlg_rollout's v7 / v2 kernels only)");
     if (bt.B == 0) return 0;
     int p = 1;
     while (p < sp.grid) p <<= 1;
diff --git a/ma-league_amd/csrc/rollout.hip b/ma-league_amd/csrc/rollout.hip
--- a/ma-league_amd/csrc/rollout.hip
+++ b/ma-league_amd/csrc/rollout.hip
@@ -168,6 +168,42 @@
     }
     int64_t* ac = bt.actions + r0 * N;
     for (int x = lane; x < n * N; x += nl) gst(ac + x, (int64_t)0);
+    for (int x = lane; x < n; x += nl) {
+        gst(bt.reward + r0 + x, 0.f);
+        gst(bt.terminated + r0 + x, (uint8_t)0);
+        gst(bt.filled + r0 + x, (int64_t)0);
+    }
+}
+
+__device__ inline void zero_slot_steps_rolled(const MlgBatch& bt, int slot, int z0, int z1, int N, int A, int S, int DO,
+                                       int lane, int nl) {
+    if (z0 >= z1) return;
+    const int64_t r0 = (int64_t)slot * bt.T1 + z0;
+    const int n = z1 - z0;
+    auto z16 = [&](float* p, int per) {
+        float* b = p + r0 * per;
+        if (per % 4 == 0) {
+            uint4* q = reinterpret_cast<uint4*>(b);
+#pragma clang loop unroll(disable) interleave(disable) vectorize(disable)
+            for (int x = lane; x < n * per / 4; x += nl) gst(q + x, make_uint4(0u, 0u, 0u, 0u));
+        } else {
+#pragma clang loop unroll(disable) interleave(disable) vectorize(disable)
+            for (int x = lane; x < n * per; x += nl) gst(b + x, 0.f);
+        }
+    };
+    z16(bt.obs, N * DO);
+    z16(bt.state, S);
+    int* av = bt.avail + r0 * N * A;
+    float* oh = bt.actions_onehot + r0 * N * A;
+#pragma clang loop unroll(disable) interleave(disable) vectorize(disable)
+    for (int x = lane; x < n * N * A; x += nl) {
+        gst(av + x, 0);
+        gst(oh + x, 0.f);
+    }
+    int64_t* ac = bt.actions + r0 * N;
+#pragma clang loop unroll(disable) interleave(disable) vectorize(disable)
+    for (int x = lane; x < n * N; x += nl) gst(ac + x, (int64_t)0);
+#pragma clang loop unroll(disable) interleave(disable) vectorize(disable)
     for (int x = lane; x < n; x += nl) {
         gst(bt.reward + r0 + x, 0.f);
         gst(bt.terminated + r0 + x, (uint8_t)0);
@@ -1244,12 +1280,44 @@
     env_observe(C, spec, E.slot, t + 1, E.e, hbase, hl, E.u, sp);
 }
 
+template <bool ROLLED = false>
 __device__ inline void env_lane_tail(const EnvCtx& C, EnvLane& E, int steps, int hl) {
     const int z0 = E.zcur & 0xFFFF, zend = E.zcur >> 16;
     if (!C.bt.full_write || E.st != 2 || z0 >= zend || E.b >= C.B) return;
     const int z1 = z0 + steps < zend ? z0 + steps : zend;
-    zero_slot_steps(C.bt, E.slot, z0, z1, C.N, C.A, 6 * C.U, 8 * C.U, hl, 32);
+    if constexpr (ROLLED)
+        zero_slot_steps_rolled(C.bt, E.slot, z0, z1, C.N, C.A, 6 * C.U, 8 * C.U, hl, 32);
+    else
+        zero_slot_steps(C.bt, E.slot, z0, z1, C.N, C.A, 6 * C.U, 8 * C.U, hl, 32);
     E.zcur = (E.zcur & ~0xFFFF) | z1;
+}
+
+constexpr int ENV_COMPLETE = 4, ENV_PUBLISHED = 6;
+
+__device__ inline void env_lane_mark_complete(const EnvCtx& C, EnvLane& E, int hl) {
+    if (E.st != 2 || E.zcur < 0 || E.b >= C.B) return;
+    if (C.bt.full_write && (E.zcur & 0xFFFF) < (E.zcur >> 16)) return;
+    E.zcur |= (int)0x80000000u;
+    if (hl == 0) C.R.status[E.e] = ENV_COMPLETE;
+}
+
+__device__ __forceinline__ uint32_t publish_plan(const EnvCtx& C, int lane) {
+    const int stv = C.R.status[lane & 15];
+    const uint32_t pend = (uint32_t)__ballot(lane < 16 && stv == ENV_COMPLETE);
+    if (!pend) return 0u;
+    const uint32_t run = (uint32_t)__ballot(lane < 16 && stv < 2);
+    const uint32_t idle = ~(run | (run >> 1)) & 0x5555u;
+    return idle ? pend | ((uint32_t)(__builtin_ctz(idle) >> 1) << 16) : 0u;
+}
+
+__device__ __forceinline__ void release_begin() { asm volatile("buffer_wbl2 sc1" ::: "memory"); }
+
+__device__ inline void publish_slots(const EnvCtx& C, uint32_t mask, int lane) {
+    asm volatile("s_waitcnt vmcnt(0)" ::: "memory");
+    if (lane < 16 && ((mask >> lane) & 1u)) {
+        __hip_atomic_store(C.info.slot_ready + C.R.slot[lane], C.info.run_tag, __ATOMIC_RELAXED, __HIP_MEMORY_SCOPE_AGENT);
+        C.R.status[lane] = ENV_PUBLISHED;
+    }
 }
 
 __device__ inline void env_lane_finish(const EnvCtx& C, const MlgEnvState& st, EnvLane& E, int hl) {
@@ -1319,7 +1387,7 @@
     return b;
 }
 
-template <int H, bool G8, int SN = 0, int SU = 0>
+template <int H, bool G8, int SN = 0, int SU = 0, bool PUB = false>
 __device__ __forceinline__ void rollout_v2_body(const MlgEnvSpec& spec, const MlgEnvState& st, const AgentLayout& L,
                                                 const float* __restrict__ P, const MlgBatch& bt_arg, const MlgRunInfo& info,
                                                 float eps, int test_mode, const RolloutLds2& lay, int DU, int DN,
@@ -1381,7 +1449,15 @@
         else
             ph_gru<H>(W, lay, fm, hc, hn, SR, N, j, gi, G, lane);
         sp.mark(1);
+        uint32_t pub = 0u;
+        if constexpr (PUB) {
+            pub = publish_plan(C, lane);
+            if (pub) asm volatile("s_waitcnt vmcnt(0)" ::: "memory");
+            if ((int)(pub >> 16) != wave) pub = 0u;
+        }
         lds_barrier();
+        if constexpr (PUB)
+            if (pub) release_begin();
         if constexpr (G8) sp.mark(13);
         if constexpr (G8)
             ph_fc2_g8<H>(spec, L, lay, fm, wmap, C.R, bt, hn, tiles, wave, NW, e0, t, eps, test_mode, lane, pre);
@@ -1396,15 +1472,19 @@
         sp.mark(2);
         lds_barrier();
         sp.mark(3);
+        if constexpr (PUB)
+            if (pub) publish_slots(C, pub & 0xFFFFu, lane);
         const EnvCtx Ce = env_ctx_step(C);
         env_lane_step1(Ce, E, t, hl);
         sp.mark(4);
         env_lane_step2(Ce, E, t, hl, sp);
 #if defined(MLG_V7_TAIL_MIXED)
-        if (!E.stepped && (t & 1)) env_lane_tail(Ce, E, 8, hl);
+        const bool tail_now = !E.stepped;
 #else
-        if (__ballot(E.stepped) == 0 && (t & 1)) env_lane_tail(Ce, E, 8, hl);
+        const bool tail_now = PUB ? !E.stepped : __ballot(E.stepped) == 0;
 #endif
+        if (tail_now && (t & 1)) env_lane_tail<PUB>(Ce, E, 8, hl);
+        if constexpr (PUB) env_lane_mark_complete(Ce, E, hl);
         sp.mark(8);
         lds_barrier();
         sp.mark(10);
@@ -1412,18 +1492,27 @@
     sp.flush();
     if (threadIdx.x == 0 && info.agent_rows) atomicAdd(info.agent_rows, (unsigned long long)rows_issued);
     env_lane_finish(C, st, E, hl);
-}
-
-template <int H, bool G8 = false, int SN = 0, int SU = 0>
+    if constexpr (PUB) {
+        asm volatile("s_waitcnt vmcnt(0)" ::: "memory");
+        __syncthreads();
+        if (wave == 0) {
+            const int stl = C.R.status[lane & (REW - 1)];
+            __builtin_amdgcn_fence(__ATOMIC_RELEASE, "agent");
+            publish_slots(C, (uint32_t)__ballot(lane < REW && stl != ENV_PUBLISHED && e0 + lane < C.B), lane);
+        }
+    }
+}
+
+template <int H, bool G8 = false, int SN = 0, int SU = 0, bool PUB = false>
 __global__ void __launch_bounds__(512, 2) rollout_v2_kernel(MlgEnvSpec spec, MlgEnvState st, AgentLayout L,
                                                            const float* __restrict__ P, MlgBatch bt, MlgRunInfo info,
                                                            float eps, int test_mode, RolloutLds2 lay) {
     using S = StaticShape<H, G8, SN, SU>;
     if constexpr (S::on)
-        rollout_v2_body<H, G8, SN, SU>(spec, st, S::L, P, bt, info, eps, test_mode, S::lay, SU, SN, 5 + SU, true);
+        rollout_v2_body<H, G8, SN, SU, PUB>(spec, st, S::L, P, bt, info, eps, test_mode, S::lay, SU, SN, 5 + SU, true);
     else
-        rollout_v2_body<H, G8>(spec, st, L, P, bt, info, eps, test_mode, lay, spec.U, spec.n_agents, spec.n_actions,
-                               G8);
+        rollout_v2_body<H, G8, 0, 0, PUB>(spec, st, L, P, bt, info, eps, test_mode, lay, spec.U, spec.n_agents,
+                                         spec.n_actions, G8);
 }
 
 #include "rollout_sp.inc"
@@ -1659,6 +1748,13 @@
         kern = p.sn == 5   ? rollout_v2_kernel<64, true, 5, 10>
                : p.sn == 3 ? rollout_v2_kernel<64, true, 3, 6>
                            : rollout_v2_kernel<64, true>;
+    if (info.slot_ready) {
+        kern = L.H == 64 ? rollout_v2_kernel<64, false, 0, 0, true> : rollout_v2_kernel<32, false, 0, 0, true>;
+        if (p.arm == Arm::V7)
+            kern = p.sn == 5   ? rollout_v2_kernel<64, true, 5, 10, true>
+                   : p.sn == 3 ? rollout_v2_kernel<64, true, 3, 6, true>
+                               : rollout_v2_kernel<64, true, 0, 0, true>;
+    }
     const int threads = 512, rew = 16;
     if (int rc = allow_lds(kern, p.lds_bytes, "rollout v2")) return rc;
     hipLaunchKernelGGL(kern, dim3((bt.B + rew - 1) / rew), dim3(threads), p.lds_bytes, s, spec, st, L, P, bt, info, eps,
@@ -1815,6 +1911,14 @@
     const float eps = test_mode ? 0.f : epsilon;
     RolloutPlan plan;
     if (int rc = plan_rollout(L, *spec, false, &plan)) return rc;
+    MLG_REQUIRE(!info->slot_ready || plan.arm != Arm::V1,
+                "rollout: slot_ready needs a kernel with env lanes (v7-static, v7, v2); this shape runs %s", plan.name);
+    if (info->slot_ready) {
+        if (mlg::SideStream* side = mlg::side_stream(s)) {
+            side->armed = hipEventRecord(side->ev[4], s) == hipSuccess;
+            side->armed_tag = info->run_tag;
+        }
+    }
     if (plan.arm != Arm::V1) return launch_rollout_v2(s, *spec, *st, L, packed, *batch, *info, eps, test_mode, plan);
     Sides sd;
     sd.bt[0] = sd.bt[1] = *batch;
@@ -1834,6 +1938,7 @@
         check_rollout_batch(away, spec, st, "rollout_selfplay (away)"))
         return 1;
     MLG_REQUIRE(info->ep_len && info->ret && info->won && info->draw, "rollout_selfplay: run info has null tensors");
+    MLG_REQUIRE(!info->slot_ready, "rollout_selfplay: slot_ready is not supported (mlg_rollout's v7 / v2 kernels only)");
     if (check_selfplay_dims(spec, dims)) return 1;
     const AgentLayout L = make_agent_layout(*dims);
     hipStream_t s = (hipStream_t)stream;
diff --git a/ma-league_amd/csrc/rollout_ff.hip b/ma-league_amd/csrc/rollout_ff.hip
--- a/ma-league_amd/csrc/rollout_ff.hip
+++ b/ma-league_amd/csrc/rollout_ff.hip
@@ -165,6 +165,7 @@
     MLG_REQUIRE(mlg::aligned16(packed), "rollout_ff: packed must be 16-byte aligned");
     if (check_rollout_batch(batch, spec, st, "rollout_ff")) return 1;
     MLG_REQUIRE(info->ep_len && info->ret && info->won && info->draw, "rollout_ff: run info has null tensors");
+    MLG_REQUIRE(!info->slot_ready, "rollout_ff: slot_ready is not supported (mlg_rollout's v7 / v2 kernels only)");
     FFPlan plan;
     if (int rc = plan_ff(spec, dims, &plan)) return rc;
     hipStream_t s = (hipStream_t)stream;
diff --git a/ma-league_amd/csrc/rollout_policy.hip b/ma-league_amd/csrc/rollout_policy.hip
--- a/ma-league_amd/csrc/rollout_policy.hip
+++ b/ma-league_amd/csrc/rollout_policy.hip
@@ -258,6 +258,7 @@
     MLG_REQUIRE(packed && batch && info, "rollout_policy: null pointer");
     if (check_rollout_batch(batch, spec, st, "rollout_policy")) return 1;
     MLG_REQUIRE(info->ep_len && info->ret && info->won && info->draw, "rollout_policy: run info has null tensors");
+    MLG_REQUIRE(!info->slot_ready, "rollout_policy: slot_ready is not supported (mlg_rollout's v7 / v2 kernels only)");
     PolicyPlan plan;
     if (int rc = plan_policy(spec, dims, &plan)) return rc;
     hipStream_t s = (hipStream_t)stream;
diff --git a/ma-league_amd/maleague/_native.py b/ma-league_amd/maleague/_native.py
--- a/ma-league_amd/maleague/_native.py
+++ b/ma-league_amd/maleague/_native.py
@@ -37,7 +37,8 @@
 
 class MlgRunInfo(ctypes.Structure):
     _fields_ = [("ep_len", ctypes.c_void_p), ("ret", ctypes.c_void_p), ("won", ctypes.c_void_p),
-                ("draw", ctypes.c_void_p), ("agent_rows", ctypes.c_void_p), ("ret_away", ctypes.c_void_p)]
+                ("draw", ctypes.c_void_p), ("agent_rows", ctypes.c_void_p), ("ret_away", ctypes.c_void_p),
+                ("slot_ready", ctypes.c_void_p), ("run_tag", ctypes.c_int32)]
 
 
 class MlgAgentParams(ctypes.Structure):
@@ -71,7 +72,9 @@
 class MlgLearnerBufs(ctypes.Structure):
     _fields_ = [("batch", MlgBatch)] + [(n, ctypes.c_void_p) for n in ["params", "grads", "square_avg",
                                                                       "target_params", "workspace", "stats",
-                                                                      "target_sync", "trained_steps", "host_rows"]]
+                                                                      "target_sync", "trained_steps", "host_rows"]] + \
+               [("slot_ready", ctypes.c_void_p), ("run_tag", ctypes.c_int32), ("n_wait_rows", ctypes.c_int32),
+                ("wait_rows", ctypes.c_void_p), ("gate_error", ctypes.c_void_p)]
 
 
 class MlgEntityEnvSpec(ctypes.Structure):
diff --git a/ma-league_amd/maleague/components/replay_buffer.py b/ma-league_amd/maleague/components/replay_buffer.py
--- a/ma-league_amd/maleague/components/replay_buffer.py
+++ b/ma-league_amd/maleague/components/replay_buffer.py
@@ -6,6 +6,7 @@
 import numpy as np
 import torch
 
+from .._native import NativeError
 from .episode_batch import EpisodeBatch
 
 
@@ -19,6 +20,31 @@
         self.slot_extent = (torch.full((buffer_size,), max_seq_length, dtype=torch.int32, device=device)
                             if torch.device(device).type == "cuda" else None)
 
+        self._slot_ready = None
+        self._gate_error = None
+        self._run_tag = 0
+        self.last_ready_run = None
+
+    def ready_flags(self) -> torch.Tensor:
+        if getattr(self, "_slot_ready", None) is None:
+            self._slot_ready = torch.zeros(self.buffer_size, dtype=torch.int32, device=self.device)
+            self._gate_error = torch.zeros(1, dtype=torch.int32, device=self.device)
+        return self._slot_ready
+
+    def next_run_tag(self) -> int:
+        self._run_tag = getattr(self, "_run_tag", 0) % 0x7FFFFFFF + 1
+        return self._run_tag
+
+    def gate_error(self) -> torch.Tensor:
+        self.ready_flags()
+        return self._gate_error
+
+    def check_gate(self):
+        err = getattr(self, "_gate_error", None)
+        if err is not None and int(err.item()) != 0:
+            err.zero_()
+            raise NativeError("the learner's early start waited 2 s for rollout slots that were never published")
+
     def update(self, data, bs=slice(None), ts=slice(None), mark_filled=True):
         super().update(data, bs, ts, mark_filled)
         self.invalidate_extents(bs)
@@ -56,7 +82,9 @@
                 raise RuntimeError("ring episodes must be inserted in the order they were written")
             self._advance(ep_batch.batch_size)
             ep_batch.committed = True
+            self.last_ready_run = ep_batch.ready_run
             return
+        self.last_ready_run = None
         self._detach_outstanding()
         room = self.buffer_size - self.buffer_index
         if ep_batch.batch_size > room:
@@ -120,8 +148,9 @@
 
 class RingEpisodeBatch(EpisodeBatch):
 
-    def __init__(self, ring: ReplayBuffer, slot0: int, batch_size: int):
+    def __init__(self, ring: ReplayBuffer, slot0: int, batch_size: int, ready_tag: int = 0):
         self.ring, self.slot0, self.committed = ring, slot0, False
+        self.ready_run = (slot0, batch_size, ready_tag) if ready_tag else None
         self.scheme, self.groups, self.preprocess = ring.scheme, ring.groups, ring.preprocess
         self.batch_size, self.max_seq_length, self.device = batch_size, ring.max_seq_length, ring.device
         self._data = None
@@ -156,6 +185,14 @@
         self._data = value
 
 
+def slots_in_run(rows, run, size):
+    if run is None:
+        return np.zeros(0, dtype=np.int32), 0
+    slot0, n, tag = run
+    rows = np.asarray(rows, dtype=np.int64)
+    return np.ascontiguousarray(rows[(rows - slot0) % size < n], dtype=np.int32), int(tag)
+
+
 class SampledEpisodeBatch(EpisodeBatch):
 
     def __init__(self, ring: ReplayBuffer, ep_ids):
@@ -164,8 +201,12 @@
         self.batch_size, self.max_seq_length, self.device = len(ep_ids), ring.max_seq_length, ring.device
         self.ep_ids = np.asarray(ep_ids, dtype=np.int64)
         self.host_rows = np.ascontiguousarray(self.ep_ids, dtype=np.int32)
+        self.ready_run = getattr(ring, "last_ready_run", None)
         self._rows = None
         self._data = None
+
+    def current_run_rows(self):
+        return slots_in_run(self.host_rows, self.ready_run, self.ring.buffer_size)
 
     @property
     def rows(self) -> torch.Tensor:
diff --git a/ma-league_amd/maleague/learners/q_learner.py b/ma-league_amd/maleague/learners/q_learner.py
--- a/ma-league_amd/maleague/learners/q_learner.py
+++ b/ma-league_amd/maleague/learners/q_learner.py
@@ -178,10 +178,14 @@
         mb, keep = mlg_batch(batch, device_rows=host_rows is None)
         sync = (episode_num - self.last_target_update_episode) / self.args.target_update_interval >= 1.0
         counter = self._trained_counters() if self._distinct else self.mac.agent.trained_counter(self.device)
+        bufs_now = (self._ws, counter)
+        settled = all(a is b for a, b in zip(bufs_now, getattr(self, "_bufs_seen", (None, None))))
+        self._bufs_seen = bufs_now
+        wait = self._early_wait(batch, host_rows, settled)
         bufs = _native.MlgLearnerBufs(mb, self._flat.flat.data_ptr(), self._grads.data_ptr(), self._sq.data_ptr(),
                                       self._tflat.flat.data_ptr(), self._ws.data_ptr(), self._stats.data_ptr(),
                                       self._tflat.flat.data_ptr() if sync else None, counter.data_ptr(),
-                                      None if host_rows is None else host_rows.ctypes.data)
+                                      None if host_rows is None else host_rows.ctypes.data, *wait[1:])
         _native.call("mlg_qlearner_train", _native.byref(cfg), _native.byref(bufs), _native.stream_ptr(self.device))
         del keep
         self._step += 1
@@ -201,6 +205,18 @@
             for k, v in self.last_stats.items():
                 self.logger.log_stat(self.name + k, v, t_env)
             self.log_stats_t = t_env
+
+    def _early_wait(self, batch, host_rows, settled=True):
+        off = (None, None, 0, 0, None, None)
+        if not settled or host_rows is None or self._distinct or isinstance(self.mac.agent, DQNAgentNetwork) or \
+                os.environ.get("MLG_LEARNER_EARLY", "1") == "0" or not hasattr(batch, "current_run_rows"):
+            return off
+        rows, tag = batch.current_run_rows()
+        if len(rows) == 0:
+            return off
+        ring = batch.ring
+        self._gate_ring = ring
+        return (rows, ring.ready_flags().data_ptr(), tag, len(rows), rows.ctypes.data, ring.gate_error().data_ptr())
 
     def _train_distinct(self, batch, t_env, episode_num):
         a = self.args
@@ -276,6 +292,8 @@
         if self._stats is None or not self._stats_fresh:
             return self._last_stats
         st = self._stats.cpu()
+        if getattr(self, "_gate_ring", None) is not None:
+            self._gate_ring.check_gate()
         self._last_stats = {"loss": float(st[0]), "grad_norm": float(st[1]), "td_error_abs": float(st[2]),
                             "q_taken_mean": float(st[3]), "target_mean": float(st[4])}
         self._stats_fresh = False
diff --git a/ma-league_amd/maleague/steppers/parallel_stepper.py b/ma-league_amd/maleague/steppers/parallel_stepper.py
--- a/ma-league_amd/maleague/steppers/parallel_stepper.py
+++ b/ma-league_amd/maleague/steppers/parallel_stepper.py
@@ -1,5 +1,6 @@
 from __future__ import annotations
 
+import os
 from collections import deque
 from collections.abc import Sequence
 from functools import partial
@@ -122,6 +123,7 @@
         self.t_history = None
         self._launches = 0
         self._ring = None
+        self._ready = (None, 0)
 
     _batch_keys = ("state", "obs", "actions", "avail_actions", "reward", "terminated", "actions_onehot", "filled")
     _HOST_RING = 4
@@ -196,6 +198,20 @@
             return _native.rollout_policy_describe(self._cspec, self.home_mac.agent.dims())
         return _native.rollout_describe(self._cspec, self.home_mac.agent.dims(), self._SELFPLAY)
 
+    _READY_KERNELS = ("v7-static", "v7", "v2")
+
+    def _publishes_slots(self) -> bool:
+        if os.environ.get("MLG_LEARNER_EARLY", "1") == "0" or self._SELFPLAY or self.device.type != "cuda":
+            return False
+        mac = self.home_mac
+        if isinstance(mac, DistinctMAC) or isinstance(mac.agent, DQNAgentNetwork) or \
+                getattr(mac, "agent_output_type", "q") == "pi_logits":
+            return False
+        key = (id(self._cspec), os.environ.get("MLG_ROLLOUT_KERNEL"), os.environ.get("MLG_ROLLOUT_GENERIC"))
+        if getattr(self, "_ready_key", None) != key:
+            self._ready_key, self._ready_ok = key, self.describe_rollout()[0] in self._READY_KERNELS
+        return self._ready_ok
+
     def initialize(self, scheme, groups, preprocess, home_mac, away_mac=None):
         if away_mac is not None:
             raise NotImplementedError("ParallelStepper drives one policy; self-play (home + away MAC) is "
@@ -329,6 +345,8 @@
     def flush(self):
         self._resolve()
         self._finish_post()
+        if self._ring is not None:
+            self._ring.check_gate()
 
     def attach_replay(self, buffer) -> bool:
         ok = (_same_device(buffer.device, self.device) and buffer.max_seq_length == self.episode_limit + 1
@@ -354,7 +372,7 @@
     def last_run_info(self) -> torch.Tensor:
         return self._host_slot if self._zero_copy() and self._host_slot is not None else self._info
 
-    def _run_info(self):
+    def _run_info(self, slot_ready=None, run_tag=0):
         B = self.batch_size
         if self._zero_copy():
             self._host_slot = self._reserve_host()
@@ -363,14 +381,15 @@
             info = self._info
         return _native.MlgRunInfo(info[0:B].data_ptr(), info[4 * B:5 * B].data_ptr(), info[B:3 * B].data_ptr(),
                                   info[3 * B:4 * B].data_ptr(), self.agent_rows.data_ptr(),
-                                  info[5 * B:6 * B].data_ptr())
+                                  info[5 * B:6 * B].data_ptr(), slot_ready, run_tag)
 
     def _timed_launch(self) -> bool:
         self._launches += 1
         return self.timing is not None and self.timing_every > 0 and self._launches % self.timing_every == 0
 
     def _launch_mb(self, mb, epsilon: float, test_mode: bool):
-        run_info = self._run_info()
+        run_info = self._run_info(*self._ready)
+        self._ready = (None, 0)
         (self.home_mac if isinstance(self.home_mac, DistinctMAC) else self.home_mac.agent).packed()
         ev = None
         if self._timed_launch():
@@ -397,9 +416,11 @@
             mb, keep = self._to_mlg(ring)
             mb.B, mb.ring_slot0, mb.ring_size, mb.full_write = self.batch_size, slot0, ring.buffer_size, 1
             mb.slot_extent = ring.extent_ptr()
+            tag = ring.next_run_tag() if self._publishes_slots() else 0
+            self._ready = (ring.ready_flags().data_ptr() if tag else None, tag)
             self._launch_mb(mb, eps, test_mode)
             del keep
-            self.home_batch = RingEpisodeBatch(ring, slot0, self.batch_size)
+            self.home_batch = RingEpisodeBatch(ring, slot0, self.batch_size, tag)
         else:
             self.home_batch = self.new_batch_fn()
             self._launch(self.home_batch, eps, test_mode)
```

Result: no change. 204.0 million, median of 2 (-0.0%).
